# JinfengX/PointCloudPDF

Measured on AMD Instinct MI355X. Metric: points/sec fwd+bwd (PT-v1 Seg50 + PDF U-decoder, 100k-pt scenes), higher is better.
Workload: dtype f32

## Files before the change

### include/pdfops.h

```cpp
#ifndef PDFOPS_H
#define PDFOPS_H

#ifdef __cplusplus
extern "C" {
#endif

#define PDF_OK 0
#define PDF_ERR_BAD_ARG (-1)
#define PDF_ERR_NSAMPLE (-2)
#define PDF_ERR_UNSUPPORTED (-3)

#define PDF_ABI_VERSION 17
int pdf_abi_version(void);
const char *pdf_build_info(void);
int pdf_dist_fma_mode(void);
#define PDF_MMA_F32 0
#define PDF_MMA_F16 1
#define PDF_MMA_BF16 2

int pdf_knn_query(int m, int nsample, const float *xyz, const float *new_xyz,
                  const int *offset, const int *new_offset, int b,
                  int *idx, float *dist2, void *stream);

long pdf_knn_workspace_bytes(int b, int n, int m);
int pdf_knn_grid_supported(int nsample);
int pdf_knn_query_ws(int m, int nsample, int n, const float *xyz, const float *new_xyz, const int *offset,
                     const int *new_offset, int b, int *idx, float *dist2, void *workspace, long workspace_bytes,
                     void *stream);
int pdf_knn_grid_build(int n, const float *xyz, const int *offset, int b, void *workspace, long workspace_bytes, void *stream);
int pdf_knn_query_grid(int m, int nsample, int n, const float *xyz, const float *new_xyz, const int *offset, const int *new_offset, int b,
                       int *idx, float *dist2, void *workspace, long workspace_bytes, void *stream);
int pdf_knn_query_ws_counted(int m, int nsample, int n, const float *xyz, const float *new_xyz, const int *offset,
                             const int *new_offset, int b, int *idx, float *dist2, void *workspace, long workspace_bytes,
                             unsigned long long *pairs, void *stream);
int pdf_knn_query_list(int m, int nsample, const float *xyz, const float *new_xyz, const int *offset,
                       const int *new_offset, int b, int *idx, float *dist2, const int *qlist, const int *qcount,
                       void *stream);

int pdf_ball_query(int m, int nsample, float min_radius, float max_radius, const float *xyz, const float *new_xyz,
                   const int *offset, const int *new_offset, int b, int *idx, float *dist2, void *stream);

int pdf_random_ball_query(int m, int nsample, float min_radius, float max_radius, const int *order, const float *xyz,
                          const float *new_xyz, const int *offset, const int *new_offset, int b, int *idx, float *dist2,
                          void *stream);

int pdf_farthest_point_sampling(int b, int n, const float *xyz, const int *offset,
                                const int *new_offset, float *tmp, int *idx, void *stream);

int pdf_fps_reference_block_log2(int n);

long pdf_fps_workspace_bytes(int b, int n_total);
long pdf_fps_stats_offset(int b, int n_total);
int pdf_farthest_point_sampling_bucketed(int b, int n, int n_total, const float *xyz, const int *offset,
                                         const int *new_offset, void *workspace, long workspace_bytes,
                                         int *idx, void *stream);

int pdf_grouping_forward(int m, int nsample, int c, const float *input, const int *idx, float *output, void *stream);
int pdf_grouping_backward(int m, int nsample, int c, const float *grad_output, const int *idx, float *grad_input, void *stream);
int pdf_grouping_forward_ordered(int m, int nsample, int c, const float *input, const int *idx, const int *order, float *output, void *stream);
int pdf_group_forward_ordered(int m, int nsample, int c, int with_xyz, const float *feat, const float *xyz, const float *new_xyz,
                              const int *idx, const int *order, float *output, void *stream);
int pdf_interpolation_forward_ordered(int n, int c, int k, const float *input, const int *idx, const float *weight, const int *order,
                                      float *output, void *stream);
int pdf_subtraction_forward_ordered(int n, int nsample, int c, const float *input1, const float *input2, const int *idx, const int *order,
                                    float *output, void *stream);
int pdf_aggregation_forward_ordered(int n, int nsample, int c, int w_c, const float *input, const float *position, const float *weight,
                                    const int *idx, const int *order, float *output, void *stream);

int pdf_interpolation_forward(int n, int c, int k, const float *input, const int *idx, const float *weight, float *output, void *stream);
int pdf_interpolation_backward(int n, int c, int k, const float *grad_output, const int *idx, const float *weight, float *grad_input, void *stream);

int pdf_subtraction_forward(int n, int nsample, int c, const float *input1, const float *input2, const int *idx, float *output, void *stream);
int pdf_subtraction_backward(int n, int nsample, int c, const int *idx, const float *grad_output, float *grad_input1, float *grad_input2, void *stream);

int pdf_aggregation_forward(int n, int nsample, int c, int w_c, const float *input, const float *position,
                            const float *weight, const int *idx, float *output, void *stream);
int pdf_aggregation_backward(int n, int nsample, int c, int w_c, const float *input, const float *position,
                             const float *weight, const int *idx, const float *grad_output,
                             float *grad_input, float *grad_position, float *grad_weight, void *stream);

int pdf_attention_relation_step_forward(int m, int g, int c, const float *query, const float *key, const float *weight,
                                        const int *index_target, const int *index_refer, float *output, void *stream);
int pdf_attention_relation_step_backward(int m, int g, int c, const float *query, float *grad_query,
                                         const float *key, float *grad_key, const float *weight, float *grad_weight,
                                         const int *index_target, const int *index_refer, const float *grad_output, void *stream);
int pdf_attention_fusion_step_forward(int m, int g, int c, const float *weight, const float *value,
                                      const int *index_target, const int *index_refer, float *output, void *stream);
int pdf_attention_fusion_step_backward(int m, int g, int c, const float *weight, float *grad_weight,
                                       const float *value, float *grad_value,
                                       const int *index_target, const int *index_refer, const float *grad_output, void *stream);


int pdf_group_forward(int m, int nsample, int c, int with_xyz, const float *feat, const float *xyz,
                      const float *new_xyz, const int *idx, float *output, void *stream);
int pdf_group_backward(int m, int nsample, int c, int with_xyz, const float *grad_output, const int *idx,
                       float *grad_feat, void *stream);

int pdf_interpolation_weights(int n, int k, const float *dist2, float *weight, void *stream);

int pdf_pt_layer_supported(int nsample, int c);
long pdf_pt_layer_partial_floats(int n, int nsample, int c);
int pdf_pt_layer_forward(int n, int nsample, int c, const float *xq, const float *xk, const float *xv,
                         const float *p, const int *idx, const float *const *weights,
                         const float *const *bn_params, float *const *bn_buffers, int training, float eps,
                         float momentum, float *bn, float *saved, float *H, float *partial, float *out,
                         int storage_bf16, const int *order, void *stream);
int pdf_pt_layer_forward_m(int n, int nsample, int c, const float *xq, const float *xk, const float *xv,
                           const float *p, const int *idx, const float *const *weights,
                           const float *const *bn_params, float *const *bn_buffers, int training, float eps,
                           float momentum, float *bn, float *saved, float *H, float *partial, float *out,
                           int storage_bf16, const int *order, const double *moments, int *out_stat_rows, void *stream);

long pdf_pt_layer_bwd_partial_floats(int n, int nsample, int c);
long pdf_pt_layer_bwd_sums_floats(int c);
int pdf_pt_layer_backward(int n, int nsample, int c, const float *xq, const float *xk, const float *xv,
                          const float *p, const int *idx, const float *const *weights, const float *bn,
                          const float *saved, const float *H, const float *gout, float *gxq, float *gxk,
                          float *gxv, float *G2, float *G3, float *Wsm, float *GR, const int *inv_off, const int *inv_entry,
                          int entry_base, float *partial, float *sums, int storage_bf16, const int *order, const double *moments,
                          void *stream);

int pdf_bn_supported(int c);
long pdf_bn_partial_floats(long n, int c);
int pdf_bn_act_forward(long n, int c, const float *x, const float *res, const float *gamma, const float *beta,
                       float *running_mean, float *running_var, int training, float eps, float momentum, int relu,
                       float *coef, float *partial, float *y, void *stream);
int pdf_bn_act_backward(long n, int c, const float *gy, const float *x, const float *res, const float *coef,
                        int training, int relu, float *partial, float *sums, float *gx, float *gres, void *stream);
int pdf_bn_coef(long n, int c, const float *x, const float *gamma, const float *beta, float *running_mean,
                float *running_var, int training, float eps, float momentum, float *coef, float *partial, void *stream);
int pdf_bn_apply(long n, int c, const float *x, const float *res, const float *coef, int relu, float *y, void *stream);

long pdf_rowlin_partial_floats(long n, int o);
int pdf_rowlin_partial_rows(long n, int k, int o);
int pdf_rowlin_forward(long n, int k, int o, const float *x, long ldx, const float *w, int transpose_w,
                       const float *bias, const float *scale, const float *shift, int relu, float *y, long ldy,
                       int accumulate, float *partial, int mma_input, void *stream);
long pdf_rowlin_wgrad_ws_floats(long n, int k, int o, int ng);
int pdf_rowlin_wgrad(long n, int k, int o, const float *g, long ldg, const float *x, long ldx,
                     const float *scale, const float *shift, int relu, float *dw, float *db, float *ws, int mma_input, void *stream);
int pdf_bn_coef_from_partial(const float *partial, int rows, long n, int c, const float *gamma, const float *beta,
                             float *running_mean, float *running_var, float eps, float momentum, float *coef, void *stream);

int pdf_rowlin_multi(long n, int k, int o, int nin, int nout, const float *const *x, long ldx, const float *const *w,
                     int transpose_w, const float *const *bias, const float *scale, const float *shift, int relu,
                     float *const *y, long ldy, int accumulate, int mma_input, void *stream);
int pdf_rowlin_wgrad_multi(long n, int k, int o, int ng, const float *const *g, long ldg, const float *x, long ldx,
                           const float *scale, const float *shift, int relu, float *const *dw, float *const *db, float *ws, int mma_input, void *stream);
int pdf_rowlin_wgrad_group(long n, int k, int o, int ng, const float *const *g, long ldg, const float *const *x, long ldx,
                           const float *const *scale, const float *const *shift, const int *relu, float *const *dw,
                           float *const *db, float *ws, int mma_input, void *stream);

int pdf_kpconv_supported(int kp, int cin);
int pdf_kpconv_gather(int n, int m, int kp, int cin, const float *query, const float *support, const int *neighbors, const float *x,
                      const float *k_points, float extent, float *weighted, void *stream);
int pdf_kpconv_scatter(int n, int m, int kp, int cin, const float *query, const float *support, const int *neighbors,
                       const float *grad_weighted, const float *k_points, float extent, float *grad_x, void *stream);
int pdf_rowlin_dgrad_bstats(long n, int k, int o, int nin, const float *const *x, long ldx, const float *const *w, float *y, long ldy,
                            const float *bx, long ldb, const float *bcoef, int brelu, float *partial, int *partial_rows,
                            int mma_input, void *stream);
int pdf_rowlin_forward_bn(long n, int k, int o, const float *x, long ldx, const float *w, const float *bias, const float *scale,
                          const float *shift, int relu, float *y, long ldy, float *partial, const float *gamma, const float *beta,
                          float *running_mean, float *running_var, float eps, float momentum, float *coef, int mma_input, void *stream);
int pdf_bn_act_backward_presummed(long n, int c, const float *gy, const float *x, const float *coef, int training, int relu,
                                  const float *partial, int partial_rows, float *sums, float *gx, void *stream);

int pdf_bn_coef_eval_or_partial(const float *partial, int rows, long n, int c, const float *gamma, const float *beta,
                                float *running_mean, float *running_var, int training, float eps, float momentum,
                                float *coef, void *stream);
int pdf_block_pre_forward(long n, int c, void *const *p, int training, float eps, float momentum, int mma_input, void *stream);
int pdf_block_pre_backward(long n, int c, void *const *p, int training, int mma_input, void *stream);
int pdf_block_post_forward(long n, int c, void *const *p, int training, float eps, float momentum, int mma_input, void *stream);
int pdf_block_post_backward(long n, int c, void *const *p, int training, int mma_input, void *stream);
int pdf_bottleneck_forward(long n, int nsample, int c, void *const *p, int training, float eps, float momentum, int storage_bf16, int mma_input, void *stream);
int pdf_bottleneck_backward(long n, int nsample, int c, void *const *p, int training, int entry_base, int storage_bf16, int mma_input, void *stream);
int pdf_linbn_forward(long n, int k, int o, void *const *p, int training, int relu, float eps, float momentum, int mma_input, void *stream);
int pdf_linbn_backward(long n, int k, int o, void *const *p, int training, int relu, int mma_input, void *stream);

int pdf_rowlin_forward_roww(long n, int k, int o, const float *x, long ldx, const float *w, int transpose_w, float *y, long ldy,
                            int accumulate, const float *roww, long rws, int mma_input, void *stream);
int pdf_rowlin_wgrad_roww(long n, int k, int o, const float *g, long ldg, const float *x, long ldx, float *dw, const float *roww,
                          long rws, float *ws, int mma_input, void *stream);
int pdf_bn_bwd_sums(long n, int c, const float *gy, const float *x, const float *coef, int relu, float *partial, float *sums,
                    void *stream);

int pdf_td_supported(int nsample, int cin, int cout);
int pdf_td_tables(long m, int b, const float *p_src, const float *p_new, const int *idx, const int *new_offset, float *rel4, float *Z,
                  float *scene_sums, long n, const int *inv_off, const int *inv_entry, int entry_base,
                  void *stream);
long pdf_td_gram_floats(int cin);
long pdf_td_fwd_scratch_floats(long n, int cin);
long pdf_td_bwd_scratch_floats(long m, int cin, int cout);
int pdf_td_forward(long n, long m, int cin, int cout, void *const *p, int training, float eps, float momentum, int mma_input, void *stream);
int pdf_td_backward(long n, long m, int cin, int cout, void *const *p, int entry_base, int mma_input, void *stream);

int pdf_seg_sum_rows(long n, int c, const float *src, const int *inv_off, const int *inv_entry, int entry_base, float scale, float *out,
                     void *stream);
int pdf_seg_sum_rows_own(long n, int c, int nsample, const float *src, const int *inv_off, const int *inv_entry, int entry_base, float scale,
                         const int *order, float *out, float *out_own, void *stream);
int pdf_seg_sum_rows_strided(long n, int c, const float *src, long src_stride, const int *inv_off, const int *inv_entry, int entry_base,
                             float scale, float *out, void *stream);
int pdf_seg_sum_rows_x(long n, int c, const float *src, long src_stride, int src_bf16, const int *inv_off, const int *inv_entry, int entry_base,
                       float scale, float *out, void *stream);
int pdf_seg_sum_weighted_x(long n, int c, int nsample, int w_c, const float *src, const float *w, int w_bf16, const int *inv_off,
                           const int *inv_entry, int entry_base, const int *order, float *out, void *stream);
int pdf_seg_sum_weighted_ordered(long n, int c, int nsample, int w_c, const float *src, const float *w, const int *inv_off,
                                 const int *inv_entry, int entry_base, const int *order, float *out, void *stream);
int pdf_seg_sum_weighted(long n, int c, int nsample, int w_c, const float *src, const float *w, const int *inv_off, const int *inv_entry,
                         int entry_base, float *out, void *stream);

long pdf_ce_workspace_floats(void);
int pdf_ce_forward(long n, int c, const float *logits, const long *target, long ignore, float *grad, float *acc, float *loss,
                   void *stream);
int pdf_ce_backward(long n, int c, const float *dlogits, const float *acc, const float *gy, float *grad_out, void *stream);

#define PDF_REDUCE_NONE 0
#define PDF_REDUCE_MEAN 1
#define PDF_REDUCE_SUM 2
long pdf_criteria_workspace_floats(int c);
int pdf_ce_ex_forward(long n, int c, const float *logits, const long *target, const float *weight, float label_smoothing, int reduction,
                      long ignore, float *grad, float *acc, float *loss, void *stream);
int pdf_ce_ex_backward(long n, int c, const float *dlogits, const float *acc, const float *gy, int reduction, float *grad_out, void *stream);
int pdf_focal_forward(long n, int c, const float *logits, const long *target, const float *alpha_vec, float alpha, float gamma, int reduction,
                      long ignore, float *grad, float *acc, float *loss, void *stream);
int pdf_focal_backward(long n, int c, const float *dlogits, const float *acc, const float *gy, float *grad_out, void *stream);
int pdf_dice_forward(long n, int c, const float *logits, const long *target, float smooth, float exponent, long ignore, float *prob,
                     float *acc, float *loss, void *stream);
int pdf_dice_backward(long n, int c, const float *prob, const long *target, long ignore, float exponent, const float *acc, const float *gy,
                      float *grad_out, void *stream);
int pdf_bfocal_forward(long n, const float *pred, const float *target, float alpha, float gamma, int logits, int reduce, float *grad,
                       float *acc, float *loss, void *stream);
int pdf_bfocal_backward(long n, const float *dpred, const float *acc, const float *gy, int reduce, float *grad_out, void *stream);

int pdf_cac_supported(int K, int c);
long pdf_cac_workspace_floats(long n, int K, int c, int scenes);
int pdf_cac_soft_proto_forward(long n, int K, int c, int scenes, const float *feat, const float *logits, const int *offset,
                               float conf_thresh, float *proto, float *mass, float *ws, void *stream);
int pdf_cac_soft_proto_backward(long n, int K, int c, int scenes, const float *feat, const float *logits, const int *offset,
                                float conf_thresh, const float *proto, const float *mass, const float *gproto, float *gfeat,
                                float *glogits, void *stream);
int pdf_cac_label_proto_forward(long n, int K, int c, const float *feat, const long *target, const float *base, float *proto,
                                float *count, float *ws, void *stream);
int pdf_cac_label_proto_backward(long n, int K, int c, const long *target, const float *count, const float *gproto, float *gfeat,
                                 void *stream);
int pdf_cac_cosine_forward(long n, int K, int c, int scenes, const float *x, const float *proto, const int *offset, float scale,
                           float *out, void *stream);
int pdf_cac_cosine_backward(long n, int K, int c, int scenes, const float *x, const float *proto, const int *offset, float scale,
                            const float *gout, float *gx, float *gproto, float *ws, void *stream);
// ... 252 lines not shown
```

### pointcloudpdf_amd/_native.py

```python
import ctypes
import os
import threading

import torch

_HERE = os.path.dirname(os.path.abspath(__file__))
DIST_FMA = int(os.environ.get("PDFOPS_DIST_FMA", "0") or 0)
if DIST_FMA not in (0, 1, 2):
    raise RuntimeError(f"PDFOPS_DIST_FMA={DIST_FMA}: expected 0 (as written), 1 or 2 (csrc/pdfops_common.h)")


def library_path(dist_fma=0):
    return os.path.join(_HERE, "lib", "libpdfops.so" if not dist_fma else f"libpdfops_fma{int(dist_fma)}.so")


LIB_PATH = library_path(DIST_FMA)
ABI_VERSION = 17

c_int = ctypes.c_int
c_long = ctypes.c_long
c_void_p = ctypes.c_void_p
c_float = ctypes.c_float
c_double = ctypes.c_double

_PROTOS = {
    "knn_query": "iippppipp",
    "ball_query": "iiffppppipp",
    "random_ball_query": "iiffpppppipp",
    "farthest_point_sampling": "iippppp",
    "grouping_forward": "iiippp",
    "grouping_backward": "iiippp",
    "interpolation_forward": "iiipppp",
    "interpolation_backward": "iiipppp",
    "subtraction_forward": "iiipppp",
    "subtraction_backward": "iiipppp",
    "aggregation_forward": "iiiippppp",
    "aggregation_backward": "iiiipppppppp",
    "attention_relation_step_forward": "iiipppppp",
    "attention_relation_step_backward": "iiippppppppp",
    "attention_fusion_step_forward": "iiippppp",
    "attention_fusion_step_backward": "iiippppppp",
    "attention_step1_forward_v2": "iiiiippppp",
    "attention_step1_backward_v2": "iiiiippppppp",
    "dot_prod_with_idx_forward_v3": "iiiiipppppppp",
    "dot_prod_with_idx_backward_v3": "iiiiipppppppppppp",
    "attention_step2_with_rel_pos_value_forward_v2": "iiiiippppppp",
    "attention_step2_with_rel_pos_value_backward_v2": "iiiiipppppppppp",
    "segment_softmax_forward": "iiippp",
    "segment_softmax_backward": "iiipppp",
}
_HIP_ONLY_PROTOS = {
    "grid_hash": "lippdddippp",
    "grid_hash_f64": "lippdddppp",
    "philox4x64": "llllp",
    "aug_bounds": "ippppp",
    "aug_points": "ilpipppppp",
    "aug_keys": "ilpplp",
    "aug_elastic_noise": "ilpplp",
    "aug_elastic_blur": "ilpppi",
    "aug_elastic_apply": "ilpppppdpp",
    "radius_neighbors_self": "iifppipppl",
    "radius_neighbors_self_adaptive": "iiffppippppl",
    "vote_accumulate": "lipppppp",
    "fragment_bounds": "lliiipppppp",
    "fragment_gather": "lliiipppppipppppppp",
    "fragment_vote": "lliiippppppppp",
    "graph_forest": "lipppppipppl",
    "gmm2_1d": "ipppidd",
    "dot_prod_with_idx_forward_v3_l": "iiiiipppppppp",
    "dot_prod_with_idx_backward_v3_l": "iiiiipppppppppppp",
    "attention_step2_with_rel_pos_value_backward_v2_l": "iiiiipppppppppp",
    "scene_sum_rows": "ipiplip",
    "scene_repeat_rows": "iplipip",
    "region_stats": "ippppifppp",
    "region_seeds": "ippppip",
    "region_grow": "ippipppipiipppp",
    "region_edges": "ipppppippppppppppppl",
    "sort_floats_dev": "ipppppp",
    "gmm2_weak_dev": "ippppppppidd",
    "region_mask": "ippppppp",
    "region_tree": "ippipppppppp",
    "graph_forest_dev": "lipppppippppl",
    "gmm2_1d_dev": "ippppidd",
    "graph_forest_batch_dev": "ippippppppipppl",
    "wa_segment_rows": "iiiipppppplfpplf",
    "wa_segment_rows_ordered": "iiiipppppplfpplfp",
    "wa_table_grad": "iiiippppplfpp",
    "wa_grad_attn": "iiiiiplppplppp",
    "wa_logits_forward": "iiiiipplfpppppp",
    "wa_permute_edges": "iippp",
    "wa_logits_forward_ordered": "iiiiipplfppppppp",
    "wa_grad_attn_ordered": "iiiiiplppplpppp",
    "window_keys": "ippippfippp",
    "window_keys_scene": "ippippfippp",
    "scene_bounds": "ippipp",
    "window_edges_count": "ippipppppp",
    "window_edges_fill": "ipppppppffipppp",
    "group_forward": "iiiippppp",
    "group_backward": "iiiippp",
    "interpolation_weights": "iipp",
# ... 570 lines not shown
        lib.pdf_spconv_colsum_ws_floats.restype = c_long
        lib.pdf_spconv_colsum_ws_floats.argtypes = [c_int]
        lib.pdf_incr_kl_workspace_floats.restype = c_long
        lib.pdf_incr_kl_workspace_floats.argtypes = []
        lib.pdf_incr_kl_forward.restype = c_int
        lib.pdf_incr_kl_forward.argtypes = [c_long, c_int, c_int, c_void_p, c_void_p, c_void_p, c_long, ctypes.c_float, ctypes.c_float,
                                            c_void_p, c_void_p, c_void_p, c_void_p]
        lib.pdf_incr_kl_backward.restype = c_int
        lib.pdf_incr_kl_backward.argtypes = [c_long, c_int, c_void_p, c_void_p, c_void_p, c_void_p, c_void_p]
        lib.pdf_lovasz_workspace_bytes.restype = c_long
        lib.pdf_lovasz_workspace_bytes.argtypes = [c_long, c_int]
        lib.pdf_lovasz_forward.restype = c_int
        lib.pdf_lovasz_forward.argtypes = [c_long, c_int, c_void_p, c_void_p, c_long, c_void_p, c_void_p, c_void_p, c_void_p, c_void_p, c_void_p]
        lib.pdf_lovasz_backward.restype = c_int
        lib.pdf_lovasz_backward.argtypes = [c_long, c_int, c_void_p, c_void_p, ctypes.c_float, c_void_p, c_void_p]
        lib.pdf_openset_metrics_workspace_bytes.restype = c_long
        lib.pdf_openset_metrics_workspace_bytes.argtypes = [c_long, c_int]
        lib.pdf_openset_metrics.restype = c_int
        lib.pdf_openset_metrics.argtypes = [c_long, c_int, c_void_p, c_void_p, c_void_p, c_void_p, c_long, c_void_p, c_int, c_void_p, c_void_p,
                                            c_void_p, c_void_p]
        lib.pdf_knn_rel_moments.restype = c_int
        lib.pdf_knn_rel_moments.argtypes = [c_int, c_long, c_int, c_void_p, c_void_p, c_void_p, c_void_p, c_void_p, c_void_p]
        lib.pdf_knn_rel_moments_ws_doubles.restype = c_long
        lib.pdf_knn_rel_moments_ws_doubles.argtypes = [c_int, c_long]
        lib.pdf_knn_rel_moments_q.restype = c_int
        lib.pdf_knn_rel_moments_q.argtypes = [c_int, c_long, c_int, c_void_p, c_void_p, c_void_p, c_void_p, c_void_p, c_void_p, c_void_p]
        class CopySeg(ctypes.Structure):
            _fields_ = [("src", c_void_p), ("dst", c_void_p), ("nbytes", c_long), ("src_offset", c_void_p), ("sub", c_void_p),
                        ("sub_const", c_int), ("src_elems", c_int)]

        self.CopySeg = CopySeg
        lib.pdf_stage_copy.restype = c_int
        lib.pdf_stage_copy.argtypes = [c_int, c_void_p, c_void_p]
        lib.pdf_scene_morton_keys.restype = c_int
        lib.pdf_scene_morton_keys.argtypes = [c_long, c_int, c_void_p, c_void_p, c_void_p, c_void_p, c_void_p]
        lib.pdf_sgd_chunk.restype = c_int
        lib.pdf_sgd_chunk.argtypes = []
        lib.pdf_sgd_step.restype = c_int
        lib.pdf_sgd_step.argtypes = [c_int, c_void_p, c_void_p, ctypes.c_float, ctypes.c_float, ctypes.c_float, c_void_p, c_void_p]
        lib.pdf_grad_unscale.restype = c_int
        lib.pdf_grad_unscale.argtypes = [c_int, c_void_p, c_void_p, c_void_p, c_void_p, c_void_p]
        lib.pdf_scaler_update.restype = c_int
        lib.pdf_scaler_update.argtypes = [c_void_p, c_void_p, c_void_p, c_void_p, ctypes.c_float, ctypes.c_float, c_int, c_void_p]
        lib.pdf_adam_step.restype = c_int
        lib.pdf_adam_step.argtypes = [c_int, c_int, c_void_p, c_void_p, ctypes.c_double, ctypes.c_double, ctypes.c_double, ctypes.c_double,
                                      ctypes.c_double, c_int, c_void_p, c_void_p]
        lib.pdf_adam_grad_unscale.restype = c_int
        lib.pdf_adam_grad_unscale.argtypes = [c_int, c_void_p, c_void_p, c_void_p, c_void_p, c_void_p]
        lib.pdf_linbn_forward.restype = c_int
        lib.pdf_linbn_forward.argtypes = [c_long, c_int, c_int, c_void_p, c_int, c_int, ctypes.c_float, ctypes.c_float, c_int, c_void_p]
        lib.pdf_linbn_backward.restype = c_int
        lib.pdf_linbn_backward.argtypes = [c_long, c_int, c_int, c_void_p, c_int, c_int, c_int, c_void_p]
        lib.pdf_bottleneck_forward.restype = c_int
        lib.pdf_bottleneck_forward.argtypes = [c_long, c_int, c_int, c_void_p, c_int, ctypes.c_float, ctypes.c_float, c_int, c_int, c_void_p]
        lib.pdf_bottleneck_backward.restype = c_int
        lib.pdf_bottleneck_backward.argtypes = [c_long, c_int, c_int, c_void_p, c_int, c_int, c_int, c_int, c_void_p]
        for nm in ("pre_backward", "post_backward"):
            f = getattr(lib, "pdf_block_" + nm)
            f.restype = c_int
            f.argtypes = [c_long, c_int, c_void_p, c_int, c_int, c_void_p]
        lib.pdf_rowlin_multi.restype = c_int
        lib.pdf_rowlin_multi.argtypes = [c_long, c_int, c_int, c_int, c_int, c_void_p, c_long, c_void_p, c_int, c_void_p, c_void_p, c_void_p,
                                         c_int, c_void_p, c_long, c_int, c_int, c_void_p]
        lib.pdf_kpconv_supported.restype = c_int
        lib.pdf_kpconv_supported.argtypes = [c_int, c_int]
        for nm in ("pdf_kpconv_gather", "pdf_kpconv_scatter"):
            f = getattr(lib, nm)
            f.restype = c_int
            f.argtypes = [c_int, c_int, c_int, c_int, c_void_p, c_void_p, c_void_p, c_void_p, c_void_p, ctypes.c_float, c_void_p, c_void_p]
        lib.pdf_rowlin_wgrad_group.restype = c_int
        lib.pdf_rowlin_wgrad_group.argtypes = [c_long, c_int, c_int, c_int, c_void_p, c_long, c_void_p, c_long, c_void_p, c_void_p, c_void_p,
                                               c_void_p, c_void_p, c_void_p, c_int, c_void_p]
        lib.pdf_rowlin_wgrad_multi.restype = c_int
        lib.pdf_rowlin_wgrad_multi.argtypes = [c_long, c_int, c_int, c_int, c_void_p, c_long, c_void_p, c_long, c_void_p, c_void_p, c_int,
                                               c_void_p, c_void_p, c_void_p, c_int, c_void_p]
        lib.pdf_rowlin_wgrad_ws_floats.restype = c_long
        lib.pdf_rowlin_wgrad_ws_floats.argtypes = [c_long, c_int, c_int, c_int]
        lib.pdf_rowlin_dgrad_bstats.restype = c_int
        lib.pdf_rowlin_dgrad_bstats.argtypes = [c_long, c_int, c_int, c_int, c_void_p, c_long, c_void_p, c_void_p, c_long, c_void_p, c_long,
                                                c_void_p, c_int, c_void_p, ctypes.POINTER(c_int), c_int, c_void_p]
        lib.pdf_bn_act_backward_presummed.restype = c_int
        lib.pdf_bn_act_backward_presummed.argtypes = [c_long, c_int, c_void_p, c_void_p, c_void_p, c_int, c_int, c_void_p, c_int, c_void_p,
                                                      c_void_p, c_void_p]
        lib.pdf_rowlin_partial_floats.restype = c_long
        lib.pdf_rowlin_partial_floats.argtypes = [c_long, c_int]
        lib.pdf_rowlin_partial_rows.restype = c_int
        lib.pdf_rowlin_partial_rows.argtypes = [c_long, c_int, c_int]
        lib.pdf_rowlin_forward.restype = c_int
        lib.pdf_rowlin_forward.argtypes = [c_long, c_int, c_int, c_void_p, c_long, c_void_p, c_int, c_void_p, c_void_p, c_void_p,
                                           c_int, c_void_p, c_long, c_int, c_void_p, c_int, c_void_p]
        lib.pdf_rowlin_wgrad.restype = c_int
        lib.pdf_rowlin_wgrad.argtypes = [c_long, c_int, c_int, c_void_p, c_long, c_void_p, c_long, c_void_p, c_void_p, c_int,
                                         c_void_p, c_void_p, c_void_p, c_int, c_void_p]
        lib.pdf_bn_coef_from_partial.restype = c_int
        lib.pdf_bn_coef_from_partial.argtypes = [c_void_p, c_int, c_long, c_int, c_void_p, c_void_p, c_void_p, c_void_p,
                                                 ctypes.c_float, ctypes.c_float, c_void_p, c_void_p]
        lib.pdf_bn_coef.restype = c_int
        lib.pdf_bn_coef.argtypes = [c_long, c_int, c_void_p, c_void_p, c_void_p, c_void_p, c_void_p, c_int, ctypes.c_float,
                                    ctypes.c_float, c_void_p, c_void_p, c_void_p]
        lib.pdf_bn_apply.restype = c_int
        lib.pdf_bn_apply.argtypes = [c_long, c_int, c_void_p, c_void_p, c_void_p, c_int, c_void_p, c_void_p]
        lib.pdf_bn_supported.restype = c_int
        lib.pdf_bn_supported.argtypes = [c_int]
        lib.pdf_bn_partial_floats.restype = c_long
        lib.pdf_bn_partial_floats.argtypes = [c_long, c_int]
        lib.pdf_bn_act_forward.restype = c_int
        lib.pdf_bn_act_forward.argtypes = [c_long, c_int] + [c_void_p] * 6 + [c_int, ctypes.c_float, ctypes.c_float, c_int] + [c_void_p] * 4
        lib.pdf_bn_act_backward.restype = c_int
        lib.pdf_bn_act_backward.argtypes = [c_long, c_int] + [c_void_p] * 4 + [c_int, c_int] + [c_void_p] * 5
        lib.pdf_pt_layer_supported.restype = c_int
        lib.pdf_pt_layer_supported.argtypes = [c_int, c_int]
        for fn in (lib.pdf_pt_layer_partial_floats, lib.pdf_pt_layer_bwd_partial_floats):
            fn.restype = c_long
            fn.argtypes = [c_int, c_int, c_int]
        lib.pdf_pt_layer_bwd_sums_floats.restype = c_long
        lib.pdf_pt_layer_bwd_sums_floats.argtypes = [c_int]
        lib.pdf_pt_layer_forward.restype = c_int
        lib.pdf_pt_layer_forward.argtypes = [c_int, c_int, c_int] + [c_void_p] * 8 + [c_int, ctypes.c_float, ctypes.c_float] + [c_void_p] * 5 + [c_int, c_void_p, c_void_p]
        lib.pdf_knn_grid_build.restype = c_int
        lib.pdf_knn_grid_build.argtypes = [c_int, c_void_p, c_void_p, c_int, c_void_p, c_long, c_void_p]
        lib.pdf_knn_query_grid.restype = c_int
        lib.pdf_knn_query_grid.argtypes = [c_int, c_int, c_int, c_void_p, c_void_p, c_void_p, c_void_p, c_int, c_void_p, c_void_p, c_void_p, c_long, c_void_p]
        lib.pdf_pt_layer_backward.restype = c_int
        lib.pdf_pt_layer_backward.argtypes = [c_int, c_int, c_int] + [c_void_p] * 19 + [c_int] + [c_void_p] * 2 + [c_int, c_void_p, c_void_p, c_void_p]
        lib.pdf_grid_pool_workspace_bytes.restype = c_long
        lib.pdf_grid_pool_workspace_bytes.argtypes = [c_long]
        lib.pdf_gva_supported.restype = c_int
        lib.pdf_gva_supported.argtypes = [c_int, c_int, c_int]
        self.fps_mode = os.environ.get("PDFOPS_FPS", "bucketed")
        self.knn_mode = os.environ.get("PDFOPS_KNN", "grid")
        lib.pdf_knn_workspace_bytes.restype = c_long
        lib.pdf_knn_workspace_bytes.argtypes = [c_int, c_int, c_int]
        lib.pdf_graph_forest_workspace_bytes.restype = c_long
        lib.pdf_region_grow_list_points.restype = c_long
        lib.pdf_region_grow_list_points.argtypes = []
        lib.pdf_graph_forest_workspace_bytes.argtypes = [c_long, c_long, c_long]
        lib.pdf_knn_grid_supported.restype = c_int
        lib.pdf_knn_grid_supported.argtypes = [c_int]
        lib.pdf_knn_query_ws.restype = c_int
        lib.pdf_knn_query_ws.argtypes = [c_int, c_int, c_int] + [c_void_p] * 4 + [c_int] + [c_void_p] * 3 + [c_long, c_void_p]
        lib.pdf_knn_query_ws_counted.restype = c_int
        lib.pdf_knn_query_ws_counted.argtypes = [c_int, c_int, c_int] + [c_void_p] * 4 + [c_int] + [c_void_p] * 3 + [c_long, c_void_p, c_void_p]

    KNN_GRID_MAX_SCENES = 64
    use_inverse = os.environ.get("PDFOPS_INVERSE", "1") != "0"
    storage_bf16 = os.environ.get("PDFOPS_STORAGE", "f32") == "bf16"

    def set_storage(self, kind):
        if kind not in ("f32", "bf16"):
            raise ValueError("storage: 'f32' or 'bf16'")
        self.storage_bf16 = kind == "bf16"

    def grouping_forward(self, input, idx):
        _check(input, torch.float32, "input"); _check(idx, torch.int32, "idx")
        m, ns = idx.shape
        c = input.shape[1]
        out = self._new(input, (m, ns, c), torch.float32)
        self._call("grouping_forward_ordered", m, ns, c, input, idx, order_of(idx), out)
        return out

    def interpolation_forward(self, input, idx, weight):
        _check(input, torch.float32, "input"); _check(idx, torch.int32, "idx"); _check(weight, torch.float32, "weight")
        n, k = idx.shape
        c = input.shape[1]
        out = self._new(input, (n, c), torch.float32)
        self._call("interpolation_forward_ordered", n, c, k, input, idx, weight, order_of(idx), out)
# ... 1534 lines not shown
```

### pointcloudpdf_amd/csrc/block.hip

```cpp
#include "pdfops_common.h"

namespace {
struct Err {
    int rc = 0;
    Err &operator<<(int r) { if (rc == 0 && r != 0) rc = r; return *this; }
};

}

extern "C" int pdf_bn_coef_eval_or_partial(const float *partial, int rows, long n, int c, const float *gamma, const float *beta,
                                           float *running_mean, float *running_var, int training, float eps, float momentum,
                                           float *coef, void *stream) {
    if (training) return pdf_bn_coef_from_partial(partial, rows, n, c, gamma, beta, running_mean, running_var, eps, momentum, coef, stream);
    return pdf_bn_coef(n, c, nullptr, gamma, beta, running_mean, running_var, 0, eps, momentum, coef, nullptr, stream);
}

extern "C" int pdf_block_pre_forward(long n, int c, void *const *p, int training, float eps, float momentum, int mma_input, void *stream) {
    if (n < 1 || !p) return PDF_ERR_BAD_ARG;
    if (!pdf_bn_supported(c)) return PDF_ERR_UNSUPPORTED;
    const float *x = (const float *)p[0], *W1 = (const float *)p[1], *g1 = (const float *)p[2], *b1 = (const float *)p[3];
    float *rm1 = (float *)p[4], *rv1 = (float *)p[5];
    float *z1 = (float *)p[12], *coef1 = (float *)p[13], *partial = (float *)p[17];
    Err e;
    if (training) {
        e << pdf_rowlin_forward_bn(n, c, c, x, c, W1, nullptr, nullptr, nullptr, 0, z1, c, partial, g1, b1, rm1, rv1, eps, momentum, coef1, mma_input, stream);
    } else {
        e << pdf_rowlin_forward(n, c, c, x, c, W1, 0, nullptr, nullptr, nullptr, 0, z1, c, 0, nullptr, mma_input, stream);
        e << pdf_bn_coef_eval_or_partial(partial, 0, n, c, g1, b1, rm1, rv1, 0, eps, momentum, coef1, stream);
    }
    const float *xs[1] = {z1}, *ws[3] = {(const float *)p[6], (const float *)p[8], (const float *)p[10]};
    const float *bs[3] = {(const float *)p[7], (const float *)p[9], (const float *)p[11]};
    float *ys[3] = {(float *)p[14], (float *)p[15], (float *)p[16]};
    e << pdf_rowlin_multi(n, c, c, 1, 3, xs, c, ws, 0, bs, coef1, coef1 + c, 1, ys, c, 0, mma_input, stream);
    return e.rc;
}

static bool inkernel_bn() {
    static const bool on = [] { const char *v = getenv("PDFOPS_INKERNEL_BN"); return !(v && v[0] == '0'); }();
    return on;
}
static bool dgrad_bstats() {
    static const bool on = [] { const char *v = getenv("PDFOPS_DGRAD_BSTATS"); return !(v && v[0] == '0'); }();
    return on;
}

static int block_pre_backward(long n, int c, void *const *p, int training, int accumulate_gx, int mma_input, void *stream, bool defer_wgrad = false) {
    if (n < 1 || !p || !p[14]) return PDF_ERR_BAD_ARG;
    const float *x = (const float *)p[0], *z1 = (const float *)p[1], *coef1 = (const float *)p[2], *W1 = (const float *)p[3];
    float *gx = (float *)p[10], *grads = (float *)p[11], *dy = (float *)p[12], *partial = (float *)p[13], *wslab = (float *)p[14];
    const long cc = (long)c * c;
    float *dW1 = grads, *db1 = grads + cc, *dqkv = db1 + 2 * c;
    Err e;
    const float *gs[3] = {(const float *)p[7], (const float *)p[8], (const float *)p[9]};
    const float *ws[3] = {(const float *)p[4], (const float *)p[5], (const float *)p[6]};
    float *dws[3] = {dqkv, dqkv + (cc + c), dqkv + 2 * (cc + c)}, *dbs[3] = {dqkv + cc, dqkv + (cc + c) + cc, dqkv + 2 * (cc + c) + cc};
    float *ys[1] = {dy};
    if (!defer_wgrad) e << pdf_rowlin_wgrad_multi(n, c, c, 3, gs, c, z1, c, coef1, coef1 + c, 1, dws, dbs, wslab, mma_input, stream);
    int prow = 0;
    const int rc1 = dgrad_bstats() ? pdf_rowlin_dgrad_bstats(n, c, c, 3, gs, c, ws, dy, c, z1, c, coef1, 1, partial, &prow, mma_input, stream) : PDF_ERR_UNSUPPORTED;
    if (rc1 == PDF_ERR_UNSUPPORTED) {
        e << pdf_rowlin_multi(n, c, c, 3, 1, gs, c, ws, 1, nullptr, nullptr, nullptr, 0, ys, c, 0, mma_input, stream);
        e << pdf_bn_act_backward(n, c, dy, z1, nullptr, coef1, training, 1, partial, db1, dy, nullptr, stream);
    } else {
        e << rc1;
        e << pdf_bn_act_backward_presummed(n, c, dy, z1, coef1, training, 1, partial, prow, db1, dy, stream);
    }
    if (!defer_wgrad) e << pdf_rowlin_wgrad(n, c, c, dy, c, x, c, nullptr, nullptr, 0, dW1, nullptr, wslab, mma_input, stream);
    e << pdf_rowlin_forward(n, c, c, dy, c, W1, 1, nullptr, nullptr, nullptr, 0, gx, c, accumulate_gx, nullptr, mma_input, stream);
    return e.rc;
}

extern "C" int pdf_block_pre_backward(long n, int c, void *const *p, int training, int mma_input, void *stream) {
    return block_pre_backward(n, c, p, training, 0, mma_input, stream, false);
}

static int block_post_forward(long n, int c, void *const *p, int training, float eps, float momentum, int t_stat_rows, int mma_input, void *stream) {
    if (n < 1 || !p) return PDF_ERR_BAD_ARG;
    if (!pdf_bn_supported(c)) return PDF_ERR_UNSUPPORTED;
    const float *t = (const float *)p[0], *x = (const float *)p[1];
    float *coef2 = (float *)p[11], *z3 = (float *)p[12], *coef3 = (float *)p[13], *y = (float *)p[14], *partial = (float *)p[15];
    Err e;
    if (training && t_stat_rows > 0)
        e << pdf_bn_coef_from_partial(partial, t_stat_rows, n, c, (const float *)p[2], (const float *)p[3], (float *)p[4], (float *)p[5], eps, momentum, coef2, stream);
    else
        e << pdf_bn_coef(n, c, t, (const float *)p[2], (const float *)p[3], (float *)p[4], (float *)p[5], training, eps, momentum, coef2, partial, stream);
    bool applied = false;
    if (training && inkernel_bn()) {
        int rows = 0;
        const int rc = pdf_rowlin_forward_stats_ho(n, c, c, t, c, (const float *)p[6], nullptr, coef2, coef2 + c, 1, z3, c, partial + PDF_HO_FLOATS, partial,
                                                   &rows, mma_input, stream);
        if (rc == PDF_OK) {
            e << pdf_bn_apply_rows(n, c, z3, x, partial + PDF_HO_FLOATS, rows, (const float *)p[7], (const float *)p[8], (float *)p[9], (float *)p[10], eps,
                                   momentum, coef3, partial, 1, y, stream);
            applied = true;
        } else if (rc != PDF_ERR_UNSUPPORTED) {
            e << rc;
        }
    }
    if (applied) return e.rc;
    if (training) {
        e << pdf_rowlin_forward_bn(n, c, c, t, c, (const float *)p[6], nullptr, coef2, coef2 + c, 1, z3, c, partial, (const float *)p[7], (const float *)p[8],
                                   (float *)p[9], (float *)p[10], eps, momentum, coef3, mma_input, stream);
    } else {
        e << pdf_rowlin_forward(n, c, c, t, c, (const float *)p[6], 0, nullptr, coef2, coef2 + c, 1, z3, c, 0, nullptr, mma_input, stream);
        e << pdf_bn_coef_eval_or_partial(partial, 0, n, c, (const float *)p[7], (const float *)p[8], (float *)p[9], (float *)p[10], 0, eps, momentum, coef3, stream);
    }
    e << pdf_bn_apply(n, c, z3, x, coef3, 1, y, stream);
    return e.rc;
}
extern "C" int pdf_block_post_forward(long n, int c, void *const *p, int training, float eps, float momentum, int mma_input, void *stream) {
    return block_post_forward(n, c, p, training, eps, momentum, 0, mma_input, stream);
}

static int block_post_backward(long n, int c, void *const *p, int training, int mma_input, void *stream, bool defer_wgrad = false) {
    if (n < 1 || !p || !p[12]) return PDF_ERR_BAD_ARG;
    const float *gy = (const float *)p[0], *t = (const float *)p[1], *x = (const float *)p[2], *z3 = (const float *)p[3];
    const float *coef2 = (const float *)p[4], *coef3 = (const float *)p[5], *W3 = (const float *)p[6];
    float *gt = (float *)p[7], *gres = (float *)p[8], *grads = (float *)p[9], *da = (float *)p[10], *partial = (float *)p[11];
    const long cc = (long)c * c;
    float *dW3 = grads, *db2 = grads + cc, *db3 = db2 + 2 * c;
    Err e;
    e << pdf_bn_act_backward(n, c, gy, z3, x, coef3, training, 1, partial, db3, da, gres, stream);
    if (!defer_wgrad) e << pdf_rowlin_wgrad(n, c, c, da, c, t, c, coef2, coef2 + c, 1, dW3, nullptr, (float *)p[12], mma_input, stream);
    int prow = 0;
    const float *das[1] = {da}, *w3s[1] = {W3};
    const int rc2 = dgrad_bstats() ? pdf_rowlin_dgrad_bstats(n, c, c, 1, das, c, w3s, gt, c, t, c, coef2, 1, partial, &prow, mma_input, stream) : PDF_ERR_UNSUPPORTED;
    if (rc2 == PDF_ERR_UNSUPPORTED) {
        e << pdf_rowlin_forward(n, c, c, da, c, W3, 1, nullptr, nullptr, nullptr, 0, gt, c, 0, nullptr, mma_input, stream);
        e << pdf_bn_act_backward(n, c, gt, t, nullptr, coef2, training, 1, partial, db2, gt, nullptr, stream);
    } else {
        e << rc2;
        e << pdf_bn_act_backward_presummed(n, c, gt, t, coef2, training, 1, partial, prow, db2, gt, stream);
    }
    return e.rc;
}

extern "C" int pdf_block_post_backward(long n, int c, void *const *p, int training, int mma_input, void *stream) {
    return block_post_backward(n, c, p, training, mma_input, stream, false);
}

extern "C" int pdf_bottleneck_forward(long n, int nsample, int c, void *const *p, int training, float eps, float momentum, int storage_bf16, int mma_input, void *stream) {
    if (n < 1 || !p) return PDF_ERR_BAD_ARG;
    Err e;
    void *pre[18] = {p[0], p[1], p[2], p[3], p[4], p[5], p[6], p[7], p[8], p[9], p[10], p[11], p[43], p[44], p[45], p[46], p[47], p[56]};
    e << pdf_block_pre_forward(n, c, pre, training, eps, momentum, mma_input, stream);
    const float *weights[8], *bn_params[6];
    float *bn_buffers[6];
    for (int i = 0; i < 8; ++i) weights[i] = (const float *)p[14 + i];
    for (int i = 0; i < 6; ++i) { bn_params[i] = (const float *)p[22 + i]; bn_buffers[i] = (float *)p[28 + i]; }
    static const bool p4_stats = [] { const char *v = getenv("PDFOPS_P4_STATS"); return !(v && v[0] == '0'); }();
    int t_rows = 0;
    e << pdf_pt_layer_forward_m((int)n, nsample, c, (const float *)p[45], (const float *)p[46], (const float *)p[47], (const float *)p[12],
                                (const int *)p[13], weights, bn_params, bn_buffers, training, eps, momentum, (float *)p[48], (float *)p[49],
                                (float *)p[50], (float *)p[56], (float *)p[51], storage_bf16, (const int *)p[57], (const double *)p[58],
                                p4_stats ? &t_rows : nullptr, stream);
    void *post[16] = {p[51], p[0], p[34], p[35], p[36], p[37], p[38], p[39], p[40], p[41], p[42], p[52], p[53], p[54], p[55], p[56]};
    e << block_post_forward(n, c, post, training, eps, momentum, e.rc == 0 ? t_rows : 0, mma_input, stream);
    return e.rc;
}

extern "C" int pdf_bottleneck_backward(long n, int nsample, int c, void *const *p, int training, int entry_base, int storage_bf16, int mma_input, void *stream) {
    if (n < 1 || !p) return PDF_ERR_BAD_ARG;
    Err e;
    if (!p[50]) return PDF_ERR_BAD_ARG;
    static const bool group = [] { const char *v = getenv("PDFOPS_WGRAD_GROUP"); return !(v && v[0] == '0'); }();
    float *ws_post = (float *)p[50], *ws_pre = ws_post + pdf_rowlin_wgrad_ws_floats(n, c, c, 1);
    void *post[13] = {p[0], p[24], p[1], p[25], p[26], p[27], p[28], p[33], p[29], p[31], p[34], p[40], ws_post};
    e << block_post_backward(n, c, post, training, mma_input, stream, group);
    const float *weights[8];
    for (int i = 0; i < 8; ++i) weights[i] = (const float *)p[10 + i];
    e << pdf_pt_layer_backward((int)n, nsample, c, (const float *)p[21], (const float *)p[22], (const float *)p[23], (const float *)p[8],
                               (const int *)p[9], weights, (const float *)p[18], (const float *)p[19], (const float *)p[20],
                               (const float *)p[33], (float *)p[35], (float *)p[36], (float *)p[37], (float *)p[38], (float *)p[39],
                               (float *)p[41], (float *)p[42], (const int *)p[43], (const int *)p[44], entry_base,
                               (float *)p[40], (float *)p[32], storage_bf16, (const int *)p[49], (const double *)p[46], stream);
    void *pre[15] = {p[1], p[2], p[3], p[4], p[5], p[6], p[7], p[35], p[36], p[37], p[29], p[30], p[45], p[40], ws_pre};
    e << block_pre_backward(n, c, pre, training, 1, mma_input, stream, group);
    if (group && e.rc == 0) {
        const long cc = (long)c * c;
        float *gpre = (float *)p[30], *gpost = (float *)p[31];
        float *dW1 = gpre, *dqkv = gpre + cc + 2 * c, *dW3 = gpost;
        const float *coef1 = (const float *)p[3], *coef2 = (const float *)p[26];
        const float *g[5] = {(const float *)p[34], (const float *)p[35], (const float *)p[36], (const float *)p[37], (const float *)p[45]};
        const float *x[5] = {(const float *)p[24], (const float *)p[2], (const float *)p[2], (const float *)p[2], (const float *)p[1]};
        const float *sc[5] = {coef2, coef1, coef1, coef1, nullptr}, *sh[5] = {coef2 + c, coef1 + c, coef1 + c, coef1 + c, nullptr};
        const int relu[5] = {1, 1, 1, 1, 0};
        float *dw[5] = {dW3, dqkv, dqkv + (cc + c), dqkv + 2 * (cc + c), dW1};
        float *db[5] = {nullptr, dqkv + cc, dqkv + (cc + c) + cc, dqkv + 2 * (cc + c) + cc, nullptr};
        const int rc = pdf_rowlin_wgrad_group(n, c, c, 5, g, c, x, c, sc, sh, relu, dw, db, ws_post, mma_input, stream);
        if (rc == PDF_ERR_UNSUPPORTED) {
            e << pdf_rowlin_wgrad(n, c, c, g[0], c, x[0], c, sc[0], sh[0], 1, dw[0], nullptr, ws_post, mma_input, stream);
            e << pdf_rowlin_wgrad_multi(n, c, c, 3, g + 1, c, x[1], c, sc[1], sh[1], 1, dw + 1, db + 1, ws_pre, mma_input, stream);
            e << pdf_rowlin_wgrad(n, c, c, g[4], c, x[4], c, nullptr, nullptr, 0, dw[4], nullptr, ws_pre, mma_input, stream);
        } else {
            e << rc;
        }
    }
    return e.rc;
}

extern "C" int pdf_linbn_forward(long n, int k, int o, void *const *p, int training, int relu, float eps, float momentum, int mma_input, void *stream) {
    if (n < 1 || !p) return PDF_ERR_BAD_ARG;
    if (!pdf_bn_supported(o)) return PDF_ERR_UNSUPPORTED;
    Err e;
    float *z = (float *)p[7], *coef = (float *)p[8], *partial = (float *)p[10];
    if (training) {
        e << pdf_rowlin_forward_bn(n, k, o, (const float *)p[0], k, (const float *)p[1], (const float *)p[2], nullptr, nullptr, 0, z, o, partial,
                                   (const float *)p[3], (const float *)p[4], (float *)p[5], (float *)p[6], eps, momentum, coef, mma_input, stream);
    } else {
        e << pdf_rowlin_forward(n, k, o, (const float *)p[0], k, (const float *)p[1], 0, (const float *)p[2], nullptr, nullptr, 0, z, o, 0, nullptr, mma_input, stream);
        e << pdf_bn_coef_eval_or_partial(partial, 0, n, o, (const float *)p[3], (const float *)p[4], (float *)p[5], (float *)p[6], 0, eps, momentum, coef, stream);
    }
    e << pdf_bn_apply(n, o, z, nullptr, coef, relu, (float *)p[9], stream);
    return e.rc;
}

extern "C" int pdf_linbn_backward(long n, int k, int o, void *const *p, int training, int relu, int mma_input, void *stream) {
    if (n < 1 || !p || !p[9]) return PDF_ERR_BAD_ARG;
    float *grads = (float *)p[6], *gz = (float *)p[7];
    const long ok = (long)o * k;
    Err e;
    e << pdf_bn_act_backward(n, o, (const float *)p[0], (const float *)p[2], nullptr, (const float *)p[3], training, relu, (float *)p[8],
                             grads + ok + o, gz, nullptr, stream);
    if (p[5]) e << pdf_rowlin_forward(n, o, k, gz, o, (const float *)p[4], 1, nullptr, nullptr, nullptr, 0, (float *)p[5], k, 0, nullptr, mma_input, stream);
    e << pdf_rowlin_wgrad(n, k, o, gz, o, (const float *)p[1], k, nullptr, nullptr, 0, grads, grads + ok, (float *)p[9], mma_input, stream);
    return e.rc;
}
```

### pointcloudpdf_amd/csrc/pdfops_common.h

```cpp
#pragma once
#include <hip/hip_runtime.h>
#include <stdint.h>
#include <atomic>
#include "../../include/pdfops.h"

#define PDF_WAVE 64
#define PDF_MAX_DEVICES_LDS 64

static inline int pdf_launch_status() {
    hipError_t e = hipGetLastError();
    return e == hipSuccess ? PDF_OK : (int)e;
}

struct PdfLdsLimit { std::atomic<int> state[PDF_MAX_DEVICES_LDS]; };
static inline bool pdf_lds_limit_raised(PdfLdsLimit &site, const void *kernel, int bytes) {
    int dev = 0;
    if (hipGetDevice(&dev) != hipSuccess || dev < 0 || dev >= PDF_MAX_DEVICES_LDS) return hipFuncSetAttribute(kernel, hipFuncAttributeMaxDynamicSharedMemorySize, bytes) == hipSuccess;
    int st = site.state[dev].load(std::memory_order_acquire);
    if (st == 0) {
        st = hipFuncSetAttribute(kernel, hipFuncAttributeMaxDynamicSharedMemorySize, bytes) == hipSuccess ? 1 : 2;
        if (st == 2) (void)hipGetLastError();
        site.state[dev].store(st, std::memory_order_release);
    }
    return st == 1;
// ... 9 lines not shown
        T *p = reinterpret_cast<T *>(reinterpret_cast<uintptr_t>(base) + off);
        off += (count * sizeof(T) + 255) & ~(size_t)255;
        return p;
    }
};

#define PDF_MAX_BLOCKS 2048

__device__ __forceinline__ int pdf_lane() { return (int)(threadIdx.x & 63); }

__device__ __forceinline__ void wave_sync() {
    __builtin_amdgcn_fence(__ATOMIC_RELEASE, "wavefront");
    __builtin_amdgcn_wave_barrier();
    __builtin_amdgcn_fence(__ATOMIC_ACQUIRE, "wavefront");
}

__device__ __forceinline__ int pdf_wave_min_i32(int v) {
#pragma unroll
    for (int o = 32; o >= 1; o >>= 1) v = min(v, __shfl_xor(v, o, 64));
    return v;
}
__device__ __forceinline__ int pdf_wave_max_i32(int v) {
#pragma unroll
    for (int o = 32; o >= 1; o >>= 1) v = max(v, __shfl_xor(v, o, 64));
    return v;
}
__device__ __forceinline__ unsigned long long pdf_wave_max_u64(unsigned long long v) {
#pragma unroll
    for (int o = 32; o >= 1; o >>= 1) {
        unsigned long long w = __shfl_xor(v, o, 64);
        v = w > v ? w : v;
    }
    return v;
}
__device__ __forceinline__ float pdf_wave_sum_f32(float v) {
#pragma unroll
    for (int o = 32; o >= 1; o >>= 1) v += __shfl_xor(v, o, 64);
    return v;
}

#ifndef PDF_DIST_FMA
#define PDF_DIST_FMA 0
#endif
__host__ __device__ __forceinline__ float pdf_sqdist3(float dx, float dy, float dz) {
#if PDF_DIST_FMA == 1
    return __builtin_fmaf(dz, dz, __builtin_fmaf(dy, dy, dx * dx));
#elif PDF_DIST_FMA == 2
    return __builtin_fmaf(dz, dz, __builtin_fmaf(dx, dx, dy * dy));
#else
    return dx * dx + dy * dy + dz * dz;
#endif
}

__device__ __forceinline__ unsigned pdf_f32_ordered(float f) {
    unsigned u = __float_as_uint(f);
    return (u & 0x80000000u) ? ~u : (u | 0x80000000u);
}

__device__ __forceinline__ void pdf_atomic_add(float *p, float v) {
    __hip_atomic_fetch_add(p, v, __ATOMIC_RELAXED, __HIP_MEMORY_SCOPE_AGENT);
}

#define PDF_XCDS 8
__device__ __forceinline__ unsigned pdf_xcd_chunked_block(unsigned b, unsigned g) {
    const unsigned q = g / PDF_XCDS, r = g % PDF_XCDS, x = b % PDF_XCDS;
    return (x < r ? x * (q + 1) : r * (q + 1) + (x - r) * q) + b / PDF_XCDS;
}

struct PdfRowsBn {
    const float *rows; int nrows; int c; double count;
    const float *gamma, *beta; float *running_mean, *running_var; float eps, momentum;
    float *coef;
    unsigned long long *gran;
    unsigned *sync;
};
#define PDF_HO_WORDS(c) (2 * (size_t)(c) * 2 + 4)
#define PDF_HO_FLOATS PDF_HO_WORDS(1024)
int pdf_rowlin_forward_stats_ho(long n, int k, int o, const float *x, long ldx, const float *w, const float *bias, const float *scale,
                                const float *shift, int relu, float *y, long ldy, float *rows_out, void *handoff, int *rows, int mma_input,
                                void *stream);
int pdf_bn_apply_rows(long n, int c, const float *x, const float *res, const float *rows, int nrows, const float *gamma, const float *beta,
                      float *running_mean, float *running_var, float eps, float momentum, float *coef, void *handoff, int relu, float *y,
                      void *stream);

__device__ __forceinline__ void pdf_handoff_zero(unsigned long long *gran, int c, unsigned *sync) {
    for (int e = threadIdx.x; e < 2 * c; e += blockDim.x) gran[e] = 0ull;
    if (threadIdx.x == 0) sync[0] = 0u;
}

template <int NT>
__device__ __forceinline__ void pdf_bn_reduce_slice(const PdfRowsBn &b, int sl, double *lds_red) {
    constexpr int RL = NT / 16;
    const int c = b.c, cl = threadIdx.x & 15, rl = threadIdx.x >> 4;
    const int ch = sl * 16 + cl;
    double s = 0.0, ss = 0.0;
    if (ch < c) {
        const float *p0 = b.rows + ch, *p1 = b.rows + c + ch;
        const size_t stride = 2 * (size_t)c;
        for (int r = rl; r < b.nrows; r += 8 * RL) {
            float v0[8], v1[8];
#pragma unroll
            for (int t = 0; t < 8; ++t) {
                const int rr = r + t * RL < b.nrows ? r + t * RL : b.nrows - 1;
                v0[t] = p0[(size_t)rr * stride]; v1[t] = p1[(size_t)rr * stride];
            }
#pragma unroll
            for (int t = 0; t < 8; ++t) {
                const bool ok = r + t * RL < b.nrows;
                s += ok ? (double)v0[t] : 0.0; ss += ok ? (double)v1[t] : 0.0;
            }
        }
    }
    __syncthreads();
    lds_red[(0 * RL + rl) * 17 + cl] = s;
    lds_red[(1 * RL + rl) * 17 + cl] = ss;
    __syncthreads();
    if (rl == 0 && ch < c) {
        double a = 0.0, q = 0.0;
        for (int k = 0; k < RL; ++k) { a += lds_red[(0 * RL + k) * 17 + cl]; q += lds_red[(1 * RL + k) * 17 + cl]; }
        const double mean = a / b.count;
        double var = q / b.count - mean * mean;
        if (var < 0.0) var = 0.0;
        const float rstd = (float)(1.0 / sqrt(var + (double)b.eps));
        const float sc = b.gamma[ch] * rstd, sh = b.beta[ch] - (float)mean * sc;
        b.coef[ch] = sc; b.coef[c + ch] = sh; b.coef[2 * c + ch] = (float)mean; b.coef[3 * c + ch] = rstd;
        if (b.running_mean && b.sync != nullptr) {
            const double unbiased = b.count > 1.0 ? var * b.count / (b.count - 1.0) : var;
            b.running_mean[ch] = (1.f - b.momentum) * b.running_mean[ch] + b.momentum * (float)mean;
            b.running_var[ch] = (1.f - b.momentum) * b.running_var[ch] + b.momentum * (float)unbiased;
        }
        __hip_atomic_store(b.gran + ch, (1ull << 32) | (unsigned long long)__float_as_uint(sc), __ATOMIC_RELAXED, __HIP_MEMORY_SCOPE_AGENT);
        __hip_atomic_store(b.gran + c + ch, (1ull << 32) | (unsigned long long)__float_as_uint(sh), __ATOMIC_RELAXED, __HIP_MEMORY_SCOPE_AGENT);
    }
}

template <int NT>
__device__ __forceinline__ void pdf_bn_coef_inkernel(const PdfRowsBn &b, float *lds_coef, double *lds_red, unsigned *lds_word) {
    (void)lds_word;
    const int c = b.c, nsl = (c + 15) / 16;
    const unsigned me = blockIdx.x + gridDim.x * (blockIdx.y + gridDim.y * blockIdx.z), nblk = gridDim.x * gridDim.y * gridDim.z;
    for (unsigned sl = me; sl < (unsigned)nsl; sl += nblk) pdf_bn_reduce_slice<NT>(b, (int)sl, lds_red);
    for (unsigned spins = 0;; ++spins) {
        bool ok = true;
        for (int e = threadIdx.x; e < 2 * c; e += NT) {
            const unsigned long long g = __hip_atomic_load(b.gran + e, __ATOMIC_RELAXED, __HIP_MEMORY_SCOPE_AGENT);
            ok = ok && (g >> 32) == 1ull;
            lds_coef[e] = __uint_as_float((unsigned)g);
        }
        if (__syncthreads_and(ok)) break;
        if (spins == (1u << 14)) {
            PdfRowsBn mine = b;
            mine.sync = nullptr;
            for (int sl = 0; sl < nsl; ++sl) pdf_bn_reduce_slice<NT>(mine, sl, lds_red);
        }
        __builtin_amdgcn_s_sleep(8);
    }
}
```

### pointcloudpdf_amd/csrc/pointwise.hip

```cpp
#include "pdfops_common.h"
#include <cstdlib>

namespace pw {

constexpr int PB = 256;
constexpr int MAXB = 1024;

static inline int grid_rows(long n, int c) {
    const long rows_per_block = (long)PB * 4 / c > 0 ? (long)PB * 4 / c : 1;
    static const int short_rows = [] { const char *v = getenv("PDFOPS_BN_ROWS_SHORT"); const int x = v ? atoi(v) : 0; return x > 0 ? x : 4; }();
    const long per = n * c >= (1L << 22) ? 8 : short_rows;
    long g = (n + rows_per_block * per - 1) / (rows_per_block * per);
    if (g > MAXB) g = MAXB;
    if (g < 1) g = 1;
    return (int)g;
}

__global__ __launch_bounds__(PB) void k_bn_stats(long n, int c, const float *__restrict__ x, float *partial) {
    extern __shared__ float red[];
    const int tpr = c / 4;
    const int rpb = PB / tpr;
    const int tr = threadIdx.x / tpr, tc = threadIdx.x % tpr;
    float s[4] = {0.f, 0.f, 0.f, 0.f}, ss[4] = {0.f, 0.f, 0.f, 0.f};
    if (tr < rpb) {
        for (long r = (long)blockIdx.x * rpb + tr; r < n; r += (long)gridDim.x * rpb) {
            const float4 v = *reinterpret_cast<const float4 *>(x + r * c + tc * 4);
            s[0] += v.x; s[1] += v.y; s[2] += v.z; s[3] += v.w;
            ss[0] += v.x * v.x; ss[1] += v.y * v.y; ss[2] += v.z * v.z; ss[3] += v.w * v.w;
        }
    }
#pragma unroll
    for (int k = 0; k < 4; ++k) { red[threadIdx.x * 8 + k] = s[k]; red[threadIdx.x * 8 + 4 + k] = ss[k]; }
    __syncthreads();
    if (threadIdx.x < tpr) {
#pragma unroll
        for (int k = 0; k < 8; ++k) {
            float a = 0.f;
            for (int rr = 0; rr < rpb; ++rr) a += red[(rr * tpr + threadIdx.x) * 8 + k];
            const int ch = threadIdx.x * 4 + (k & 3);
            partial[(size_t)blockIdx.x * 2 * c + (k < 4 ? ch : c + ch)] = a;
        }
    }
}

template <bool RES>
__global__ __launch_bounds__(PB) void k_bn_apply(long n4, int c4, const float4 *__restrict__ x, const float4 *__restrict__ scale,
                                                 const float4 *__restrict__ shift, const float4 *__restrict__ res, int relu,
                                                 float4 *__restrict__ y) {
    for (long e = (long)blockIdx.x * PB + threadIdx.x; e < n4; e += (long)gridDim.x * PB) {
        const int cc = (int)(e % c4);
        const float4 v = x[e], sc = scale[cc], sh = shift[cc];
        const float4 r = RES ? res[e] : make_float4(0.f, 0.f, 0.f, 0.f);
        float4 o = make_float4(v.x * sc.x + sh.x + r.x, v.y * sc.y + sh.y + r.y, v.z * sc.z + sh.z + r.z, v.w * sc.w + sh.w + r.w);
        if (relu) { o.x = fmaxf(o.x, 0.f); o.y = fmaxf(o.y, 0.f); o.z = fmaxf(o.z, 0.f); o.w = fmaxf(o.w, 0.f); }
        y[e] = o;
    }
}

template <bool RES>
__global__ __launch_bounds__(PB) void k_bn_apply_rows(long n4, int c4, const float4 *__restrict__ x, PdfRowsBn b, const float4 *__restrict__ res,
                                                      int relu, float4 *__restrict__ y) {
    extern __shared__ __attribute__((aligned(16))) float lds[];
    const int c = 4 * c4;
    double *red = reinterpret_cast<double *>(lds + 2 * c);
    unsigned *word = reinterpret_cast<unsigned *>(red + 2 * (PB / 16) * 17);
    pdf_bn_coef_inkernel<PB>(b, lds, red, word);
    const float4 *scale = reinterpret_cast<const float4 *>(lds), *shift = reinterpret_cast<const float4 *>(lds + c);
    for (long e = (long)blockIdx.x * PB + threadIdx.x; e < n4; e += (long)gridDim.x * PB) {
        const int cc = (int)(e % c4);
        const float4 v = x[e], sc = scale[cc], sh = shift[cc];
        const float4 r = RES ? res[e] : make_float4(0.f, 0.f, 0.f, 0.f);
        float4 o = make_float4(v.x * sc.x + sh.x + r.x, v.y * sc.y + sh.y + r.y, v.z * sc.z + sh.z + r.z, v.w * sc.w + sh.w + r.w);
        if (relu) { o.x = fmaxf(o.x, 0.f); o.y = fmaxf(o.y, 0.f); o.z = fmaxf(o.z, 0.f); o.w = fmaxf(o.w, 0.f); }
        y[e] = o;
    }
}

template <bool RES>
__global__ __launch_bounds__(PB) void k_bn_bwd_reduce(long n, int c, const float *__restrict__ gy, const float *__restrict__ x,
                                                      const float *__restrict__ res, const float *__restrict__ scale,
                                                      const float *__restrict__ shift, const float *__restrict__ mean,
                                                      const float *__restrict__ rstd, int relu, float *partial) {
    extern __shared__ float red[];
    const int tpr = c / 4, rpb = PB / tpr;
    const int tr = threadIdx.x / tpr, tc = threadIdx.x % tpr;
    float s[4] = {0.f, 0.f, 0.f, 0.f}, sx[4] = {0.f, 0.f, 0.f, 0.f};
    if (tr < rpb) {
        float sc[4], sh[4], mu[4], rs[4];
#pragma unroll
        for (int k = 0; k < 4; ++k) { sc[k] = scale[tc * 4 + k]; sh[k] = shift[tc * 4 + k]; mu[k] = mean[tc * 4 + k]; rs[k] = rstd[tc * 4 + k]; }
        for (long r = (long)blockIdx.x * rpb + tr; r < n; r += (long)gridDim.x * rpb) {
            const float4 g4 = *reinterpret_cast<const float4 *>(gy + r * c + tc * 4);
            const float4 x4 = *reinterpret_cast<const float4 *>(x + r * c + tc * 4);
            const float4 r4 = RES ? *reinterpret_cast<const float4 *>(res + r * c + tc * 4) : make_float4(0.f, 0.f, 0.f, 0.f);
            const float g[4] = {g4.x, g4.y, g4.z, g4.w}, xv[4] = {x4.x, x4.y, x4.z, x4.w}, rv[4] = {r4.x, r4.y, r4.z, r4.w};
#pragma unroll
            for (int k = 0; k < 4; ++k) {
                const float pre = xv[k] * sc[k] + sh[k] + rv[k];
                const float gm = (!relu || pre > 0.f) ? g[k] : 0.f;
                s[k] += gm;
                sx[k] += gm * ((xv[k] - mu[k]) * rs[k]);
            }
        }
    }
#pragma unroll
    for (int k = 0; k < 4; ++k) { red[threadIdx.x * 8 + k] = s[k]; red[threadIdx.x * 8 + 4 + k] = sx[k]; }
    __syncthreads();
    if (threadIdx.x < tpr) {
#pragma unroll
        for (int k = 0; k < 8; ++k) {
            float a = 0.f;
            for (int rr = 0; rr < rpb; ++rr) a += red[(rr * tpr + threadIdx.x) * 8 + k];
            const int ch = threadIdx.x * 4 + (k & 3);
            partial[(size_t)blockIdx.x * 2 * c + (k < 4 ? ch : c + ch)] = a;
        }
    }
}

template <bool RES>
__global__ __launch_bounds__(PB) void k_bn_bwd_apply(long n4, int c4, const float4 *__restrict__ gy, const float4 *__restrict__ x,
                                                     const float4 *__restrict__ res, const float4 *__restrict__ scale,
                                                     const float4 *__restrict__ shift, const float4 *__restrict__ mean,
                                                     const float4 *__restrict__ rstd, const float4 *__restrict__ sums, float inv_n,
                                                     int relu, float4 *__restrict__ gx, float4 *__restrict__ gres) {
    for (long e = (long)blockIdx.x * PB + threadIdx.x; e < n4; e += (long)gridDim.x * PB) {
        const int cc = (int)(e % c4);
        const float4 g4 = gy[e], x4 = x[e], sc = scale[cc], sh = shift[cc], mu = mean[cc], rs = rstd[cc];
        const float4 s1 = sums[cc], s2 = sums[c4 + cc];
        const float4 r4 = RES ? res[e] : make_float4(0.f, 0.f, 0.f, 0.f);
        float4 gm, o;
#define PW_ONE(f)                                                                     \
        {                                                                             \
            const float pre = x4.f * sc.f + sh.f + r4.f;                              \
            gm.f = (!relu || pre > 0.f) ? g4.f : 0.f;                                 \
            const float xh = (x4.f - mu.f) * rs.f;                                    \
            o.f = sc.f * (gm.f - s1.f * inv_n - xh * s2.f * inv_n);                   \
        }
        PW_ONE(x) PW_ONE(y) PW_ONE(z) PW_ONE(w)
#undef PW_ONE
        gx[e] = o;
        if (gres) gres[e] = gm;
    }
}

template <bool RES>
__global__ __launch_bounds__(PB) void k_bn_bwd_eval(long n4, int c4, const float4 *__restrict__ gy, const float4 *__restrict__ x,
                                                    const float4 *__restrict__ res, const float4 *__restrict__ scale,
                                                    const float4 *__restrict__ shift, int relu, float4 *__restrict__ gx,
                                                    float4 *__restrict__ gres) {
    for (long e = (long)blockIdx.x * PB + threadIdx.x; e < n4; e += (long)gridDim.x * PB) {
        const int cc = (int)(e % c4);
        const float4 g4 = gy[e], x4 = x[e], sc = scale[cc], sh = shift[cc];
        const float4 r4 = RES ? res[e] : make_float4(0.f, 0.f, 0.f, 0.f);
        float4 gm;
        gm.x = (!relu || x4.x * sc.x + sh.x + r4.x > 0.f) ? g4.x : 0.f;
        gm.y = (!relu || x4.y * sc.y + sh.y + r4.y > 0.f) ? g4.y : 0.f;
        gm.z = (!relu || x4.z * sc.z + sh.z + r4.z > 0.f) ? g4.z : 0.f;
        gm.w = (!relu || x4.w * sc.w + sh.w + r4.w > 0.f) ? g4.w : 0.f;
        gx[e] = make_float4(gm.x * sc.x, gm.y * sc.y, gm.z * sc.z, gm.w * sc.w);
        if (gres) gres[e] = gm;
    }
}

static inline int grid_elems(long n4) {
    long g = (n4 + PB - 1) / PB;
    if (g > 2048) g = 2048;
    if (g < 1) g = 1;
    return (int)g;
}

}

namespace fl {
void launch_bn_finalize(const float *partial, int rows, int nch, double count, const float *gamma, const float *beta, float eps,
                        float momentum, float *running_mean, float *running_var, float *scale, float *shift, float *mean_out,
                        float *rstd_out, hipStream_t s);
void launch_bn_eval(int nch, const float *gamma, const float *beta, float eps, const float *running_mean, const float *running_var,
                    float *scale, float *shift, float *mean_out, float *rstd_out, hipStream_t s);
void launch_colsum(const float *partial, int rows, int width, float *out, hipStream_t s);
}

extern "C" int pdf_bn_supported(int c) { return c >= 4 && c % 4 == 0 && c <= 1024 && (1024 % c == 0); }
extern "C" long pdf_bn_partial_floats(long n, int c) { return (long)pw::grid_rows(n, c) * 2 * c + (long)PDF_HO_FLOATS; }

extern "C" int pdf_bn_act_forward(long n, int c, const float *x, const float *res, const float *gamma, const float *beta,
                                  float *running_mean, float *running_var, int training, float eps, float momentum,
                                  int relu, float *coef, float *partial, float *y, void *stream) {
    if (n < 1 || !x || !gamma || !beta || !coef || !y) return PDF_ERR_BAD_ARG;
    if (!pdf_bn_supported(c)) return PDF_ERR_UNSUPPORTED;
    hipStream_t s = static_cast<hipStream_t>(stream);
    float *scale = coef, *shift = coef + c, *mean = coef + 2 * c, *rstd = coef + 3 * c;
    if (training) {
        if (!partial) return PDF_ERR_BAD_ARG;
        const int g = pw::grid_rows(n, c);
        pw::k_bn_stats<<<g, pw::PB, pw::PB * 8 * sizeof(float), s>>>(n, c, x, partial);
        fl::launch_bn_finalize(partial, g, c, (double)n, gamma, beta, eps, momentum, running_mean, running_var, scale, shift, mean, rstd, s);
    } else {
        if (!running_mean || !running_var) return PDF_ERR_BAD_ARG;
        fl::launch_bn_eval(c, gamma, beta, eps, running_mean, running_var, scale, shift, mean, rstd, s);
    }
    const long n4 = n * (c / 4);
    (res ? pw::k_bn_apply<true> : pw::k_bn_apply<false>)<<<pw::grid_elems(n4), pw::PB, 0, s>>>(n4, c / 4, reinterpret_cast<const float4 *>(x),
                                                        reinterpret_cast<const float4 *>(scale), reinterpret_cast<const float4 *>(shift),
                                                        reinterpret_cast<const float4 *>(res), relu, reinterpret_cast<float4 *>(y));
    return pdf_launch_status();
}

static int bn_act_backward(long n, int c, const float *gy, const float *x, const float *res, const float *coef,
                           int training, int relu, float *partial, float *sums, int sums_zeroed, float *gx, float *gres, void *stream,
                           int presummed = 0) {
    (void)sums_zeroed;
    if (n < 1 || !gy || !x || !coef || !partial || !sums || !gx) return PDF_ERR_BAD_ARG;
    if (!pdf_bn_supported(c)) return PDF_ERR_UNSUPPORTED;
    hipStream_t s = static_cast<hipStream_t>(stream);
    const float *scale = coef, *shift = coef + c, *mean = coef + 2 * c, *rstd = coef + 3 * c;
    const int g = pw::grid_rows(n, c);
    const long n4 = n * (c / 4);
    if (presummed > 0) {
        fl::launch_colsum(partial, presummed, 2 * c, sums, s);
    } else {
        (res ? pw::k_bn_bwd_reduce<true> : pw::k_bn_bwd_reduce<false>)<<<g, pw::PB, pw::PB * 8 * sizeof(float), s>>>(
            n, c, gy, x, res, scale, shift, mean, rstd, relu, partial);
        fl::launch_colsum(partial, g, 2 * c, sums, s);
    }
#define F4(p) reinterpret_cast<const float4 *>(p)
    if (training)
        (res ? pw::k_bn_bwd_apply<true> : pw::k_bn_bwd_apply<false>)<<<pw::grid_elems(n4), pw::PB, 0, s>>>(n4, c / 4, F4(gy), F4(x), F4(res), F4(scale), F4(shift), F4(mean), F4(rstd),
                                                                F4(sums), (float)(1.0 / (double)n), relu, reinterpret_cast<float4 *>(gx),
                                                                reinterpret_cast<float4 *>(gres));
    else
        (res ? pw::k_bn_bwd_eval<true> : pw::k_bn_bwd_eval<false>)<<<pw::grid_elems(n4), pw::PB, 0, s>>>(n4, c / 4, F4(gy), F4(x), F4(res), F4(scale), F4(shift), relu,
                                                               reinterpret_cast<float4 *>(gx), reinterpret_cast<float4 *>(gres));
#undef F4
    return pdf_launch_status();
}

extern "C" int pdf_bn_act_backward(long n, int c, const float *gy, const float *x, const float *res, const float *coef,
                                   int training, int relu, float *partial, float *sums, float *gx, float *gres, void *stream) {
    return bn_act_backward(n, c, gy, x, res, coef, training, relu, partial, sums, 0, gx, gres, stream);
}
extern "C" int pdf_bn_act_backward_presummed(long n, int c, const float *gy, const float *x, const float *coef, int training, int relu,
                                             const float *partial, int partial_rows, float *sums, float *gx, void *stream) {
    if (partial_rows < 1 || !partial) return PDF_ERR_BAD_ARG;
    return bn_act_backward(n, c, gy, x, nullptr, coef, training, relu, const_cast<float *>(partial), sums, 0, gx, nullptr, stream, partial_rows);
}
extern "C" int pdf_bn_coef_from_partial(const float *partial, int rows, long n, int c, const float *gamma, const float *beta,
                                        float *running_mean, float *running_var, float eps, float momentum, float *coef,
                                        void *stream) {
    if (!partial || rows < 1 || n < 1 || c < 1 || !gamma || !beta || !coef) return PDF_ERR_BAD_ARG;
    fl::launch_bn_finalize(partial, rows, c, (double)n, gamma, beta, eps, momentum, running_mean, running_var, coef, coef + c,
                           coef + 2 * c, coef + 3 * c, static_cast<hipStream_t>(stream));
    return pdf_launch_status();
}

extern "C" int pdf_bn_apply(long n, int c, const float *x, const float *res, const float *coef, int relu, float *y, void *stream) {
    if (n < 1 || !x || !coef || !y) return PDF_ERR_BAD_ARG;
    if (!pdf_bn_supported(c)) return PDF_ERR_UNSUPPORTED;
    const long n4 = n * (c / 4);
    (res ? pw::k_bn_apply<true> : pw::k_bn_apply<false>)<<<pw::grid_elems(n4), pw::PB, 0, static_cast<hipStream_t>(stream)>>>(
        n4, c / 4, reinterpret_cast<const float4 *>(x), reinterpret_cast<const float4 *>(coef), reinterpret_cast<const float4 *>(coef + c),
        reinterpret_cast<const float4 *>(res), relu, reinterpret_cast<float4 *>(y));
    return pdf_launch_status();
}

int pdf_bn_apply_rows(long n, int c, const float *x, const float *res, const float *rows, int nrows, const float *gamma, const float *beta,
                      float *running_mean, float *running_var, float eps, float momentum, float *coef, void *handoff, int relu, float *y,
                      void *stream) {
    if (n < 1 || !x || !rows || nrows < 1 || !gamma || !beta || !coef || !handoff || !y) return PDF_ERR_BAD_ARG;
    if (!pdf_bn_supported(c)) return PDF_ERR_UNSUPPORTED;
    PdfRowsBn b;
    b.rows = rows; b.nrows = nrows; b.c = c; b.count = (double)n; b.gamma = gamma; b.beta = beta; b.running_mean = running_mean;
    b.running_var = running_var; b.eps = eps; b.momentum = momentum; b.coef = coef;
    b.gran = static_cast<unsigned long long *>(handoff); b.sync = reinterpret_cast<unsigned *>(b.gran + 2 * (size_t)c);
    const long n4 = n * (c / 4);
    const size_t lds = sizeof(float) * 2 * c + sizeof(double) * 2 * (pw::PB / 16) * 17 + 16;
    (res ? pw::k_bn_apply_rows<true> : pw::k_bn_apply_rows<false>)<<<pw::grid_elems(n4), pw::PB, lds, static_cast<hipStream_t>(stream)>>>(
        n4, c / 4, reinterpret_cast<const float4 *>(x), b, reinterpret_cast<const float4 *>(res), relu, reinterpret_cast<float4 *>(y));
    return pdf_launch_status();
}

extern "C" int pdf_bn_coef(long n, int c, const float *x, const float *gamma, const float *beta, float *running_mean,
                           float *running_var, int training, float eps, float momentum, float *coef, float *partial, void *stream) {
    if (n < 1 || !gamma || !beta || !coef) return PDF_ERR_BAD_ARG;
    if (!pdf_bn_supported(c)) return PDF_ERR_UNSUPPORTED;
    hipStream_t s = static_cast<hipStream_t>(stream);
    if (training) {
        if (!partial || !x) return PDF_ERR_BAD_ARG;
        const int g = pw::grid_rows(n, c);
        pw::k_bn_stats<<<g, pw::PB, pw::PB * 8 * sizeof(float), s>>>(n, c, x, partial);
        fl::launch_bn_finalize(partial, g, c, (double)n, gamma, beta, eps, momentum, running_mean, running_var, coef, coef + c, coef + 2 * c, coef + 3 * c, s);
    } else {
        if (!running_mean || !running_var) return PDF_ERR_BAD_ARG;
        fl::launch_bn_eval(c, gamma, beta, eps, running_mean, running_var, coef, coef + c, coef + 2 * c, coef + 3 * c, s);
    }
    return pdf_launch_status();
}

extern "C" int pdf_bn_bwd_sums(long n, int c, const float *gy, const float *x, const float *coef, int relu, float *partial, float *sums,
                               void *stream) {
    if (n < 1 || !gy || !x || !coef || !partial || !sums) return PDF_ERR_BAD_ARG;
    if (!pdf_bn_supported(c)) return PDF_ERR_UNSUPPORTED;
    hipStream_t s = static_cast<hipStream_t>(stream);
    const int g = pw::grid_rows(n, c);
    pw::k_bn_bwd_reduce<false><<<g, pw::PB, pw::PB * 8 * sizeof(float), s>>>(n, c, gy, x, nullptr, coef, coef + c, coef + 2 * c, coef + 3 * c, relu, partial);
    fl::launch_colsum(partial, g, 2 * c, sums, s);
    return pdf_launch_status();
}
```

### pointcloudpdf_amd/csrc/rowlin.hip

```cpp
#include "pdfops_common.h"
#include <cstdlib>

namespace rl {

typedef float f32x16 __attribute__((ext_vector_type(16)));
constexpr int BM = 128, BN = 64, BK = 32, LDT = 33;

struct FwdArgs {
    long N;
    int K, O;
    const float *X; long ldx;
    const float *W; long wso, wsk;
    const float *bias;
    const float *scale, *shift;
    int relu;
    float *Y; long ldy;
    int accumulate;
    float *partial;
};

template <bool PRE, bool STATS>
__global__ __launch_bounds__(256) void k_rowlin(FwdArgs a) {
    __shared__ float xs[BM * LDT];
    __shared__ float ws[BN * LDT];
// ... 64 lines not shown
        }
    }
    if (STATS) {
        __syncthreads();
        if (tid < BN && o0 + tid < a.O) {
            const float s = red[0][0][tid] + red[1][0][tid] + red[2][0][tid] + red[3][0][tid];
            const float ss = red[0][1][tid] + red[1][1][tid] + red[2][1][tid] + red[3][1][tid];
            a.partial[(size_t)blockIdx.x * 2 * a.O + o0 + tid] = s;
            a.partial[(size_t)blockIdx.x * 2 * a.O + a.O + o0 + tid] = ss;
        }
    }
}

struct WArgs {
    long N;
    int K, O;
    const float *G; long ldg;
    const float *X; long ldx;
    const float *scale, *shift;
    int relu;
    float *dW;
    float *db;
    long rows_per_block;
    float *slab;
    float *bslab;
};

template <bool PRE>
__global__ __launch_bounds__(256) void k_wgrad(WArgs a) {
    const int lane = threadIdx.x & 63, wave = threadIdx.x >> 6;
    const int kblocks = (a.K + 31) / 32;
    const int o0 = (blockIdx.y / kblocks) * 32, c0 = (blockIdx.y % kblocks) * 32;
    const int ch = lane & 31, par = lane >> 5;
    const int oc = o0 + ch, cc = c0 + ch;
    const bool ov = oc < a.O, cv = cc < a.K;
    float sc = 1.f, sh = 0.f;
    if (PRE && cv) { sc = a.scale[cc]; sh = a.shift[cc]; }
    const long rb = (long)blockIdx.x * a.rows_per_block;
    const long re = min(rb + a.rows_per_block, a.N);
    f32x16 acc;
#pragma unroll
    for (int r = 0; r < 16; ++r) acc[r] = 0.f;
    float gsum = 0.f;
    for (long r0 = rb + 8 * wave; r0 < re; r0 += 32) {
        float g[4], x[4];
#pragma unroll
        for (int u = 0; u < 4; ++u) {
            const long r = r0 + 2 * u + par;
            g[u] = (r < re && ov) ? a.G[r * a.ldg + oc] : 0.f;
            float v = 0.f;
            if (r < re && cv) {
                v = a.X[r * a.ldx + cc];
                if (PRE) { v = v * sc + sh; if (a.relu) v = fmaxf(v, 0.f); }
            }
            x[u] = v;
        }
#pragma unroll
        for (int u = 0; u < 4; ++u) {
            acc = __builtin_amdgcn_mfma_f32_32x32x2f32(g[u], x[u], acc, 0, 0, 0);
            gsum += g[u];
        }
    }
    __shared__ float comb[4][1024 + 32];
#pragma unroll
    for (int r = 0; r < 16; ++r) {
        const int i = (r & 3) + 8 * (r >> 2) + 4 * (lane >> 5);
        comb[wave][i * 32 + ch] = acc[r];
    }
    gsum += __shfl_xor(gsum, 32, 64);
    if (lane < 32) comb[wave][1024 + ch] = gsum;
    __syncthreads();
    const size_t sidx = blockIdx.x, nsl = gridDim.x;
    float *slab = a.slab + ((size_t)blockIdx.y * nsl + sidx) * 1024;
#pragma unroll
    for (int e = threadIdx.x; e < 1024; e += 256) slab[e] = ((comb[0][e] + comb[1][e]) + comb[2][e]) + comb[3][e];
    if (a.db && c0 == 0 && threadIdx.x < 32)
        a.bslab[((size_t)(o0 / 32) * nsl + sidx) * 32 + threadIdx.x] =
            ((comb[0][1024 + threadIdx.x] + comb[1][1024 + threadIdx.x]) + comb[2][1024 + threadIdx.x]) + comb[3][1024 + threadIdx.x];
}

}

namespace rl2 {
int try_forward(long n, int k, int o, int nin, int nout, const float *const *x, long ldx, const float *const *w, int transpose_w,
                const float *const *bias, const float *scale, const float *shift, int relu, float *const *y, long ldy,
                int accumulate, float *partial, int mma, hipStream_t s, const float *roww = nullptr, long rws = 0, const float *bx = nullptr,
                long ldb = 0, const float *bcoef = nullptr, int brelu = 0, int *partial_rows = nullptr, long ldw = 0, void *handoff = nullptr);
long stats_rows_floats(long n, int o);
int try_wgrad(long n, int k, int o, int ng, const float *const *g, long ldg, const float *x, long ldx, const float *scale,
              const float *shift, int relu, float *const *dw, float *const *db, float *ws, int mma, hipStream_t s, const float *roww = nullptr, long rws = 0);
long wgrad_ws_floats(long n, int k, int o, int ng);
constexpr int WG_MAXG = 5;
struct RArgs {
    const float *slab, *bslab;
    float *dW[WG_MAXG], *db[WG_MAXG];
    int B, tiles_k, tiles, otiles, split, K, O;
};
int try_wgrad_group(long n, int k, int o, int ng, const float *const *g, long ldg, const float *const *x, long ldx, const float *const *scale,
                    const float *const *shift, const int *relu, float *const *dw, float *const *db, float *ws, int mma, hipStream_t s);
void launch_slab_reduce(const RArgs &a, int ng, bool any_bias, hipStream_t s);
int stats_rows(long n);
}

static inline void tiled_wg_plan(long n, int k, int o, int *blocks_oc, long *split, long *rows_per_block) {
    *blocks_oc = ((o + 31) / 32) * ((k + 31) / 32);
    long sp = (2048 + *blocks_oc - 1) / *blocks_oc;
    const long max_split = (n + 255) / 256;
    if (sp > max_split) sp = max_split;
    if (sp < 1) sp = 1;
    *rows_per_block = ((n + sp - 1) / sp + 31) / 32 * 32;
    *split = (n + *rows_per_block - 1) / *rows_per_block;
}

static inline bool rowlin_streams(int k, int o) {
    return (k == 32 || k == 64 || k == 128 || k == 256 || k == 512) && o % 16 == 0 && getenv("PDFOPS_ROWLIN_TILED") == nullptr;
}

extern "C" int pdf_rowlin_partial_rows(long n, int k, int o) {
    return rowlin_streams(k, o) ? rl2::stats_rows(n) : (int)((n + rl::BM - 1) / rl::BM);
}
extern "C" long pdf_rowlin_partial_floats(long n, int o) {
    const long a = (n + rl::BM - 1) / rl::BM * 2 * (long)o, b = rl2::stats_rows_floats(n, o);
    return (a > b ? a : b) + (long)PDF_HO_FLOATS;
}

extern "C" int pdf_rowlin_forward(long n, int k, int o, const float *x, long ldx, const float *w, int transpose_w,
                                  const float *bias, const float *scale, const float *shift, int relu, float *y, long ldy,
                                  int accumulate, float *partial, int mma_input, void *stream) {
    if (mma_input < 0 || mma_input > 2) return PDF_ERR_BAD_ARG;
    if (n < 1 || k < 1 || o < 1 || !x || !w || !y || ldx < k || ldy < o) return PDF_ERR_BAD_ARG;
    if (rowlin_streams(k, o)) {
        if (rl2::try_forward(n, k, o, 1, 1, &x, ldx, &w, transpose_w, &bias, scale, shift, relu, &y, ldy, accumulate, partial,
                             mma_input, static_cast<hipStream_t>(stream)))
            return pdf_launch_status();
        if (partial) return PDF_ERR_BAD_ARG;
    }
    if (!transpose_w && !partial && !scale && k == 1024 && rowlin_streams(512, o) && !(ldx & 3) && !(ldy & 3)) {
        const float *xs[2] = {x, x + 512}, *ws[2] = {w, w + 512};
        if (rl2::try_forward(n, 512, o, 2, 1, xs, ldx, ws, 0, &bias, nullptr, nullptr, 0, &y, ldy, accumulate, nullptr, mma_input, static_cast<hipStream_t>(stream),
                             nullptr, 0, nullptr, 0, nullptr, 0, nullptr, k))
            return pdf_launch_status();
    }
    rl::FwdArgs a;
    a.N = n; a.K = k; a.O = o; a.X = x; a.ldx = ldx; a.W = w;
    a.wso = transpose_w ? 1 : k; a.wsk = transpose_w ? o : 1;
    a.bias = bias; a.scale = scale; a.shift = shift; a.relu = relu; a.Y = y; a.ldy = ldy; a.accumulate = accumulate;
    a.partial = partial;
    const dim3 grid((unsigned)((n + rl::BM - 1) / rl::BM), (unsigned)((o + rl::BN - 1) / rl::BN));
    hipStream_t s = static_cast<hipStream_t>(stream);
    const bool pre = scale != nullptr, stats = partial != nullptr;
    if (pre && stats) rl::k_rowlin<true, true><<<grid, 256, 0, s>>>(a);
    else if (pre) rl::k_rowlin<true, false><<<grid, 256, 0, s>>>(a);
    else if (stats) rl::k_rowlin<false, true><<<grid, 256, 0, s>>>(a);
    else rl::k_rowlin<false, false><<<grid, 256, 0, s>>>(a);
    return pdf_launch_status();
}

extern "C" long pdf_rowlin_wgrad_ws_floats(long n, int k, int o, int ng) {
    if (n < 1 || k < 1 || o < 1 || ng < 1) return 0;
    int blocks_oc; long split, rpb;
    tiled_wg_plan(n, k, o, &blocks_oc, &split, &rpb);
    const long tiled = (long)blocks_oc * split * 4 * 1024 + (long)((o + 31) / 32) * split * 4 * 32;
    const long streaming = rowlin_streams(k, o) ? rl2::wgrad_ws_floats(n, k, o, ng) : 0;
    return tiled > streaming ? tiled : streaming;
}

extern "C" int pdf_bn_coef_from_partial(const float *partial, int rows, long n, int c, const float *gamma, const float *beta,
                                        float *running_mean, float *running_var, float eps, float momentum, float *coef, void *stream);

extern "C" int pdf_rowlin_forward_bn(long n, int k, int o, const float *x, long ldx, const float *w, const float *bias, const float *scale,
                                     const float *shift, int relu, float *y, long ldy, float *partial, const float *gamma, const float *beta,
                                     float *running_mean, float *running_var, float eps, float momentum, float *coef, int mma_input, void *stream) {
    if (mma_input < 0 || mma_input > 2) return PDF_ERR_BAD_ARG;
    if (n < 1 || k < 1 || o < 1 || !x || !w || !y || !partial || !gamma || !beta || !coef || ldx < k || ldy < o) return PDF_ERR_BAD_ARG;
    if (rowlin_streams(k, o)) {
        int rows = 0;
        if (rl2::try_forward(n, k, o, 1, 1, &x, ldx, &w, 0, &bias, scale, shift, relu, &y, ldy, 0, partial, mma_input, static_cast<hipStream_t>(stream),
                             nullptr, 0, nullptr, 0, nullptr, 0, &rows)) {
            return pdf_bn_coef_from_partial(partial, rows, n, o, gamma, beta, running_mean, running_var, eps, momentum, coef, stream);
        }
    }
    const int rc = pdf_rowlin_forward(n, k, o, x, ldx, w, 0, bias, scale, shift, relu, y, ldy, 0, partial, mma_input, stream);
// ... 12 lines not shown
}

extern "C" int pdf_rowlin_wgrad(long n, int k, int o, const float *g, long ldg, const float *x, long ldx,
                                const float *scale, const float *shift, int relu, float *dw, float *db, float *ws, int mma_input, void *stream) {
    if (mma_input < 0 || mma_input > 2) return PDF_ERR_BAD_ARG;
    if (n < 1 || k < 1 || o < 1 || !g || !x || !dw || !ws || ldg < o || ldx < k) return PDF_ERR_BAD_ARG;
    if (rowlin_streams(k, o) && rl2::try_wgrad(n, k, o, 1, &g, ldg, x, ldx, scale, shift, relu, &dw, &db, ws, mma_input, static_cast<hipStream_t>(stream)))
        return pdf_launch_status();
    rl::WArgs a;
    a.N = n; a.K = k; a.O = o; a.G = g; a.ldg = ldg; a.X = x; a.ldx = ldx; a.scale = scale; a.shift = shift; a.relu = relu;
    a.dW = dw; a.db = db;
    int blocks_oc; long split;
    tiled_wg_plan(n, k, o, &blocks_oc, &split, &a.rows_per_block);
    a.slab = ws;
    a.bslab = ws + (size_t)blocks_oc * split * 1024;
    const dim3 grid((unsigned)split, (unsigned)blocks_oc);
    hipStream_t s = static_cast<hipStream_t>(stream);
    if (scale) rl::k_wgrad<true><<<grid, 256, 0, s>>>(a);
    else rl::k_wgrad<false><<<grid, 256, 0, s>>>(a);
    rl2::RArgs r;
    r.slab = a.slab; r.bslab = a.bslab; r.B = 32; r.tiles_k = (k + 31) / 32; r.tiles = blocks_oc; r.otiles = (o + 31) / 32; r.split = (int)split;
    r.K = k; r.O = o;
    r.dW[0] = dw; r.db[0] = db; r.dW[1] = r.dW[2] = nullptr; r.db[1] = r.db[2] = nullptr;
    rl2::launch_slab_reduce(r, 1, db != nullptr, s);
    return pdf_launch_status();
}

extern "C" int pdf_rowlin_multi(long n, int k, int o, int nin, int nout, const float *const *x, long ldx, const float *const *w,
                                int transpose_w, const float *const *bias, const float *scale, const float *shift, int relu,
                                float *const *y, long ldy, int accumulate, int mma_input, void *stream) {
    if (mma_input < 0 || mma_input > 2) return PDF_ERR_BAD_ARG;
    if (n < 1 || k < 1 || o < 1 || !x || !w || !y || nin < 1 || nout < 1 || nin > 3 || nout > 3 || (nin > 1 && nout > 1)) return PDF_ERR_BAD_ARG;
    if (rowlin_streams(k, o) && rl2::try_forward(n, k, o, nin, nout, x, ldx, w, transpose_w, bias, scale, shift, relu, y, ldy, accumulate,
                                                 nullptr, mma_input, static_cast<hipStream_t>(stream)))
        return pdf_launch_status();
    int rc = 0;
    if (nin == 1) {
        for (int i = 0; i < nout && rc == 0; ++i)
            rc = pdf_rowlin_forward(n, k, o, x[0], ldx, w[i], transpose_w, bias ? bias[i] : nullptr, scale, shift, relu, y[i], ldy, accumulate, nullptr, mma_input, stream);
    } else {
        for (int i = 0; i < nin && rc == 0; ++i)
            rc = pdf_rowlin_forward(n, k, o, x[i], ldx, w[i], transpose_w, (i == 0 && bias) ? bias[0] : nullptr, scale, shift, relu, y[0], ldy,
                                    accumulate || i > 0, nullptr, mma_input, stream);
    }
    return rc;
}

extern "C" int pdf_rowlin_dgrad_bstats(long n, int k, int o, int nin, const float *const *x, long ldx, const float *const *w, float *y, long ldy,
                                       const float *bx, long ldb, const float *bcoef, int brelu, float *partial, int *partial_rows,
                                       int mma_input, void *stream) {
    if (mma_input < 0 || mma_input > 2) return PDF_ERR_BAD_ARG;
    if (n < 1 || k < 1 || o < 1 || !x || !w || !y || nin < 1 || nin > 3 || !bx || !bcoef || !partial || !partial_rows) return PDF_ERR_BAD_ARG;
    if (!rowlin_streams(k, o)) return PDF_ERR_UNSUPPORTED;
    float *ys[1] = {y};
    if (!rl2::try_forward(n, k, o, nin, 1, x, ldx, w, 1, nullptr, nullptr, nullptr, 0, ys, ldy, 0, partial, mma_input, static_cast<hipStream_t>(stream),
                          nullptr, 0, bx, ldb, bcoef, brelu, partial_rows))
        return PDF_ERR_UNSUPPORTED;
    return pdf_launch_status();
}

extern "C" int pdf_rowlin_wgrad_multi(long n, int k, int o, int ng, const float *const *g, long ldg, const float *x, long ldx,
                                      const float *scale, const float *shift, int relu, float *const *dw, float *const *db,
                                      float *ws, int mma_input, void *stream) {
    if (mma_input < 0 || mma_input > 2) return PDF_ERR_BAD_ARG;
    if (n < 1 || k < 1 || o < 1 || ng < 1 || ng > 3 || !g || !x || !dw || !ws) return PDF_ERR_BAD_ARG;
    if (rowlin_streams(k, o) && rl2::try_wgrad(n, k, o, ng, g, ldg, x, ldx, scale, shift, relu, dw, db, ws, mma_input, static_cast<hipStream_t>(stream)))
        return pdf_launch_status();
    int rc = 0;
    for (int i = 0; i < ng && rc == 0; ++i) rc = pdf_rowlin_wgrad(n, k, o, g[i], ldg, x, ldx, scale, shift, relu, dw[i], db ? db[i] : nullptr, ws, mma_input, stream);
    return rc;
}

extern "C" int pdf_rowlin_wgrad_group(long n, int k, int o, int ng, const float *const *g, long ldg, const float *const *x, long ldx,
                                      const float *const *scale, const float *const *shift, const int *relu, float *const *dw,
                                      float *const *db, float *ws, int mma_input, void *stream) {
    if (mma_input < 0 || mma_input > 2) return PDF_ERR_BAD_ARG;
    if (n < 1 || k < 1 || o < 1 || ng < 1 || ng > rl2::WG_MAXG || !g || !x || !scale || !shift || !relu || !dw || !ws) return PDF_ERR_BAD_ARG;
    for (int i = 0; i < ng; ++i) if (!g[i] || !x[i] || !dw[i] || (scale[i] && !shift[i])) return PDF_ERR_BAD_ARG;
    if (!rowlin_streams(k, o) || !rl2::try_wgrad_group(n, k, o, ng, g, ldg, x, ldx, scale, shift, relu, dw, db, ws, mma_input, static_cast<hipStream_t>(stream)))
        return PDF_ERR_UNSUPPORTED;
    return pdf_launch_status();
}

extern "C" int pdf_rowlin_forward_roww(long n, int k, int o, const float *x, long ldx, const float *w, int transpose_w, float *y, long ldy,
                                       int accumulate, const float *roww, long rws, int mma_input, void *stream) {
    if (mma_input < 0 || mma_input > 2) return PDF_ERR_BAD_ARG;
    if (n < 1 || !x || !w || !y || !rowlin_streams(k, o)) return PDF_ERR_UNSUPPORTED;
    const float *bias = nullptr;
    if (!rl2::try_forward(n, k, o, 1, 1, &x, ldx, &w, transpose_w, &bias, nullptr, nullptr, 0, &y, ldy, accumulate, nullptr,
                          mma_input, static_cast<hipStream_t>(stream), roww, rws))
        return PDF_ERR_UNSUPPORTED;
    return pdf_launch_status();
}
extern "C" int pdf_rowlin_wgrad_roww(long n, int k, int o, const float *g, long ldg, const float *x, long ldx, float *dw, const float *roww,
                                     long rws, float *ws, int mma_input, void *stream) {
    if (mma_input < 0 || mma_input > 2) return PDF_ERR_BAD_ARG;
    if (n < 1 || !g || !x || !dw || !ws || !rowlin_streams(k, o)) return PDF_ERR_UNSUPPORTED;
    float *db = nullptr;
    if (!rl2::try_wgrad(n, k, o, 1, &g, ldg, x, ldx, nullptr, nullptr, 0, &dw, &db, ws, mma_input, static_cast<hipStream_t>(stream), roww, rws))
        return PDF_ERR_UNSUPPORTED;
    return pdf_launch_status();
}
```

### pointcloudpdf_amd/csrc/rowlin2.hip

```cpp
#define RL2_MAIN_TU
#include "rowlin2_impl.h"

namespace rl2 {
template int try_forward_mp<0>(long, int, int, int, int, const float *const *, long, const float *const *, int, const float *const *, const float *,
                               const float *, int, float *const *, long, int, float *, hipStream_t, const float *, long, const float *, long,
                               const float *, int, int *, long, void *);
template int try_wgrad_mp<0>(long, int, int, int, const float *const *, long, const float *, long, const float *, const float *, int,
                             float *const *, float *const *, float *, hipStream_t, const float *, long);
template int try_wgrad_group_mp<0>(long, int, int, int, const float *const *, long, const float *const *, long, const float *const *, const float *const *, const int *,
                                   float *const *, float *const *, float *, hipStream_t);
extern template int try_wgrad_group_mp<1>(long, int, int, int, const float *const *, long, const float *const *, long, const float *const *, const float *const *, const int *,
                                   float *const *, float *const *, float *, hipStream_t);
extern template int try_wgrad_group_mp<2>(long, int, int, int, const float *const *, long, const float *const *, long, const float *const *, const float *const *, const int *,
                                   float *const *, float *const *, float *, hipStream_t);
extern template int try_forward_mp<1>(long, int, int, int, int, const float *const *, long, const float *const *, int, const float *const *, const float *,
                                      const float *, int, float *const *, long, int, float *, hipStream_t, const float *, long, const float *, long,
                                      const float *, int, int *, long, void *);
extern template int try_forward_mp<2>(long, int, int, int, int, const float *const *, long, const float *const *, int, const float *const *, const float *,
                                      const float *, int, float *const *, long, int, float *, hipStream_t, const float *, long, const float *, long,
                                      const float *, int, int *, long, void *);
extern template int try_wgrad_mp<1>(long, int, int, int, const float *const *, long, const float *, long, const float *, const float *, int,
                                    float *const *, float *const *, float *, hipStream_t, const float *, long);
extern template int try_wgrad_mp<2>(long, int, int, int, const float *const *, long, const float *, long, const float *, const float *, int,
                                    float *const *, float *const *, float *, hipStream_t, const float *, long);

int try_forward(long n, int k, int o, int nin, int nout, const float *const *x, long ldx, const float *const *w, int transpose_w,
                const float *const *bias, const float *scale, const float *shift, int relu, float *const *y, long ldy,
                int accumulate, float *partial, int mma, hipStream_t s, const float *roww, long rws, const float *bx, long ldb, const float *bcoef,
                int brelu, int *partial_rows, long ldw, void *handoff) {
#define RL2_FWD(MP_) try_forward_mp<MP_>(n, k, o, nin, nout, x, ldx, w, transpose_w, bias, scale, shift, relu, y, ldy, accumulate, partial, s, roww, rws, \
                                         bx, ldb, bcoef, brelu, partial_rows, ldw, handoff)
    switch (mma) {
    case 1: return RL2_FWD(1);
    case 2: return RL2_FWD(2);
    default: return RL2_FWD(0);
    }
#undef RL2_FWD
}

int try_wgrad(long n, int k, int o, int ng, const float *const *g, long ldg, const float *x, long ldx, const float *scale,
              const float *shift, int relu, float *const *dw, float *const *db, float *ws, int mma, hipStream_t s, const float *roww, long rws) {
    switch (mma) {
    case 1: return try_wgrad_mp<1>(n, k, o, ng, g, ldg, x, ldx, scale, shift, relu, dw, db, ws, s, roww, rws);
    case 2: return try_wgrad_mp<2>(n, k, o, ng, g, ldg, x, ldx, scale, shift, relu, dw, db, ws, s, roww, rws);
    default: return try_wgrad_mp<0>(n, k, o, ng, g, ldg, x, ldx, scale, shift, relu, dw, db, ws, s, roww, rws);
    }
}

int try_wgrad_group(long n, int k, int o, int ng, const float *const *g, long ldg, const float *const *x, long ldx, const float *const *scale,
                    const float *const *shift, const int *relu, float *const *dw, float *const *db, float *ws, int mma, hipStream_t s) {
    switch (mma) {
    case 1: return try_wgrad_group_mp<1>(n, k, o, ng, g, ldg, x, ldx, scale, shift, relu, dw, db, ws, s);
    case 2: return try_wgrad_group_mp<2>(n, k, o, ng, g, ldg, x, ldx, scale, shift, relu, dw, db, ws, s);
    default: return try_wgrad_group_mp<0>(n, k, o, ng, g, ldg, x, ldx, scale, shift, relu, dw, db, ws, s);
    }
}
}
```

### pointcloudpdf_amd/csrc/rowlin2_bf16.hip

```cpp
#include "rowlin2_impl.h"

namespace rl2 {
template int try_forward_mp<2>(long, int, int, int, int, const float *const *, long, const float *const *, int, const float *const *, const float *,
                               const float *, int, float *const *, long, int, float *, hipStream_t, const float *, long, const float *, long,
                               const float *, int, int *, long, void *);
template int try_wgrad_mp<2>(long, int, int, int, const float *const *, long, const float *, long, const float *, const float *, int,
                             float *const *, float *const *, float *, hipStream_t, const float *, long);
template int try_wgrad_group_mp<2>(long, int, int, int, const float *const *, long, const float *const *, long, const float *const *, const float *const *, const int *,
                                   float *const *, float *const *, float *, hipStream_t);
}
```

### pointcloudpdf_amd/csrc/rowlin2_f16.hip

```cpp
#include "rowlin2_impl.h"

namespace rl2 {
template int try_forward_mp<1>(long, int, int, int, int, const float *const *, long, const float *const *, int, const float *const *, const float *,
                               const float *, int, float *const *, long, int, float *, hipStream_t, const float *, long, const float *, long,
                               const float *, int, int *, long, void *);
template int try_wgrad_mp<1>(long, int, int, int, const float *const *, long, const float *, long, const float *, const float *, int,
                             float *const *, float *const *, float *, hipStream_t, const float *, long);
template int try_wgrad_group_mp<1>(long, int, int, int, const float *const *, long, const float *const *, long, const float *const *, const float *const *, const int *,
                                   float *const *, float *const *, float *, hipStream_t);
}
```

### pointcloudpdf_amd/csrc/rowlin2_impl.h

```cpp
#pragma once
#include "pdfops_common.h"
#include <algorithm>
#include <cstdlib>
#include <cstring>

namespace rl2 {

typedef float f32x4 __attribute__((ext_vector_type(4)));

typedef _Float16 h16x4 __attribute__((ext_vector_type(4)));
typedef __bf16 b16x4 __attribute__((ext_vector_type(4)));
typedef short s16x4 __attribute__((ext_vector_type(4)));
template <int MP> struct Mma;
template <> struct Mma<0> {
    typedef f32x4 frag;
    static __device__ __forceinline__ frag cvt(f32x4 v) { return v; }
};
template <> struct Mma<1> {
    typedef h16x4 frag;
    static __device__ __forceinline__ frag cvt(f32x4 v) { return __builtin_convertvector(v, h16x4); }
    static __device__ __forceinline__ f32x4 mma(frag a, frag b, f32x4 acc) { return __builtin_amdgcn_mfma_f32_16x16x16f16(a, b, acc, 0, 0, 0); }
};
template <> struct Mma<2> {
    typedef s16x4 frag;
    static __device__ __forceinline__ frag cvt(f32x4 v) { return __builtin_bit_cast(s16x4, __builtin_convertvector(v, b16x4)); }
    static __device__ __forceinline__ f32x4 mma(frag a, frag b, f32x4 acc) { return __builtin_amdgcn_mfma_f32_16x16x16bf16_1k(a, b, acc, 0, 0, 0); }
};

long stats_rows_floats(long n, int o);

struct FwdArgs {
    long N;
    int O;
    const float *X[3]; long ldx;
    const float *W[3]; long wso, wsk;
    const float *bias[3];
    const float *scale, *shift; int relu;
    float *Y[3]; long ldy;
    int accumulate;
    float *partial;
    const float *bx; long ldb; const float *bcoef; int brelu;
    const float *roww; long rws;
    unsigned long long *ho_gran; unsigned *ho_sync;
};

constexpr int FWD_CAP = 1024;
static inline int fwd_row_blocks(long n) {
    const long tiles = (n + 15) / 16, b = (tiles + 3) / 4;
    return (int)(b < 1 ? 1 : (b > FWD_CAP ? FWD_CAP : b));
}

template <int K, int NOB, int NIN, bool PRE, int ST, int MP>
__global__ __launch_bounds__(256) void k_fwd(FwdArgs a) {
    typedef typename Mma<MP>::frag wfrag;
    constexpr bool STATS = ST != 0;
    constexpr int NJ = K / 16;
    constexpr bool COEF_REGS = K <= 64;
    const int lane = threadIdx.x & 63, wave = threadIdx.x >> 6;
    const int li = lane & 15, kq = lane >> 4;
    if (ST == 1 && a.ho_gran && blockIdx.x == 0 && blockIdx.y == 0) pdf_handoff_zero(a.ho_gran, a.O, a.ho_sync);
    const int gcol0 = blockIdx.y * NOB * 16;
    int outi[NOB], colb[NOB];
#pragma unroll
    for (int ob = 0; ob < NOB; ++ob) { outi[ob] = (gcol0 + ob * 16) / a.O; colb[ob] = gcol0 + ob * 16 - outi[ob] * a.O; }
    wfrag Wr[NIN][NOB][NJ];
#pragma unroll
    for (int in = 0; in < NIN; ++in) {
#pragma unroll
        for (int ob = 0; ob < NOB; ++ob) {
            const float *W = a.W[NIN > 1 ? in : outi[ob]];
            const long o = colb[ob] + li;
#pragma unroll
            for (int j = 0; j < NJ; ++j) {
                f32x4 w4;
                if (a.wsk == 1) {
                    w4 = *reinterpret_cast<const f32x4 *>(W + o * a.wso + 16 * j + 4 * kq);
                } else {
#pragma unroll
                    for (int c = 0; c < 4; ++c) w4[c] = W[o * a.wso + (long)(16 * j + 4 * kq + c) * a.wsk];
                }
                Wr[in][ob][j] = Mma<MP>::cvt(w4);
            }
        }
    }
    f32x4 bias4[NOB];
#pragma unroll
    for (int ob = 0; ob < NOB; ++ob) {
        const float *b = a.bias[NIN > 1 ? 0 : outi[ob]];
#pragma unroll
        for (int r = 0; r < 4; ++r) bias4[ob][r] = b ? b[colb[ob] + 4 * kq + r] : 0.f;
    }
    f32x4 sc4[COEF_REGS && PRE ? NJ : 1], sh4[COEF_REGS && PRE ? NJ : 1];
    if (PRE && COEF_REGS) {
#pragma unroll
        for (int j = 0; j < NJ; ++j) {
            sc4[j] = *reinterpret_cast<const f32x4 *>(a.scale + 16 * j + 4 * kq);
            sh4[j] = *reinterpret_cast<const f32x4 *>(a.shift + 16 * j + 4 * kq);
        }
    }
    f32x4 s4[STATS ? NOB : 1], ss4[STATS ? NOB : 1];
    if (STATS) {
#pragma unroll
        for (int ob = 0; ob < NOB; ++ob) { s4[ob] = f32x4{0.f, 0.f, 0.f, 0.f}; ss4[ob] = f32x4{0.f, 0.f, 0.f, 0.f}; }
    }
    __shared__ float bco[ST == 2 ? 3 : 1][NOB * 16];
    if (ST == 2) {
        if (threadIdx.x < 3 * NOB * 16) {
            const int v = threadIdx.x / (NOB * 16), t = threadIdx.x % (NOB * 16);
            bco[ST == 2 ? v : 0][t] = a.bcoef[(long)v * a.O + gcol0 + t];
        }
        __syncthreads();
    }
    __shared__ float pco[PRE && !COEF_REGS ? 2 : 1][PRE && !COEF_REGS ? K : 1];
    if (PRE && !COEF_REGS) {
        for (int t = threadIdx.x; t < K; t += 256) { pco[0][t] = a.scale[t]; pco[PRE && !COEF_REGS ? 1 : 0][t] = a.shift[t]; }
        __syncthreads();
    }
    const float relu_lo = a.relu ? 0.f : -INFINITY;
    constexpr int XB0 = NJ < 16 ? NJ : 16;
    constexpr int XB = (K == 256 && NIN == 3) ? 4 : ((ST != 0 && NOB > 1 && NIN * NOB * NJ * 4 >= 128) ? ((PRE && K == 128) ? 2 : XB0 / 2) : XB0);
    const long ntiles = (a.N + 15) / 16;
    for (long tile = (long)blockIdx.x * 4 + wave; tile < ntiles; tile += (long)gridDim.x * 4) {
        const long n = tile * 16 + li;
        const bool valid = n < a.N;
        f32x4 acc[NOB];
#pragma unroll
        for (int ob = 0; ob < NOB; ++ob) acc[ob] = f32x4{0.f, 0.f, 0.f, 0.f};
#pragma unroll
        for (int in = 0; in < NIN; ++in) {
            const float *xr = a.X[in] + (valid ? n : 0) * a.ldx + 4 * kq;
#pragma unroll
            for (int j0 = 0; j0 < NJ; j0 += XB) {
                f32x4 xb[XB];
#pragma unroll
                for (int t = 0; t < XB; ++t) xb[t] = *reinterpret_cast<const f32x4 *>(xr + 16 * (j0 + t));
                __builtin_amdgcn_sched_barrier(0);
#pragma unroll
                for (int t = 0; t < XB; ++t) {
                    const int j = j0 + t;
                    f32x4 x4 = xb[t];
                    if (PRE) {
                        const f32x4 sc = COEF_REGS ? sc4[COEF_REGS ? j : 0] : *reinterpret_cast<const f32x4 *>(&pco[0][16 * j + 4 * kq]);
                        const f32x4 sh = COEF_REGS ? sh4[COEF_REGS ? j : 0] : *reinterpret_cast<const f32x4 *>(&pco[PRE && !COEF_REGS ? 1 : 0][16 * j + 4 * kq]);
                        x4 = x4 * sc + sh;
#pragma unroll
                        for (int c = 0; c < 4; ++c) x4[c] = fmaxf(x4[c], relu_lo);
                    }
                    if constexpr (MP == 0) {
#pragma unroll
                        for (int c = 0; c < 4; ++c)
#pragma unroll
                            for (int ob = 0; ob < NOB; ++ob)
                                acc[ob] = __builtin_amdgcn_mfma_f32_16x16x4f32(Wr[in][ob][j][c], x4[c], acc[ob], 0, 0, 0);
                    } else {
                        const wfrag xh = Mma<MP>::cvt(x4);
#pragma unroll
                        for (int ob = 0; ob < NOB; ++ob) acc[ob] = Mma<MP>::mma(Wr[in][ob][j], xh, acc[ob]);
                    }
                }
            }
        }
#pragma unroll
        for (int ob = 0; ob < NOB; ++ob) {
            f32x4 v = acc[ob];
            if (a.roww) v *= a.roww[(valid ? n : 0) * a.rws];
            v += bias4[ob];
            float *dst = a.Y[outi[ob]] + (valid ? n : 0) * a.ldy + colb[ob] + 4 * kq;
            if (a.accumulate && valid) v += *reinterpret_cast<const f32x4 *>(dst);
            if (valid) *reinterpret_cast<f32x4 *>(dst) = v;
            if (ST == 1 && valid) { s4[ob] += v; ss4[ob] += v * v; }
            if (ST == 2) {
                const f32x4 x4 = *reinterpret_cast<const f32x4 *>(a.bx + (valid ? n : 0) * a.ldb + colb[ob] + 4 * kq);
                const f32x4 sc = *reinterpret_cast<const f32x4 *>(&bco[0][ob * 16 + 4 * kq]);
                const f32x4 sh = *reinterpret_cast<const f32x4 *>(&bco[ST == 2 ? 1 : 0][ob * 16 + 4 * kq]);
                const f32x4 mu = *reinterpret_cast<const f32x4 *>(&bco[ST == 2 ? 2 : 0][ob * 16 + 4 * kq]);
                const f32x4 pre = x4 * sc + sh;
                f32x4 gm;
#pragma unroll
                for (int c = 0; c < 4; ++c) gm[c] = (valid && (!a.brelu || pre[c] > 0.f)) ? v[c] : 0.f;
                s4[ob] += gm;
                ss4[ob] += gm * (x4 - mu);
            }
        }
    }
    if (STATS) {
        __shared__ float red[4][2][NOB * 16];
#pragma unroll
        for (int ob = 0; ob < NOB; ++ob)
#pragma unroll
            for (int r = 0; r < 4; ++r) {
                float s = s4[ob][r], ss = ss4[ob][r];
#pragma unroll
                for (int m = 1; m < 16; m <<= 1) { s += __shfl_xor(s, m, 64); ss += __shfl_xor(ss, m, 64); }
                if (li == 0) { red[wave][0][ob * 16 + 4 * kq + r] = s; red[wave][1][ob * 16 + 4 * kq + r] = ss; }
            }
        __syncthreads();
        const int t = threadIdx.x;
        if (t < NOB * 16) {
            float *row = a.partial + (size_t)blockIdx.x * 2 * a.O;
            row[gcol0 + t] = red[0][0][t] + red[1][0][t] + red[2][0][t] + red[3][0][t];
            const float ss = red[0][1][t] + red[1][1][t] + red[2][1][t] + red[3][1][t];
            row[a.O + gcol0 + t] = ST == 2 ? ss * a.bcoef[3 * (long)a.O + gcol0 + t] : ss;
        }
    }
}

constexpr int GROUP_GN = 2;
template <int K, int GN, int NIN, int MP> constexpr int group_lds_bytes() { return NIN * GN * (K / 16) * 64 * (int)sizeof(typename Mma<MP>::frag); }

template <int K, int GN, int NIN, bool PRE, int ST, int MP>
__global__ __launch_bounds__(256, 2) void k_fwd_group(FwdArgs a) {
    typedef typename Mma<MP>::frag wfrag;
    constexpr bool STATS = ST != 0;
    constexpr int NJ = K / 16;
    static_assert(K >= 128 && NJ % 8 == 0 && (NIN == 1 || NIN == 3), "group form: K = 128 / 256 / 512, one or three inputs");
    extern __shared__ __attribute__((aligned(16))) unsigned char group_lds[];
    wfrag *Wl = reinterpret_cast<wfrag *>(group_lds);
    const int lane = threadIdx.x & 63, wave = threadIdx.x >> 6;
    const int li = lane & 15, kq = lane >> 4;
    if (ST == 1 && a.ho_gran && blockIdx.x == 0 && blockIdx.y == 0) pdf_handoff_zero(a.ho_gran, a.O, a.ho_sync);
    const int gcol0 = blockIdx.y * GN * 16;
    int outi[GN], colb[GN];
#pragma unroll
    for (int ob = 0; ob < GN; ++ob) { outi[ob] = (gcol0 + ob * 16) / a.O; colb[ob] = gcol0 + ob * 16 - outi[ob] * a.O; }
    {
        constexpr int PER_WAVE = NIN * GN * NJ / 4;
        f32x4 w4[PER_WAVE];
#pragma unroll
        for (int t = 0; t < PER_WAVE; ++t) {
            const int f = t * 4 + wave;
            const int j = f % NJ, ob = (f / NJ) % GN, in = f / (NJ * GN);
            const int col = gcol0 + ob * 16, oi = col / a.O;
            const float *W = a.W[NIN > 1 ? in : oi];
            const long o = col - oi * a.O + li;
            if (a.wsk == 1) {
                w4[t] = *reinterpret_cast<const f32x4 *>(W + o * a.wso + 16 * j + 4 * kq);
            } else {
#pragma unroll
                for (int c = 0; c < 4; ++c) w4[t][c] = W[o * a.wso + (long)(16 * j + 4 * kq + c) * a.wsk];
            }
        }
#pragma unroll
        for (int t = 0; t < PER_WAVE; ++t) Wl[(t * 4 + wave) * 64 + lane] = Mma<MP>::cvt(w4[t]);
    }
    __shared__ float bco[ST == 2 ? 3 : 1][GN * 16];
    if (ST == 2 && threadIdx.x < 3 * GN * 16) {
        const int v = threadIdx.x / (GN * 16), t = threadIdx.x % (GN * 16);
        bco[ST == 2 ? v : 0][t] = a.bcoef[(long)v * a.O + gcol0 + t];
    }
    __shared__ float pco[PRE ? 2 : 1][PRE ? K : 1];
    if (PRE)
        for (int t = threadIdx.x; t < K; t += 256) { pco[0][t] = a.scale[t]; pco[PRE ? 1 : 0][t] = a.shift[t]; }
    __syncthreads();
    f32x4 s4[STATS ? GN : 1], ss4[STATS ? GN : 1];
    if (STATS) {
#pragma unroll
        for (int ob = 0; ob < GN; ++ob) { s4[ob] = f32x4{0.f, 0.f, 0.f, 0.f}; ss4[ob] = f32x4{0.f, 0.f, 0.f, 0.f}; }
    }
    const float relu_lo = a.relu ? 0.f : -INFINITY;
    constexpr int XB = 8, NBJ = NJ / XB, NB = NIN * NBJ;
    const long ntiles = (a.N + 15) / 16;
    for (long tile = (long)blockIdx.x * 4 + wave; tile < ntiles; tile += (long)gridDim.x * 4) {
        const long n = tile * 16 + li;
        const bool valid = n < a.N;
        const long row = valid ? n : 0;
        f32x4 acc[GN];
#pragma unroll
        for (int ob = 0; ob < GN; ++ob) acc[ob] = f32x4{0.f, 0.f, 0.f, 0.f};
        f32x4 xb[2][XB];
#pragma unroll
        for (int t = 0; t < XB; ++t) xb[0][t] = *reinterpret_cast<const f32x4 *>(a.X[0] + row * a.ldx + 4 * kq + 16 * t);
#pragma unroll
        for (int b = 0; b < NB; ++b) {
            if (b + 1 < NB) {
                const float *xr = a.X[(b + 1) / NBJ] + row * a.ldx + 4 * kq + 16 * ((b + 1) % NBJ) * XB;
#pragma unroll
                for (int t = 0; t < XB; ++t) xb[(b + 1) & 1][t] = *reinterpret_cast<const f32x4 *>(xr + 16 * t);
            }
            __builtin_amdgcn_sched_barrier(0);
            const int in = b / NBJ;
#pragma unroll
            for (int t = 0; t < XB; ++t) {
                const int j = (b % NBJ) * XB + t;
                f32x4 x4 = xb[b & 1][t];
                if (PRE) {
                    const f32x4 sc = *reinterpret_cast<const f32x4 *>(&pco[0][16 * j + 4 * kq]);
                    const f32x4 sh = *reinterpret_cast<const f32x4 *>(&pco[PRE ? 1 : 0][16 * j + 4 * kq]);
                    x4 = x4 * sc + sh;
#pragma unroll
                    for (int c = 0; c < 4; ++c) x4[c] = fmaxf(x4[c], relu_lo);
                }
                wfrag wa[GN];
#pragma unroll
                for (int ob = 0; ob < GN; ++ob) wa[ob] = Wl[((in * GN + ob) * NJ + j) * 64 + lane];
                if constexpr (MP == 0) {
#pragma unroll
                    for (int c = 0; c < 4; ++c)
#pragma unroll
                        for (int ob = 0; ob < GN; ++ob)
                            acc[ob] = __builtin_amdgcn_mfma_f32_16x16x4f32(wa[ob][c], x4[c], acc[ob], 0, 0, 0);
                } else {
                    const wfrag xh = Mma<MP>::cvt(x4);
#pragma unroll
                    for (int ob = 0; ob < GN; ++ob) acc[ob] = Mma<MP>::mma(wa[ob], xh, acc[ob]);
                }
            }
        }
#pragma unroll
        for (int ob = 0; ob < GN; ++ob) {
            f32x4 v = acc[ob];
            if (a.roww) v *= a.roww[row * a.rws];
            const float *bp = a.bias[NIN > 1 ? 0 : outi[ob]];
            f32x4 bias4;
#pragma unroll
            for (int r = 0; r < 4; ++r) bias4[r] = bp ? bp[colb[ob] + 4 * kq + r] : 0.f;
            v += bias4;
            float *dst = a.Y[outi[ob]] + row * a.ldy + colb[ob] + 4 * kq;
            if (a.accumulate && valid) v += *reinterpret_cast<const f32x4 *>(dst);
            if (valid) *reinterpret_cast<f32x4 *>(dst) = v;
            if (ST == 1 && valid) { s4[ob] += v; ss4[ob] += v * v; }
            if (ST == 2) {
                const f32x4 x4 = *reinterpret_cast<const f32x4 *>(a.bx + row * a.ldb + colb[ob] + 4 * kq);
                const f32x4 sc = *reinterpret_cast<const f32x4 *>(&bco[0][ob * 16 + 4 * kq]);
                const f32x4 sh = *reinterpret_cast<const f32x4 *>(&bco[ST == 2 ? 1 : 0][ob * 16 + 4 * kq]);
                const f32x4 mu = *reinterpret_cast<const f32x4 *>(&bco[ST == 2 ? 2 : 0][ob * 16 + 4 * kq]);
                const f32x4 pre = x4 * sc + sh;
                f32x4 gm;
#pragma unroll
                for (int c = 0; c < 4; ++c) gm[c] = (valid && (!a.brelu || pre[c] > 0.f)) ? v[c] : 0.f;
                s4[ob] += gm;
                ss4[ob] += gm * (x4 - mu);
            }
        }
    }
    if (STATS) {
        __shared__ float red[4][2][GN * 16];
#pragma unroll
        for (int ob = 0; ob < GN; ++ob)
#pragma unroll
            for (int r = 0; r < 4; ++r) {
                float s = s4[ob][r], ss = ss4[ob][r];
#pragma unroll
                for (int m = 1; m < 16; m <<= 1) { s += __shfl_xor(s, m, 64); ss += __shfl_xor(ss, m, 64); }
                if (li == 0) { red[wave][0][ob * 16 + 4 * kq + r] = s; red[wave][1][ob * 16 + 4 * kq + r] = ss; }
            }
        __syncthreads();
        const int t = threadIdx.x;
        if (t < GN * 16) {
            float *prow = a.partial + (size_t)blockIdx.x * 2 * a.O;
            prow[gcol0 + t] = red[0][0][t] + red[1][0][t] + red[2][0][t] + red[3][0][t];
            const float ss = red[0][1][t] + red[1][1][t] + red[2][1][t] + red[3][1][t];
            prow[a.O + gcol0 + t] = ST == 2 ? ss * a.bcoef[3 * (long)a.O + gcol0 + t] : ss;
        }
    }
}

constexpr int WG_MAXG = 5;
struct WArgs {
    long N;
    int K, O;
    const float *G[WG_MAXG]; long ldg;
    const float *X; long ldx;
    const float *scale, *shift; int relu;
    int per_z; const float *Xz[WG_MAXG]; const float *scalez[WG_MAXG], *shiftz[WG_MAXG]; int reluz[WG_MAXG];
    float *dW[WG_MAXG], *db[WG_MAXG];
    long rows_per_block;
    const float *roww; long rws;
    float *slab;
    float *bslab;
};

template <int VW> struct Vec;
template <> struct Vec<2> { typedef float type __attribute__((ext_vector_type(2))); };
template <> struct Vec<4> { typedef float type __attribute__((ext_vector_type(4))); };

template <int VW, bool PRE, bool RW, int MP>
__global__ __launch_bounds__(256) void k_wg(WArgs a) {
    typedef typename Vec<VW>::type vec;
    constexpr int B = 16 * VW;
    __shared__ float red[4][B * B];
    __shared__ float redb[4][B];
    const int lane = threadIdx.x & 63, wave = threadIdx.x >> 6;
    const int li = lane & 15, nq = lane >> 4;
    const int nkb = a.K / B;
    const int ob = (blockIdx.y / nkb) * B, kb = (blockIdx.y % nkb) * B;
    const float *G = a.G[blockIdx.z];
    const float *X = (PRE && a.per_z) ? a.Xz[blockIdx.z] : a.X;
    vec sc, sh;
    bool relu = a.relu != 0;
    if (PRE) {
        const float *scp = a.per_z ? a.scalez[blockIdx.z] : a.scale, *shp = a.per_z ? a.shiftz[blockIdx.z] : a.shift;
        if (a.per_z) relu = scp != nullptr && a.reluz[blockIdx.z] != 0;
        if (scp) {
            sc = *reinterpret_cast<const vec *>(scp + kb + VW * li);
            sh = *reinterpret_cast<const vec *>(shp + kb + VW * li);
        } else {
#pragma unroll
            for (int c = 0; c < VW; ++c) { sc[c] = 1.f; sh[c] = 0.f; }
        }
    }
    const float relu_lo = relu ? 0.f : -INFINITY;
    f32x4 acc[VW][VW];
    float gsum[VW];
#pragma unroll
    for (int c = 0; c < VW; ++c) {
        gsum[c] = 0.f;
#pragma unroll
        for (int c2 = 0; c2 < VW; ++c2) acc[c][c2] = f32x4{0.f, 0.f, 0.f, 0.f};
    }
    const long rb = (long)blockIdx.x * a.rows_per_block;
    const long re = rb + a.rows_per_block < a.N ? rb + a.rows_per_block : a.N;
    for (long r0 = rb + 16 * wave; r0 < re; r0 += 64) {
        vec gv[4], xv[4];
        float rw[RW ? 4 : 1];
        bool ok[4];
#pragma unroll
        for (int t = 0; t < 4; ++t) {
            const long n = r0 + 4 * t + nq;
            ok[t] = n < re;
            const long nn = ok[t] ? n : rb;
            gv[t] = *reinterpret_cast<const vec *>(G + nn * a.ldg + ob + VW * li);
            xv[t] = *reinterpret_cast<const vec *>(X + nn * a.ldx + kb + VW * li);
            if (RW) rw[RW ? t : 0] = a.roww[nn * a.rws];
        }
        __builtin_amdgcn_sched_barrier(0);
#pragma unroll
        for (int t = 0; t < 4; ++t) {
            if (RW) gv[t] *= rw[RW ? t : 0];
            if (PRE) {
                xv[t] = xv[t] * sc + sh;
#pragma unroll
                for (int c = 0; c < VW; ++c) xv[t][c] = fmaxf(xv[t][c], relu_lo);
            }
#pragma unroll
            for (int c = 0; c < VW; ++c) { gv[t][c] = ok[t] ? gv[t][c] : 0.f; xv[t][c] = ok[t] ? xv[t][c] : 0.f; }
        }
        if constexpr (MP == 0) {
#pragma unroll
            for (int t = 0; t < 4; ++t)
#pragma unroll
                for (int c = 0; c < VW; ++c) {
                    gsum[c] += gv[t][c];
#pragma unroll
                    for (int c2 = 0; c2 < VW; ++c2)
                        acc[c][c2] = __builtin_amdgcn_mfma_f32_16x16x4f32(gv[t][c], xv[t][c2], acc[c][c2], 0, 0, 0);
                }
        } else {
            typename Mma<MP>::frag ga[VW], xa[VW];
#pragma unroll
            for (int c = 0; c < VW; ++c) {
                gsum[c] += (gv[0][c] + gv[1][c]) + (gv[2][c] + gv[3][c]);
                ga[c] = Mma<MP>::cvt(f32x4{gv[0][c], gv[1][c], gv[2][c], gv[3][c]});
                xa[c] = Mma<MP>::cvt(f32x4{xv[0][c], xv[1][c], xv[2][c], xv[3][c]});
            }
#pragma unroll
            for (int c = 0; c < VW; ++c)
#pragma unroll
                for (int c2 = 0; c2 < VW; ++c2) acc[c][c2] = Mma<MP>::mma(ga[c], xa[c2], acc[c][c2]);
        }
    }
#pragma unroll
    for (int c = 0; c < VW; ++c)
#pragma unroll
        for (int c2 = 0; c2 < VW; ++c2)
#pragma unroll
            for (int r = 0; r < 4; ++r) red[wave][(VW * (4 * nq + r) + c) * B + VW * li + c2] = acc[c][c2][r];
    float *db = a.db[blockIdx.z];
    const bool want_db = db && kb == 0;
    if (want_db) {
#pragma unroll
        for (int c = 0; c < VW; ++c) {
            float g = gsum[c];
            g += __shfl_xor(g, 16, 64);
            g += __shfl_xor(g, 32, 64);
            if (nq == 0) redb[wave][VW * li + c] = g;
        }
    }
    __syncthreads();
    float *slab = a.slab + (((size_t)blockIdx.z * gridDim.y + blockIdx.y) * gridDim.x + blockIdx.x) * (B * B);
    for (int e = threadIdx.x; e < B * B; e += 256) slab[e] = (red[0][e] + red[1][e]) + (red[2][e] + red[3][e]);
    if (want_db && threadIdx.x < B)
        a.bslab[(((size_t)blockIdx.z * (a.O / B) + ob / B) * gridDim.x + blockIdx.x) * B + threadIdx.x] =
            (redb[0][threadIdx.x] + redb[1][threadIdx.x]) + (redb[2][threadIdx.x] + redb[3][threadIdx.x]);
}

struct RArgs {
    const float *slab, *bslab;
    float *dW[WG_MAXG], *db[WG_MAXG];
    int B, tiles_k, tiles, otiles, split, K, O;
};
void launch_slab_reduce(const RArgs &a, int ng, bool any_bias, hipStream_t s);
template <int L>
__global__ __launch_bounds__(64 * L) void k_slab_reduce(RArgs a) {
    __shared__ float red[L][64];
    const int e = threadIdx.x & 63, l = threadIdx.x >> 6, z = blockIdx.z;
    const int ei = blockIdx.x * 64 + e;
    const bool bias = (int)blockIdx.y >= a.tiles;
    const int t = bias ? (int)blockIdx.y - a.tiles : (int)blockIdx.y;
    const int len = bias ? a.B : a.B * a.B;
    if (bias && (int)blockIdx.x * 64 >= len) return;
    const float *src = bias ? a.bslab + ((size_t)z * a.otiles + t) * a.split * a.B : a.slab + ((size_t)z * a.tiles + t) * a.split * (size_t)(a.B * a.B);
    float s = 0.f;
    if (ei < len) {
        int k = l;
        for (; k + 3 * L < a.split; k += 4 * L) {
            const float v0 = src[(size_t)k * len + ei], v1 = src[(size_t)(k + L) * len + ei];
            const float v2 = src[(size_t)(k + 2 * L) * len + ei], v3 = src[(size_t)(k + 3 * L) * len + ei];
            s = (((s + v0) + v1) + v2) + v3;
        }
        for (; k < a.split; k += L) s += src[(size_t)k * len + ei];
    }
    red[l][e] = s;
    __syncthreads();
    if (l != 0 || ei >= len) return;
#pragma unroll
    for (int k = 1; k < L; ++k) s += red[k][e];
    if (bias) {
        const int o = t * a.B + ei;
        if (a.db[z] && o < a.O) a.db[z][o] = s;
    } else {
        const int o = (t / a.tiles_k) * a.B + ei / a.B, kk = (t % a.tiles_k) * a.B + ei % a.B;
        if (o < a.O && kk < a.K) a.dW[z][(size_t)o * a.K + kk] = s;
    }
}

#ifdef RL2_MAIN_TU
void launch_slab_reduce(const RArgs &a, int ng, bool any_bias, hipStream_t s) {
    const dim3 grid((unsigned)((a.B * a.B + 63) / 64), (unsigned)(a.tiles + (any_bias ? a.otiles : 0)), (unsigned)ng);
    if (a.split > 32) k_slab_reduce<16><<<grid, 64 * 16, 0, s>>>(a);
    else if (a.split > 4) k_slab_reduce<4><<<grid, 64 * 4, 0, s>>>(a);
    else k_slab_reduce<1><<<grid, 64, 0, s>>>(a);
}
#endif

struct WgPlan { int vw, b, nblk; long split, rows_per_block; };
static WgPlan wg_plan(long n, int k, int o, int ng) {
    WgPlan p;
    p.vw = (k % 64 == 0 && o % 64 == 0) ? 4 : ((k % 32 == 0 && o % 32 == 0) ? 2 : 0);
    p.b = 16 * p.vw;
    if (!p.vw) { p.nblk = 0; p.split = 0; p.rows_per_block = 0; return p; }
    p.nblk = (o / p.b) * (k / p.b) * ng;
    static const int target = [] { const char *v = getenv("PDFOPS_WG_BLOCKS"); const int x = v ? atoi(v) : 0; return x > 0 ? x : 512; }();
    long split = (target + p.nblk - 1) / p.nblk;
    const long max_split = (n + 255) / 256;
    if (split > max_split) split = max_split;
    if (split < 1) split = 1;
    p.rows_per_block = ((n + split - 1) / split + 63) / 64 * 64;
    p.split = (n + p.rows_per_block - 1) / p.rows_per_block;
    return p;
}
#ifdef RL2_MAIN_TU
long wgrad_ws_floats(long n, int k, int o, int ng) {
    const WgPlan p = wg_plan(n, k, o, ng);
    if (!p.vw) return 0;
    return (long)p.nblk * p.split * p.b * p.b + (long)ng * (o / p.b) * p.split * p.b;
}
#endif

static inline bool aligned16(const void *p) { return (reinterpret_cast<uintptr_t>(p) & 15) == 0; }

constexpr long GROUP_MAX_ROWS = 16384;
static bool group_form_wanted(const FwdArgs &a, int k, int blocks) {
    if (blocks % GROUP_GN) return false;
    if (const char *f = getenv("PDFOPS_RL_FORM")) {
        if (!strcmp(f, "slab")) return false;
        if (!strcmp(f, "group")) return true;
    }
    return a.N <= GROUP_MAX_ROWS && !(k == 128 && blocks * 16 > a.O);
}

template <int K, int GN, int NIN, bool PRE, int ST, int MP>
static bool launch_group_kernel(const FwdArgs &a, dim3 grid, hipStream_t s) {
    constexpr int lds = group_lds_bytes<K, GN, NIN, MP>();
    static PdfLdsLimit site;
    if (!pdf_lds_limit_raised(site, reinterpret_cast<const void *>(&k_fwd_group<K, GN, NIN, PRE, ST, MP>), lds)) return false;
    k_fwd_group<K, GN, NIN, PRE, ST, MP><<<grid, 256, lds, s>>>(a);
    return true;
}

template <int K, int GN, int NIN, int MP>
static bool launch_fwd_group(const FwdArgs &a, int blocks, int gx, hipStream_t s) {
    const bool pre = a.scale != nullptr, stats = a.partial != nullptr, bst = stats && a.bx != nullptr;
    const dim3 grid((unsigned)gx, (unsigned)(blocks / GN));
    if (bst) return launch_group_kernel<K, GN, NIN, false, 2, MP>(a, grid, s);
    if constexpr (NIN == 1) {
        if (stats) return pre ? launch_group_kernel<K, GN, 1, true, 1, MP>(a, grid, s) : launch_group_kernel<K, GN, 1, false, 1, MP>(a, grid, s);
    }
    return pre ? launch_group_kernel<K, GN, NIN, true, 0, MP>(a, grid, s) : launch_group_kernel<K, GN, NIN, false, 0, MP>(a, grid, s);
}

template <int K, int NOB, int NIN, int MP>
static int launch_fwd(const FwdArgs &a, int nslabs, hipStream_t s) {
    const bool pre = a.scale != nullptr, stats = a.partial != nullptr, bst = stats && a.bx != nullptr;
    static const int total = [] { const char *v = getenv("PDFOPS_RL_BLOCKS"); const int x = v ? atoi(v) : 0; return x > 0 ? x : 512; }();
    int gx = fwd_row_blocks(a.N);
    if (!stats || bst) gx = std::max(1, std::min(gx, std::max(8, total / std::max(nslabs, 1))));
    if constexpr (K >= 128 && NIN != 2) {
        if (group_form_wanted(a, K, nslabs * NOB) && launch_fwd_group<K, GROUP_GN, NIN, MP>(a, nslabs * NOB, gx, s)) return gx;
    }
    const dim3 grid((unsigned)gx, (unsigned)nslabs);
    if (bst) {
        k_fwd<K, NOB, NIN, false, 2, MP><<<grid, 256, 0, s>>>(a);
    } else if (NIN == 1 && stats) {
        if (pre) k_fwd<K, NOB, 1, true, 1, MP><<<grid, 256, 0, s>>>(a);
        else k_fwd<K, NOB, 1, false, 1, MP><<<grid, 256, 0, s>>>(a);
    } else {
        if (pre) k_fwd<K, NOB, NIN, true, 0, MP><<<grid, 256, 0, s>>>(a);
        else k_fwd<K, NOB, NIN, false, 0, MP><<<grid, 256, 0, s>>>(a);
    }
    return gx;
}

#ifdef RL2_MAIN_TU
long stats_rows_floats(long n, int o) { return (long)fwd_row_blocks(n) * 2 * o; }
#endif

template <int MP>
int try_forward_mp(long n, int k, int o, int nin, int nout, const float *const *x, long ldx, const float *const *w, int transpose_w,
                   const float *const *bias, const float *scale, const float *shift, int relu, float *const *y, long ldy,
                   int accumulate, float *partial, hipStream_t s, const float *roww, long rws, const float *bx, long ldb, const float *bcoef,
                   int brelu, int *partial_rows, long ldw, void *handoff) {
    if (nin < 1 || nout < 1 || (nin > 1 && nout > 1) || nin > 3 || nout > 3) return 0;
    if (nin == 2 && (scale || bx)) return 0;
    if (partial && !bx && (nin != 1 || nout != 1)) return 0;
    if (bx && (!partial || nout != 1 || scale || !bcoef || (ldb & 3) || !aligned16(bx) || !aligned16(bcoef))) return 0;
    if ((ldx & 3) || (ldy & 3) || (o & 15)) return 0;
    for (int i = 0; i < (nin > 1 ? nin : nout); ++i) if (!aligned16(w[i])) return 0;
    if (scale && (!aligned16(scale) || !aligned16(shift))) return 0;
    for (int i = 0; i < nin; ++i) if (!aligned16(x[i])) return 0;
    for (int i = 0; i < nout; ++i) if (!aligned16(y[i])) return 0;
    FwdArgs a;
    a.N = n; a.O = o; a.ldx = ldx; a.ldy = ldy; a.scale = scale; a.shift = shift; a.relu = relu; a.accumulate = accumulate;
    a.partial = partial; a.roww = roww; a.rws = rws;
    a.bx = bx; a.ldb = ldb; a.bcoef = bcoef; a.brelu = brelu;
    a.ho_gran = static_cast<unsigned long long *>(handoff);
    a.ho_sync = handoff ? reinterpret_cast<unsigned *>(a.ho_gran + 2 * (size_t)o) : nullptr;
    a.wso = transpose_w ? 1 : (ldw ? ldw : k); a.wsk = transpose_w ? o : 1;
    for (int i = 0; i < 3; ++i) {
        a.X[i] = i < nin ? x[i] : nullptr;
        a.W[i] = i < (nin > 1 ? nin : nout) ? w[i] : nullptr;
        a.bias[i] = (bias && i < nout) ? bias[i] : nullptr;
        a.Y[i] = i < nout ? y[i] : nullptr;
    }
    const int cols = o * nout;
#define PDF_RL2(K_, NOB_, NIN_) do { if (cols % (NOB_ * 16) == 0) { \
        const int r_ = launch_fwd<K_, NOB_, NIN_, MP>(a, cols / (NOB_ * 16), s); \
        if (partial_rows) *partial_rows = r_; \
        return 1; } } while (0)
    if (nin == 1) {
        switch (k) {
        case 32: if (!partial) PDF_RL2(32, 6, 1); PDF_RL2(32, 2, 1); PDF_RL2(32, 1, 1); break;
        case 64: PDF_RL2(64, 4, 1); PDF_RL2(64, 1, 1); break;
        case 128: if (!bx) PDF_RL2(128, 4, 1); else PDF_RL2(128, 2, 1); PDF_RL2(128, 1, 1); break;
        case 256: PDF_RL2(256, 2, 1); PDF_RL2(256, 1, 1); break;
        case 512: PDF_RL2(512, 1, 1); break;
        default: break;
        }
    } else if (nin == 2) {
        if (k == 512) PDF_RL2(512, 1, 2);
    } else if (nin == 3) {
        switch (k) {
        case 32: PDF_RL2(32, 2, 3); break;
        case 64: PDF_RL2(64, 2, 3); break;
        case 128: PDF_RL2(128, 1, 3); break;
        case 256: PDF_RL2(256, 1, 3); break;
        default: break;
        }
    }
#undef PDF_RL2
    return 0;
}

template <int MP>
int try_wgrad_mp(long n, int k, int o, int ng, const float *const *g, long ldg, const float *x, long ldx, const float *scale,
                 const float *shift, int relu, float *const *dw, float *const *db, float *ws, hipStream_t s, const float *roww, long rws) {
    if (ng < 1 || ng > 3 || !ws) return 0;
    const WgPlan p = wg_plan(n, k, o, ng);
    const int vw = p.vw;
    if (!vw) return 0;
    if ((ldg % vw) || (ldx % vw) || !aligned16(x)) return 0;
    if (scale && (!aligned16(scale) || !aligned16(shift))) return 0;
    for (int i = 0; i < ng; ++i) if (!aligned16(g[i])) return 0;
    WArgs a;
    a.N = n; a.K = k; a.O = o; a.ldg = ldg; a.X = x; a.ldx = ldx; a.scale = scale; a.shift = shift; a.relu = relu; a.roww = roww; a.rws = rws;
    a.per_z = 0;
    bool any_bias = false;
    for (int i = 0; i < WG_MAXG; ++i) {
        a.G[i] = i < ng ? g[i] : nullptr; a.dW[i] = i < ng ? dw[i] : nullptr; a.db[i] = (db && i < ng) ? db[i] : nullptr;
        a.Xz[i] = nullptr; a.scalez[i] = a.shiftz[i] = nullptr; a.reluz[i] = 0;
        any_bias = any_bias || a.db[i] != nullptr;
    }
    const int b = p.b;
    a.rows_per_block = p.rows_per_block;
    a.slab = ws;
    a.bslab = ws + (size_t)p.nblk * p.split * b * b;
    const dim3 grid((unsigned)p.split, (unsigned)((o / b) * (k / b)), (unsigned)ng);
#define PDF_WG(VW_) do { \
        if (roww) { if (scale) k_wg<VW_, true, true, MP><<<grid, 256, 0, s>>>(a); else k_wg<VW_, false, true, MP><<<grid, 256, 0, s>>>(a); } \
        else      { if (scale) k_wg<VW_, true, false, MP><<<grid, 256, 0, s>>>(a); else k_wg<VW_, false, false, MP><<<grid, 256, 0, s>>>(a); } } while (0)
    if (vw == 4) PDF_WG(4); else PDF_WG(2);
#undef PDF_WG
    RArgs r;
    r.slab = a.slab; r.bslab = a.bslab; r.B = b; r.tiles_k = k / b; r.tiles = (o / b) * (k / b); r.otiles = o / b; r.split = (int)p.split; r.K = k; r.O = o;
    for (int i = 0; i < WG_MAXG; ++i) { r.dW[i] = a.dW[i]; r.db[i] = a.db[i]; }
    launch_slab_reduce(r, ng, any_bias, s);
    return 1;
}

template <int MP>
int try_wgrad_group_mp(long n, int k, int o, int ng, const float *const *g, long ldg, const float *const *x, long ldx,
                       const float *const *scale, const float *const *shift, const int *relu, float *const *dw, float *const *db,
                       float *ws, hipStream_t s) {
    if (ng < 1 || ng > WG_MAXG || !ws) return 0;
    const WgPlan p = wg_plan(n, k, o, ng);
    const int vw = p.vw;
    if (!vw) return 0;
    if ((ldg % vw) || (ldx % vw)) return 0;
    for (int i = 0; i < ng; ++i) {
        if (!aligned16(g[i]) || !aligned16(x[i])) return 0;
        if (scale[i] && (!aligned16(scale[i]) || !aligned16(shift[i]))) return 0;
    }
    WArgs a;
    a.N = n; a.K = k; a.O = o; a.ldg = ldg; a.X = nullptr; a.ldx = ldx; a.scale = a.shift = nullptr; a.relu = 0; a.roww = nullptr; a.rws = 0;
    a.per_z = 1;
    bool any_bias = false;
    for (int i = 0; i < WG_MAXG; ++i) {
        const bool on = i < ng;
        a.G[i] = on ? g[i] : nullptr; a.Xz[i] = on ? x[i] : nullptr;
        a.scalez[i] = on ? scale[i] : nullptr; a.shiftz[i] = on ? shift[i] : nullptr; a.reluz[i] = on ? relu[i] : 0;
        a.dW[i] = on ? dw[i] : nullptr; a.db[i] = (on && db) ? db[i] : nullptr;
        any_bias = any_bias || a.db[i] != nullptr;
    }
    const int b = p.b;
    a.rows_per_block = p.rows_per_block;
    a.slab = ws;
    a.bslab = ws + (size_t)p.nblk * p.split * b * b;
    const dim3 grid((unsigned)p.split, (unsigned)((o / b) * (k / b)), (unsigned)ng);
    if (vw == 4) k_wg<4, true, false, MP><<<grid, 256, 0, s>>>(a); else k_wg<2, true, false, MP><<<grid, 256, 0, s>>>(a);
    RArgs r;
    r.slab = a.slab; r.bslab = a.bslab; r.B = b; r.tiles_k = k / b; r.tiles = (o / b) * (k / b); r.otiles = o / b; r.split = (int)p.split; r.K = k; r.O = o;
    for (int i = 0; i < WG_MAXG; ++i) { r.dW[i] = a.dW[i]; r.db[i] = a.db[i]; }
    launch_slab_reduce(r, ng, any_bias, s);
    return 1;
}

#ifdef RL2_MAIN_TU
int stats_rows(long n) { return fwd_row_blocks(n); }
#endif

}
```

Measured before the change: 13.75 million.

## Fold batchnorm-backward elementwise into dgrad and wgrad GEMM input loads

Adds a grad-pre path in which the BN+ReLU backward value is computed inside the rowlin forward (dgrad) and weight-gradient kernels as they load the upstream gradient. This replaces a separate materialised pass that wrote the BN input gradient. It is enabled automatically at two sites, the block pre-backward and linbn backward, when the sizes are large, and can be overridden with PDFOPS_BN_FOLD. The cost is that the BN value is recomputed in both the dgrad and wgrad kernels, with extra z loads and more template instantiations. The BN backward arithmetic is moved into a shared helper with fp contraction turned off so the numerics match the unfused path.

```diff
diff --git a/include/pdfops.h b/include/pdfops.h
--- a/include/pdfops.h
+++ b/include/pdfops.h
@@ -10,7 +10,7 @@
 #define PDF_ERR_NSAMPLE (-2)
 #define PDF_ERR_UNSUPPORTED (-3)
 
-#define PDF_ABI_VERSION 17
+#define PDF_ABI_VERSION 18
 int pdf_abi_version(void);
 const char *pdf_build_info(void);
 int pdf_dist_fma_mode(void);
@@ -164,6 +164,16 @@
                           float *running_mean, float *running_var, float eps, float momentum, float *coef, int mma_input, void *stream);
 int pdf_bn_act_backward_presummed(long n, int c, const float *gy, const float *x, const float *coef, int training, int relu,
                                   const float *partial, int partial_rows, float *sums, float *gx, void *stream);
+int pdf_rowlin_forward_bnfold(long n, int k, int o, const float *g, long ldg, const float *z, long ldz, const float *coef, const float *sums,
+                              int relu, const float *w, int transpose_w, float *y, long ldy, int accumulate, int mma_input, void *stream);
+int pdf_rowlin_wgrad_bnfold(long n, int k, int o, const float *g, long ldg, const float *z, long ldz, const float *coef, const float *sums,
+                            int relu, const float *x, long ldx, float *dw, float *db, float *ws, int mma_input, void *stream);
+int pdf_bn_bwd_sums_presummed(int c, const float *partial, int partial_rows, float *sums, void *stream);
+int pdf_rowlin_wgrad_group_bnfold(long n, int k, int o, int ng, const float *const *g, long ldg, const float *const *x, long ldx,
+                                  const float *const *scale, const float *const *shift, const int *relu, float *const *dw, float *const *db,
+                                  float *ws, int fold_index, const float *z, long ldz, const float *coef, const float *sums, int fold_relu,
+                                  int mma_input, void *stream);
+int pdf_bn_fold_wanted(int site, long n, int k, int o);
 
 int pdf_bn_coef_eval_or_partial(const float *partial, int rows, long n, int c, const float *gamma, const float *beta,
                                 float *running_mean, float *running_var, int training, float eps, float momentum,
diff --git a/pointcloudpdf_amd/_native.py b/pointcloudpdf_amd/_native.py
--- a/pointcloudpdf_amd/_native.py
+++ b/pointcloudpdf_amd/_native.py
@@ -15,7 +15,7 @@
 
 
 LIB_PATH = library_path(DIST_FMA)
-ABI_VERSION = 17
+ABI_VERSION = 18
 
 c_int = ctypes.c_int
 c_long = ctypes.c_long
@@ -752,6 +752,19 @@
         lib.pdf_bn_act_backward_presummed.restype = c_int
         lib.pdf_bn_act_backward_presummed.argtypes = [c_long, c_int, c_void_p, c_void_p, c_void_p, c_int, c_int, c_void_p, c_int, c_void_p,
                                                       c_void_p, c_void_p]
+        lib.pdf_rowlin_forward_bnfold.restype = c_int
+        lib.pdf_rowlin_forward_bnfold.argtypes = [c_long, c_int, c_int, c_void_p, c_long, c_void_p, c_long, c_void_p, c_void_p, c_int, c_void_p, c_int,
+                                                  c_void_p, c_long, c_int, c_int, c_void_p]
+        lib.pdf_rowlin_wgrad_bnfold.restype = c_int
+        lib.pdf_rowlin_wgrad_bnfold.argtypes = [c_long, c_int, c_int, c_void_p, c_long, c_void_p, c_long, c_void_p, c_void_p, c_int, c_void_p, c_long,
+                                                c_void_p, c_void_p, c_void_p, c_int, c_void_p]
+        lib.pdf_bn_bwd_sums_presummed.restype = c_int
+        lib.pdf_bn_bwd_sums_presummed.argtypes = [c_int, c_void_p, c_int, c_void_p, c_void_p]
+        lib.pdf_bn_fold_wanted.restype = c_int
+        lib.pdf_bn_fold_wanted.argtypes = [c_int, c_long, c_int, c_int]
+        lib.pdf_rowlin_wgrad_group_bnfold.restype = c_int
+        lib.pdf_rowlin_wgrad_group_bnfold.argtypes = [c_long, c_int, c_int, c_int, c_void_p, c_long, c_void_p, c_long, c_void_p, c_void_p, c_void_p, c_void_p,
+                                                      c_void_p, c_void_p, c_int, c_void_p, c_long, c_void_p, c_void_p, c_int, c_int, c_void_p]
         lib.pdf_rowlin_partial_floats.restype = c_long
         lib.pdf_rowlin_partial_floats.argtypes = [c_long, c_int]
         lib.pdf_rowlin_partial_rows.restype = c_int
diff --git a/pointcloudpdf_amd/csrc/block.hip b/pointcloudpdf_amd/csrc/block.hip
--- a/pointcloudpdf_amd/csrc/block.hip
+++ b/pointcloudpdf_amd/csrc/block.hip
@@ -44,7 +44,21 @@
     return on;
 }
 
-static int block_pre_backward(long n, int c, void *const *p, int training, int accumulate_gx, int mma_input, void *stream, bool defer_wgrad = false) {
+enum { BN_FOLD_SITE_A = 0, BN_FOLD_SITE_B = 1 };
+static bool bn_fold_auto(int site, long n, int k, int o) {
+    if (site == BN_FOLD_SITE_A) return o == 32 && n >= 100000;
+    return k <= 64 && o <= 64 && n >= 25000;
+}
+extern "C" int pdf_bn_fold_wanted(int site, long n, int k, int o) {
+    if (const char *v = getenv("PDFOPS_BN_FOLD")) {
+        if (v[0] == '0') return 0;
+        if (v[0] == '1') return 1;
+    }
+    return bn_fold_auto(site, n, k, o) ? 1 : 0;
+}
+
+static int block_pre_backward(long n, int c, void *const *p, int training, int accumulate_gx, int mma_input, void *stream, bool defer_wgrad = false,
+                              bool *folded = nullptr) {
     if (n < 1 || !p || !p[14]) return PDF_ERR_BAD_ARG;
     const float *x = (const float *)p[0], *z1 = (const float *)p[1], *coef1 = (const float *)p[2], *W1 = (const float *)p[3];
     float *gx = (float *)p[10], *grads = (float *)p[11], *dy = (float *)p[12], *partial = (float *)p[13], *wslab = (float *)p[14];
@@ -63,6 +77,14 @@
         e << pdf_bn_act_backward(n, c, dy, z1, nullptr, coef1, training, 1, partial, db1, dy, nullptr, stream);
     } else {
         e << rc1;
+        if (defer_wgrad && folded && training && rc1 == PDF_OK && pdf_bn_fold_wanted(BN_FOLD_SITE_A, n, c, c) && pdf_rowlin_gp_forward_supported(c, c) &&
+            pdf_rowlin_gp_wgrad_supported(c, c)) {
+            e << pdf_bn_bwd_sums_presummed(c, partial, prow, db1, stream);
+            const PdfGradPre gp = {z1, c, coef1, db1, (float)(1.0 / (double)n), 1};
+            e << pdf_rowlin_forward_gp(n, c, c, dy, c, &gp, W1, 1, gx, c, accumulate_gx, mma_input, stream);
+            *folded = true;
+            return e.rc;
+        }
         e << pdf_bn_act_backward_presummed(n, c, dy, z1, coef1, training, 1, partial, prow, db1, dy, stream);
     }
     if (!defer_wgrad) e << pdf_rowlin_wgrad(n, c, c, dy, c, x, c, nullptr, nullptr, 0, dW1, nullptr, wslab, mma_input, stream);
@@ -175,7 +197,8 @@
                                (float *)p[41], (float *)p[42], (const int *)p[43], (const int *)p[44], entry_base,
                                (float *)p[40], (float *)p[32], storage_bf16, (const int *)p[49], (const double *)p[46], stream);
     void *pre[15] = {p[1], p[2], p[3], p[4], p[5], p[6], p[7], p[35], p[36], p[37], p[29], p[30], p[45], p[40], ws_pre};
-    e << block_pre_backward(n, c, pre, training, 1, mma_input, stream, group);
+    bool folded = false;
+    e << block_pre_backward(n, c, pre, training, 1, mma_input, stream, group, &folded);
     if (group && e.rc == 0) {
         const long cc = (long)c * c;
         float *gpre = (float *)p[30], *gpost = (float *)p[31];
@@ -187,6 +210,9 @@
         const int relu[5] = {1, 1, 1, 1, 0};
         float *dw[5] = {dW3, dqkv, dqkv + (cc + c), dqkv + 2 * (cc + c), dW1};
         float *db[5] = {nullptr, dqkv + cc, dqkv + (cc + c) + cc, dqkv + 2 * (cc + c) + cc, nullptr};
+        const PdfGradPre gp1 = {(const float *)p[2], c, coef1, gpre + cc, (float)(1.0 / (double)n), 1};
+        const PdfGradPre *gps[5] = {nullptr, nullptr, nullptr, nullptr, &gp1};
+        if (folded) return pdf_rowlin_wgrad_group_gp(n, c, c, 5, g, c, x, c, sc, sh, relu, dw, db, ws_post, gps, mma_input, stream);
         const int rc = pdf_rowlin_wgrad_group(n, c, c, 5, g, c, x, c, sc, sh, relu, dw, db, ws_post, mma_input, stream);
         if (rc == PDF_ERR_UNSUPPORTED) {
             e << pdf_rowlin_wgrad(n, c, c, g[0], c, x[0], c, sc[0], sh[0], 1, dw[0], nullptr, ws_post, mma_input, stream);
@@ -220,6 +246,16 @@
     float *grads = (float *)p[6], *gz = (float *)p[7];
     const long ok = (long)o * k;
     Err e;
+    if (training && pdf_bn_supported(o) && pdf_bn_fold_wanted(BN_FOLD_SITE_B, n, k, o) && pdf_rowlin_gp_wgrad_supported(k, o) &&
+        (!p[5] || pdf_rowlin_gp_forward_supported(o, k))) {
+        const float *gy = (const float *)p[0], *z = (const float *)p[2], *coef = (const float *)p[3];
+        float *sums = grads + ok + o;
+        e << pdf_bn_bwd_sums(n, o, gy, z, coef, relu, (float *)p[8], sums, stream);
+        const PdfGradPre gp = {z, o, coef, sums, (float)(1.0 / (double)n), relu};
+        if (p[5]) e << pdf_rowlin_forward_gp(n, o, k, gy, o, &gp, (const float *)p[4], 1, (float *)p[5], k, 0, mma_input, stream);
+        e << pdf_rowlin_wgrad_gp(n, k, o, gy, o, &gp, (const float *)p[1], k, grads, grads + ok, (float *)p[9], mma_input, stream);
+        return e.rc;
+    }
     e << pdf_bn_act_backward(n, o, (const float *)p[0], (const float *)p[2], nullptr, (const float *)p[3], training, relu, (float *)p[8],
                              grads + ok + o, gz, nullptr, stream);
     if (p[5]) e << pdf_rowlin_forward(n, o, k, gz, o, (const float *)p[4], 1, nullptr, nullptr, nullptr, 0, (float *)p[5], k, 0, nullptr, mma_input, stream);
diff --git a/pointcloudpdf_amd/csrc/bn_bwd_value.h b/pointcloudpdf_amd/csrc/bn_bwd_value.h
--- /dev/null
+++ b/pointcloudpdf_amd/csrc/bn_bwd_value.h
@@ -0,0 +1,18 @@
+#pragma once
+
+__device__ __forceinline__ float pdf_bn_pre(float z, float scale, float shift) { return __builtin_fmaf(z, scale, shift); }
+
+__device__ __forceinline__ float pdf_bn_bwd_value(float gm, float z, float scale, float mean, float rstd, float s1, float s2, float inv_n) {
+#pragma clang fp contract(off)
+    const float xh = (z - mean) * rstd;
+    const float t = xh * s2;
+    const float a = __builtin_fmaf(-s1, inv_n, gm);
+    const float b = __builtin_fmaf(-t, inv_n, a);
+    return scale * b;
+}
+
+__device__ __forceinline__ float pdf_bn_bwd_fold(float g, float z, float scale, float shift, float mean, float rstd, float s1, float s2,
+                                                 float inv_n, bool relu) {
+    const float gm = (!relu || pdf_bn_pre(z, scale, shift) > 0.f) ? g : 0.f;
+    return pdf_bn_bwd_value(gm, z, scale, mean, rstd, s1, s2, inv_n);
+}
diff --git a/pointcloudpdf_amd/csrc/pdfops_common.h b/pointcloudpdf_amd/csrc/pdfops_common.h
--- a/pointcloudpdf_amd/csrc/pdfops_common.h
+++ b/pointcloudpdf_amd/csrc/pdfops_common.h
@@ -115,6 +115,22 @@
 int pdf_bn_apply_rows(long n, int c, const float *x, const float *res, const float *rows, int nrows, const float *gamma, const float *beta,
                       float *running_mean, float *running_var, float eps, float momentum, float *coef, void *handoff, int relu, float *y,
                       void *stream);
+
+struct PdfGradPre {
+    const float *z; long ldz;
+    const float *coef;
+    const float *sums;
+    float inv_n; int relu;
+};
+bool pdf_rowlin_gp_forward_supported(int k, int o);
+bool pdf_rowlin_gp_wgrad_supported(int k, int o);
+int pdf_rowlin_forward_gp(long n, int k, int o, const float *g, long ldg, const PdfGradPre *gp, const float *w, int transpose_w, float *y, long ldy,
+                          int accumulate, int mma_input, void *stream);
+int pdf_rowlin_wgrad_gp(long n, int k, int o, const float *g, long ldg, const PdfGradPre *gp, const float *x, long ldx, float *dw, float *db,
+                        float *ws, int mma_input, void *stream);
+int pdf_rowlin_wgrad_group_gp(long n, int k, int o, int ng, const float *const *g, long ldg, const float *const *x, long ldx,
+                              const float *const *scale, const float *const *shift, const int *relu, float *const *dw, float *const *db,
+                              float *ws, const PdfGradPre *const *gp, int mma_input, void *stream);
 
 __device__ __forceinline__ void pdf_handoff_zero(unsigned long long *gran, int c, unsigned *sync) {
     for (int e = threadIdx.x; e < 2 * c; e += blockDim.x) gran[e] = 0ull;
diff --git a/pointcloudpdf_amd/csrc/pointwise.hip b/pointcloudpdf_amd/csrc/pointwise.hip
--- a/pointcloudpdf_amd/csrc/pointwise.hip
+++ b/pointcloudpdf_amd/csrc/pointwise.hip
@@ -1,4 +1,5 @@
 #include "pdfops_common.h"
+#include "bn_bwd_value.h"
 #include <cstdlib>
 
 namespace pw {
@@ -131,10 +132,9 @@
         float4 gm, o;
 #define PW_ONE(f)                                                                     \
         {                                                                             \
-            const float pre = x4.f * sc.f + sh.f + r4.f;                              \
+            const float pre = RES ? pdf_bn_pre(x4.f, sc.f, sh.f) + r4.f : pdf_bn_pre(x4.f, sc.f, sh.f); \
             gm.f = (!relu || pre > 0.f) ? g4.f : 0.f;                                 \
-            const float xh = (x4.f - mu.f) * rs.f;                                    \
-            o.f = sc.f * (gm.f - s1.f * inv_n - xh * s2.f * inv_n);                   \
+            o.f = pdf_bn_bwd_value(gm.f, x4.f, sc.f, mu.f, rs.f, s1.f, s2.f, inv_n);  \
         }
         PW_ONE(x) PW_ONE(y) PW_ONE(z) PW_ONE(w)
 #undef PW_ONE
@@ -296,6 +296,13 @@
     return pdf_launch_status();
 }
 
+extern "C" int pdf_bn_bwd_sums_presummed(int c, const float *partial, int partial_rows, float *sums, void *stream) {
+    if (!partial || partial_rows < 1 || !sums) return PDF_ERR_BAD_ARG;
+    if (!pdf_bn_supported(c)) return PDF_ERR_UNSUPPORTED;
+    fl::launch_colsum(partial, partial_rows, 2 * c, sums, static_cast<hipStream_t>(stream));
+    return pdf_launch_status();
+}
+
 extern "C" int pdf_bn_bwd_sums(long n, int c, const float *gy, const float *x, const float *coef, int relu, float *partial, float *sums,
                                void *stream) {
     if (n < 1 || !gy || !x || !coef || !partial || !sums) return PDF_ERR_BAD_ARG;
diff --git a/pointcloudpdf_amd/csrc/rowlin.hip b/pointcloudpdf_amd/csrc/rowlin.hip
--- a/pointcloudpdf_amd/csrc/rowlin.hip
+++ b/pointcloudpdf_amd/csrc/rowlin.hip
@@ -170,13 +170,16 @@
 }
 
 namespace rl2 {
+typedef PdfGradPre GradPre;
 int try_forward(long n, int k, int o, int nin, int nout, const float *const *x, long ldx, const float *const *w, int transpose_w,
                 const float *const *bias, const float *scale, const float *shift, int relu, float *const *y, long ldy,
                 int accumulate, float *partial, int mma, hipStream_t s, const float *roww = nullptr, long rws = 0, const float *bx = nullptr,
-                long ldb = 0, const float *bcoef = nullptr, int brelu = 0, int *partial_rows = nullptr, long ldw = 0, void *handoff = nullptr);
+                long ldb = 0, const float *bcoef = nullptr, int brelu = 0, int *partial_rows = nullptr, long ldw = 0, void *handoff = nullptr,
+                const GradPre *gp = nullptr);
 long stats_rows_floats(long n, int o);
 int try_wgrad(long n, int k, int o, int ng, const float *const *g, long ldg, const float *x, long ldx, const float *scale,
-              const float *shift, int relu, float *const *dw, float *const *db, float *ws, int mma, hipStream_t s, const float *roww = nullptr, long rws = 0);
+              const float *shift, int relu, float *const *dw, float *const *db, float *ws, int mma, hipStream_t s, const float *roww = nullptr, long rws = 0,
+              const GradPre *gp = nullptr);
 long wgrad_ws_floats(long n, int k, int o, int ng);
 constexpr int WG_MAXG = 5;
 struct RArgs {
@@ -185,7 +188,8 @@
     int B, tiles_k, tiles, otiles, split, K, O;
 };
 int try_wgrad_group(long n, int k, int o, int ng, const float *const *g, long ldg, const float *const *x, long ldx, const float *const *scale,
-                    const float *const *shift, const int *relu, float *const *dw, float *const *db, float *ws, int mma, hipStream_t s);
+                    const float *const *shift, const int *relu, float *const *dw, float *const *db, float *ws, int mma, hipStream_t s,
+                    const GradPre *const *gp = nullptr);
 void launch_slab_reduce(const RArgs &a, int ng, bool any_bias, hipStream_t s);
 int stats_rows(long n);
 }
@@ -364,6 +368,64 @@
     return pdf_launch_status();
 }
 
+bool pdf_rowlin_gp_forward_supported(int k, int o) { return rowlin_streams(k, o); }
+bool pdf_rowlin_gp_wgrad_supported(int k, int o) { return rowlin_streams(k, o) && k % 32 == 0 && o % 32 == 0; }
+
+int pdf_rowlin_forward_gp(long n, int k, int o, const float *g, long ldg, const PdfGradPre *gp, const float *w, int transpose_w, float *y, long ldy,
+                          int accumulate, int mma_input, void *stream) {
+    if (mma_input < 0 || mma_input > 2) return PDF_ERR_BAD_ARG;
+    if (n < 1 || k < 1 || o < 1 || !g || !gp || !w || !y || ldg < k || ldy < o || gp->ldz < k) return PDF_ERR_BAD_ARG;
+    const float *bias = nullptr;
+    if (!rowlin_streams(k, o) || !rl2::try_forward(n, k, o, 1, 1, &g, ldg, &w, transpose_w, &bias, nullptr, nullptr, 0, &y, ldy, accumulate, nullptr, mma_input,
+                                                   static_cast<hipStream_t>(stream), nullptr, 0, nullptr, 0, nullptr, 0, nullptr, 0, nullptr, gp))
+        return PDF_ERR_UNSUPPORTED;
+    return pdf_launch_status();
+}
+int pdf_rowlin_wgrad_gp(long n, int k, int o, const float *g, long ldg, const PdfGradPre *gp, const float *x, long ldx, float *dw, float *db,
+                        float *ws, int mma_input, void *stream) {
+    if (mma_input < 0 || mma_input > 2) return PDF_ERR_BAD_ARG;
+    if (n < 1 || k < 1 || o < 1 || !g || !gp || !x || !dw || !ws || ldg < o || ldx < k || gp->ldz < o) return PDF_ERR_BAD_ARG;
+    if (!pdf_rowlin_gp_wgrad_supported(k, o) ||
+        !rl2::try_wgrad(n, k, o, 1, &g, ldg, x, ldx, nullptr, nullptr, 0, &dw, &db, ws, mma_input, static_cast<hipStream_t>(stream), nullptr, 0, gp))
+        return PDF_ERR_UNSUPPORTED;
+    return pdf_launch_status();
+}
+int pdf_rowlin_wgrad_group_gp(long n, int k, int o, int ng, const float *const *g, long ldg, const float *const *x, long ldx,
+                              const float *const *scale, const float *const *shift, const int *relu, float *const *dw, float *const *db,
+                              float *ws, const PdfGradPre *const *gp, int mma_input, void *stream) {
+    if (mma_input < 0 || mma_input > 2) return PDF_ERR_BAD_ARG;
+    if (n < 1 || k < 1 || o < 1 || ng < 1 || ng > rl2::WG_MAXG || !g || !x || !scale || !shift || !relu || !dw || !ws || !gp) return PDF_ERR_BAD_ARG;
+    for (int i = 0; i < ng; ++i) if (!g[i] || !x[i] || !dw[i] || (scale[i] && !shift[i])) return PDF_ERR_BAD_ARG;
+    if (!pdf_rowlin_gp_wgrad_supported(k, o) ||
+        !rl2::try_wgrad_group(n, k, o, ng, g, ldg, x, ldx, scale, shift, relu, dw, db, ws, mma_input, static_cast<hipStream_t>(stream), gp))
+        return PDF_ERR_UNSUPPORTED;
+    return pdf_launch_status();
+}
+
+extern "C" int pdf_rowlin_forward_bnfold(long n, int k, int o, const float *g, long ldg, const float *z, long ldz, const float *coef, const float *sums,
+                                         int relu, const float *w, int transpose_w, float *y, long ldy, int accumulate, int mma_input, void *stream) {
+    if (n < 1) return PDF_ERR_BAD_ARG;
+    const PdfGradPre gp = {z, ldz, coef, sums, (float)(1.0 / (double)n), relu};
+    return pdf_rowlin_forward_gp(n, k, o, g, ldg, &gp, w, transpose_w, y, ldy, accumulate, mma_input, stream);
+}
+extern "C" int pdf_rowlin_wgrad_bnfold(long n, int k, int o, const float *g, long ldg, const float *z, long ldz, const float *coef, const float *sums,
+                                       int relu, const float *x, long ldx, float *dw, float *db, float *ws, int mma_input, void *stream) {
+    if (n < 1) return PDF_ERR_BAD_ARG;
+    const PdfGradPre gp = {z, ldz, coef, sums, (float)(1.0 / (double)n), relu};
+    return pdf_rowlin_wgrad_gp(n, k, o, g, ldg, &gp, x, ldx, dw, db, ws, mma_input, stream);
+}
+
+extern "C" int pdf_rowlin_wgrad_group_bnfold(long n, int k, int o, int ng, const float *const *g, long ldg, const float *const *x, long ldx,
+                                             const float *const *scale, const float *const *shift, const int *relu, float *const *dw,
+                                             float *const *db, float *ws, int fold_index, const float *z, long ldz, const float *coef,
+                                             const float *sums, int fold_relu, int mma_input, void *stream) {
+    if (n < 1 || ng < 1 || ng > rl2::WG_MAXG || fold_index < 0 || fold_index >= ng) return PDF_ERR_BAD_ARG;
+    const PdfGradPre gp = {z, ldz, coef, sums, (float)(1.0 / (double)n), fold_relu};
+    const PdfGradPre *gps[rl2::WG_MAXG] = {nullptr, nullptr, nullptr, nullptr, nullptr};
+    gps[fold_index] = &gp;
+    return pdf_rowlin_wgrad_group_gp(n, k, o, ng, g, ldg, x, ldx, scale, shift, relu, dw, db, ws, gps, mma_input, stream);
+}
+
 extern "C" int pdf_rowlin_forward_roww(long n, int k, int o, const float *x, long ldx, const float *w, int transpose_w, float *y, long ldy,
                                        int accumulate, const float *roww, long rws, int mma_input, void *stream) {
     if (mma_input < 0 || mma_input > 2) return PDF_ERR_BAD_ARG;
diff --git a/pointcloudpdf_amd/csrc/rowlin2.hip b/pointcloudpdf_amd/csrc/rowlin2.hip
--- a/pointcloudpdf_amd/csrc/rowlin2.hip
+++ b/pointcloudpdf_amd/csrc/rowlin2.hip
@@ -4,32 +4,32 @@
 namespace rl2 {
 template int try_forward_mp<0>(long, int, int, int, int, const float *const *, long, const float *const *, int, const float *const *, const float *,
                                const float *, int, float *const *, long, int, float *, hipStream_t, const float *, long, const float *, long,
-                               const float *, int, int *, long, void *);
+                               const float *, int, int *, long, void *, const GradPre *);
 template int try_wgrad_mp<0>(long, int, int, int, const float *const *, long, const float *, long, const float *, const float *, int,
-                             float *const *, float *const *, float *, hipStream_t, const float *, long);
+                             float *const *, float *const *, float *, hipStream_t, const float *, long, const GradPre *);
 template int try_wgrad_group_mp<0>(long, int, int, int, const float *const *, long, const float *const *, long, const float *const *, const float *const *, const int *,
-                                   float *const *, float *const *, float *, hipStream_t);
+                                   float *const *, float *const *, float *, hipStream_t, const GradPre *const *);
 extern template int try_wgrad_group_mp<1>(long, int, int, int, const float *const *, long, const float *const *, long, const float *const *, const float *const *, const int *,
-                                   float *const *, float *const *, float *, hipStream_t);
+                                   float *const *, float *const *, float *, hipStream_t, const GradPre *const *);
 extern template int try_wgrad_group_mp<2>(long, int, int, int, const float *const *, long, const float *const *, long, const float *const *, const float *const *, const int *,
-                                   float *const *, float *const *, float *, hipStream_t);
+                                   float *const *, float *const *, float *, hipStream_t, const GradPre *const *);
 extern template int try_forward_mp<1>(long, int, int, int, int, const float *const *, long, const float *const *, int, const float *const *, const float *,
                                       const float *, int, float *const *, long, int, float *, hipStream_t, const float *, long, const float *, long,
-                                      const float *, int, int *, long, void *);
+                                      const float *, int, int *, long, void *, const GradPre *);
 extern template int try_forward_mp<2>(long, int, int, int, int, const float *const *, long, const float *const *, int, const float *const *, const float *,
                                       const float *, int, float *const *, long, int, float *, hipStream_t, const float *, long, const float *, long,
-                                      const float *, int, int *, long, void *);
+                                      const float *, int, int *, long, void *, const GradPre *);
 extern template int try_wgrad_mp<1>(long, int, int, int, const float *const *, long, const float *, long, const float *, const float *, int,
-                                    float *const *, float *const *, float *, hipStream_t, const float *, long);
+                                    float *const *, float *const *, float *, hipStream_t, const float *, long, const GradPre *);
 extern template int try_wgrad_mp<2>(long, int, int, int, const float *const *, long, const float *, long, const float *, const float *, int,
-                                    float *const *, float *const *, float *, hipStream_t, const float *, long);
+                                    float *const *, float *const *, float *, hipStream_t, const float *, long, const GradPre *);
 
 int try_forward(long n, int k, int o, int nin, int nout, const float *const *x, long ldx, const float *const *w, int transpose_w,
                 const float *const *bias, const float *scale, const float *shift, int relu, float *const *y, long ldy,
                 int accumulate, float *partial, int mma, hipStream_t s, const float *roww, long rws, const float *bx, long ldb, const float *bcoef,
-                int brelu, int *partial_rows, long ldw, void *handoff) {
+                int brelu, int *partial_rows, long ldw, void *handoff, const GradPre *gp) {
 #define RL2_FWD(MP_) try_forward_mp<MP_>(n, k, o, nin, nout, x, ldx, w, transpose_w, bias, scale, shift, relu, y, ldy, accumulate, partial, s, roww, rws, \
-                                         bx, ldb, bcoef, brelu, partial_rows, ldw, handoff)
+                                         bx, ldb, bcoef, brelu, partial_rows, ldw, handoff, gp)
     switch (mma) {
     case 1: return RL2_FWD(1);
     case 2: return RL2_FWD(2);
@@ -39,20 +39,20 @@
 }
 
 int try_wgrad(long n, int k, int o, int ng, const float *const *g, long ldg, const float *x, long ldx, const float *scale,
-              const float *shift, int relu, float *const *dw, float *const *db, float *ws, int mma, hipStream_t s, const float *roww, long rws) {
+              const float *shift, int relu, float *const *dw, float *const *db, float *ws, int mma, hipStream_t s, const float *roww, long rws, const GradPre *gp) {
     switch (mma) {
-    case 1: return try_wgrad_mp<1>(n, k, o, ng, g, ldg, x, ldx, scale, shift, relu, dw, db, ws, s, roww, rws);
-    case 2: return try_wgrad_mp<2>(n, k, o, ng, g, ldg, x, ldx, scale, shift, relu, dw, db, ws, s, roww, rws);
-    default: return try_wgrad_mp<0>(n, k, o, ng, g, ldg, x, ldx, scale, shift, relu, dw, db, ws, s, roww, rws);
+    case 1: return try_wgrad_mp<1>(n, k, o, ng, g, ldg, x, ldx, scale, shift, relu, dw, db, ws, s, roww, rws, gp);
+    case 2: return try_wgrad_mp<2>(n, k, o, ng, g, ldg, x, ldx, scale, shift, relu, dw, db, ws, s, roww, rws, gp);
+    default: return try_wgrad_mp<0>(n, k, o, ng, g, ldg, x, ldx, scale, shift, relu, dw, db, ws, s, roww, rws, gp);
     }
 }
 
 int try_wgrad_group(long n, int k, int o, int ng, const float *const *g, long ldg, const float *const *x, long ldx, const float *const *scale,
-                    const float *const *shift, const int *relu, float *const *dw, float *const *db, float *ws, int mma, hipStream_t s) {
+                    const float *const *shift, const int *relu, float *const *dw, float *const *db, float *ws, int mma, hipStream_t s, const GradPre *const *gp) {
     switch (mma) {
-    case 1: return try_wgrad_group_mp<1>(n, k, o, ng, g, ldg, x, ldx, scale, shift, relu, dw, db, ws, s);
-    case 2: return try_wgrad_group_mp<2>(n, k, o, ng, g, ldg, x, ldx, scale, shift, relu, dw, db, ws, s);
-    default: return try_wgrad_group_mp<0>(n, k, o, ng, g, ldg, x, ldx, scale, shift, relu, dw, db, ws, s);
+    case 1: return try_wgrad_group_mp<1>(n, k, o, ng, g, ldg, x, ldx, scale, shift, relu, dw, db, ws, s, gp);
+    case 2: return try_wgrad_group_mp<2>(n, k, o, ng, g, ldg, x, ldx, scale, shift, relu, dw, db, ws, s, gp);
+    default: return try_wgrad_group_mp<0>(n, k, o, ng, g, ldg, x, ldx, scale, shift, relu, dw, db, ws, s, gp);
     }
 }
 }
diff --git a/pointcloudpdf_amd/csrc/rowlin2_bf16.hip b/pointcloudpdf_amd/csrc/rowlin2_bf16.hip
--- a/pointcloudpdf_amd/csrc/rowlin2_bf16.hip
+++ b/pointcloudpdf_amd/csrc/rowlin2_bf16.hip
@@ -3,9 +3,9 @@
 namespace rl2 {
 template int try_forward_mp<2>(long, int, int, int, int, const float *const *, long, const float *const *, int, const float *const *, const float *,
                                const float *, int, float *const *, long, int, float *, hipStream_t, const float *, long, const float *, long,
-                               const float *, int, int *, long, void *);
+                               const float *, int, int *, long, void *, const GradPre *);
 template int try_wgrad_mp<2>(long, int, int, int, const float *const *, long, const float *, long, const float *, const float *, int,
-                             float *const *, float *const *, float *, hipStream_t, const float *, long);
+                             float *const *, float *const *, float *, hipStream_t, const float *, long, const GradPre *);
 template int try_wgrad_group_mp<2>(long, int, int, int, const float *const *, long, const float *const *, long, const float *const *, const float *const *, const int *,
-                                   float *const *, float *const *, float *, hipStream_t);
+                                   float *const *, float *const *, float *, hipStream_t, const GradPre *const *);
 }
diff --git a/pointcloudpdf_amd/csrc/rowlin2_f16.hip b/pointcloudpdf_amd/csrc/rowlin2_f16.hip
--- a/pointcloudpdf_amd/csrc/rowlin2_f16.hip
+++ b/pointcloudpdf_amd/csrc/rowlin2_f16.hip
@@ -3,9 +3,9 @@
 namespace rl2 {
 template int try_forward_mp<1>(long, int, int, int, int, const float *const *, long, const float *const *, int, const float *const *, const float *,
                                const float *, int, float *const *, long, int, float *, hipStream_t, const float *, long, const float *, long,
-                               const float *, int, int *, long, void *);
+                               const float *, int, int *, long, void *, const GradPre *);
 template int try_wgrad_mp<1>(long, int, int, int, const float *const *, long, const float *, long, const float *, const float *, int,
-                             float *const *, float *const *, float *, hipStream_t, const float *, long);
+                             float *const *, float *const *, float *, hipStream_t, const float *, long, const GradPre *);
 template int try_wgrad_group_mp<1>(long, int, int, int, const float *const *, long, const float *const *, long, const float *const *, const float *const *, const int *,
-                                   float *const *, float *const *, float *, hipStream_t);
+                                   float *const *, float *const *, float *, hipStream_t, const GradPre *const *);
 }
diff --git a/pointcloudpdf_amd/csrc/rowlin2_impl.h b/pointcloudpdf_amd/csrc/rowlin2_impl.h
--- a/pointcloudpdf_amd/csrc/rowlin2_impl.h
+++ b/pointcloudpdf_amd/csrc/rowlin2_impl.h
@@ -1,8 +1,10 @@
 #pragma once
 #include "pdfops_common.h"
+#include "bn_bwd_value.h"
 #include <algorithm>
 #include <cstdlib>
 #include <cstring>
+#include <type_traits>
 
 namespace rl2 {
 
@@ -29,6 +31,19 @@
 
 long stats_rows_floats(long n, int o);
 
+typedef PdfGradPre GradPre;
+static inline bool aligned16(const void *p) { return (reinterpret_cast<uintptr_t>(p) & 15) == 0; }
+static inline bool grad_pre_ok(const GradPre &g, int width) {
+    return g.z && g.coef && g.sums && !(g.ldz & 3) && !(width & 3) && aligned16(g.z) && aligned16(g.coef) && aligned16(g.sums);
+}
+template <typename V, int NV>
+__device__ __forceinline__ V grad_pre_vec(V g, V z, V sc, V sh, V mu, V rs, V s1, V s2, float inv_n, bool relu) {
+    V r;
+#pragma unroll
+    for (int c = 0; c < NV; ++c) r[c] = pdf_bn_bwd_fold(g[c], z[c], sc[c], sh[c], mu[c], rs[c], s1[c], s2[c], inv_n, relu);
+    return r;
+}
+
 struct FwdArgs {
     long N;
     int O;
@@ -42,6 +57,7 @@
     const float *bx; long ldb; const float *bcoef; int brelu;
     const float *roww; long rws;
     unsigned long long *ho_gran; unsigned *ho_sync;
+    GradPre gp;
 };
 
 constexpr int FWD_CAP = 1024;
@@ -50,8 +66,9 @@
     return (int)(b < 1 ? 1 : (b > FWD_CAP ? FWD_CAP : b));
 }
 
-template <int K, int NOB, int NIN, bool PRE, int ST, int MP>
+template <int K, int NOB, int NIN, int PRE, int ST, int MP>
 __global__ __launch_bounds__(256) void k_fwd(FwdArgs a) {
+    static_assert(PRE != 2 || (NIN == 1 && ST == 0), "gradient prologue: one input, no statistics");
     typedef typename Mma<MP>::frag wfrag;
     constexpr bool STATS = ST != 0;
     constexpr int NJ = K / 16;
@@ -90,8 +107,8 @@
 #pragma unroll
         for (int r = 0; r < 4; ++r) bias4[ob][r] = b ? b[colb[ob] + 4 * kq + r] : 0.f;
     }
-    f32x4 sc4[COEF_REGS && PRE ? NJ : 1], sh4[COEF_REGS && PRE ? NJ : 1];
-    if (PRE && COEF_REGS) {
+    f32x4 sc4[COEF_REGS && PRE == 1 ? NJ : 1], sh4[COEF_REGS && PRE == 1 ? NJ : 1];
+    if (PRE == 1 && COEF_REGS) {
 #pragma unroll
         for (int j = 0; j < NJ; ++j) {
             sc4[j] = *reinterpret_cast<const f32x4 *>(a.scale + 16 * j + 4 * kq);
@@ -111,14 +128,32 @@
         }
         __syncthreads();
     }
-    __shared__ float pco[PRE && !COEF_REGS ? 2 : 1][PRE && !COEF_REGS ? K : 1];
-    if (PRE && !COEF_REGS) {
-        for (int t = threadIdx.x; t < K; t += 256) { pco[0][t] = a.scale[t]; pco[PRE && !COEF_REGS ? 1 : 0][t] = a.shift[t]; }
+    __shared__ float pco[PRE == 1 && !COEF_REGS ? 2 : 1][PRE == 1 && !COEF_REGS ? K : 1];
+    if (PRE == 1 && !COEF_REGS) {
+        for (int t = threadIdx.x; t < K; t += 256) { pco[0][t] = a.scale[t]; pco[PRE == 1 && !COEF_REGS ? 1 : 0][t] = a.shift[t]; }
         __syncthreads();
     }
+    constexpr bool GREG = PRE == 2 && COEF_REGS, GLDS = PRE == 2 && !COEF_REGS;
+    f32x4 gc4[GREG ? 6 : 1][GREG ? NJ : 1];
+    __shared__ __attribute__((aligned(16))) float gco[GLDS ? 6 : 1][GLDS ? K : 1];
+    if constexpr (GREG) {
+#pragma unroll
+        for (int v = 0; v < 6; ++v)
+#pragma unroll
+            for (int j = 0; j < NJ; ++j)
+                gc4[v][j] = *reinterpret_cast<const f32x4 *>((v < 4 ? a.gp.coef + (long)v * K : a.gp.sums + (long)(v - 4) * K) + 16 * j + 4 * kq);
+    }
+    if constexpr (GLDS) {
+        for (int t = threadIdx.x; t < 6 * K; t += 256) {
+            const int v = t / K, e = t % K;
+            gco[v][e] = v < 4 ? a.gp.coef[(long)v * K + e] : a.gp.sums[(long)(v - 4) * K + e];
+        }
+        __syncthreads();
+    }
+    const bool grelu = a.gp.relu != 0;
     const float relu_lo = a.relu ? 0.f : -INFINITY;
     constexpr int XB0 = NJ < 16 ? NJ : 16;
-    constexpr int XB = (K == 256 && NIN == 3) ? 4 : ((ST != 0 && NOB > 1 && NIN * NOB * NJ * 4 >= 128) ? ((PRE && K == 128) ? 2 : XB0 / 2) : XB0);
+    constexpr int XB = (K == 256 && NIN == 3) ? 4 : ((ST != 0 && NOB > 1 && NIN * NOB * NJ * 4 >= 128) ? ((PRE && K == 128) ? 2 : XB0 / 2) : ((PRE == 2 && K >= 256) ? XB0 / 2 : XB0));
     const long ntiles = (a.N + 15) / 16;
     for (long tile = (long)blockIdx.x * 4 + wave; tile < ntiles; tile += (long)gridDim.x * 4) {
         const long n = tile * 16 + li;
@@ -129,19 +164,33 @@
 #pragma unroll
         for (int in = 0; in < NIN; ++in) {
             const float *xr = a.X[in] + (valid ? n : 0) * a.ldx + 4 * kq;
+            const float *zr = PRE == 2 ? a.gp.z + (valid ? n : 0) * a.gp.ldz + 4 * kq : nullptr;
 #pragma unroll
             for (int j0 = 0; j0 < NJ; j0 += XB) {
-                f32x4 xb[XB];
+                f32x4 xb[XB], zb[PRE == 2 ? XB : 1];
 #pragma unroll
                 for (int t = 0; t < XB; ++t) xb[t] = *reinterpret_cast<const f32x4 *>(xr + 16 * (j0 + t));
+                if constexpr (PRE == 2) {
+#pragma unroll
+                    for (int t = 0; t < XB; ++t) zb[t] = *reinterpret_cast<const f32x4 *>(zr + 16 * (j0 + t));
+                }
                 __builtin_amdgcn_sched_barrier(0);
 #pragma unroll
                 for (int t = 0; t < XB; ++t) {
                     const int j = j0 + t;
                     f32x4 x4 = xb[t];
-                    if (PRE) {
+                    if constexpr (PRE == 2) {
+                        f32x4 co[6];
+#pragma unroll
+                        for (int v = 0; v < 6; ++v) {
+                            if constexpr (GREG) co[v] = gc4[v][j];
+                            else co[v] = *reinterpret_cast<const f32x4 *>(&gco[GLDS ? v : 0][16 * j + 4 * kq]);
+                        }
+                        x4 = grad_pre_vec<f32x4, 4>(x4, zb[t], co[0], co[1], co[2], co[3], co[4], co[5], a.gp.inv_n, grelu);
+                    }
+                    if (PRE == 1) {
                         const f32x4 sc = COEF_REGS ? sc4[COEF_REGS ? j : 0] : *reinterpret_cast<const f32x4 *>(&pco[0][16 * j + 4 * kq]);
-                        const f32x4 sh = COEF_REGS ? sh4[COEF_REGS ? j : 0] : *reinterpret_cast<const f32x4 *>(&pco[PRE && !COEF_REGS ? 1 : 0][16 * j + 4 * kq]);
+                        const f32x4 sh = COEF_REGS ? sh4[COEF_REGS ? j : 0] : *reinterpret_cast<const f32x4 *>(&pco[PRE == 1 && !COEF_REGS ? 1 : 0][16 * j + 4 * kq]);
                         x4 = x4 * sc + sh;
 #pragma unroll
                         for (int c = 0; c < 4; ++c) x4[c] = fmaxf(x4[c], relu_lo);
@@ -208,8 +257,9 @@
 constexpr int GROUP_GN = 2;
 template <int K, int GN, int NIN, int MP> constexpr int group_lds_bytes() { return NIN * GN * (K / 16) * 64 * (int)sizeof(typename Mma<MP>::frag); }
 
-template <int K, int GN, int NIN, bool PRE, int ST, int MP>
+template <int K, int GN, int NIN, int PRE, int ST, int MP>
 __global__ __launch_bounds__(256, 2) void k_fwd_group(FwdArgs a) {
+    static_assert(PRE != 2 || (NIN == 1 && ST == 0), "gradient prologue: one input, no statistics");
     typedef typename Mma<MP>::frag wfrag;
     constexpr bool STATS = ST != 0;
     constexpr int NJ = K / 16;
@@ -248,9 +298,17 @@
         const int v = threadIdx.x / (GN * 16), t = threadIdx.x % (GN * 16);
         bco[ST == 2 ? v : 0][t] = a.bcoef[(long)v * a.O + gcol0 + t];
     }
-    __shared__ float pco[PRE ? 2 : 1][PRE ? K : 1];
-    if (PRE)
-        for (int t = threadIdx.x; t < K; t += 256) { pco[0][t] = a.scale[t]; pco[PRE ? 1 : 0][t] = a.shift[t]; }
+    __shared__ float pco[PRE == 1 ? 2 : 1][PRE == 1 ? K : 1];
+    if (PRE == 1)
+        for (int t = threadIdx.x; t < K; t += 256) { pco[0][t] = a.scale[t]; pco[PRE == 1 ? 1 : 0][t] = a.shift[t]; }
+    __shared__ __attribute__((aligned(16))) float gco[PRE == 2 ? 6 : 1][PRE == 2 ? K : 1];
+    if constexpr (PRE == 2) {
+        for (int t = threadIdx.x; t < 6 * K; t += 256) {
+            const int v = t / K, e = t % K;
+            gco[v][e] = v < 4 ? a.gp.coef[(long)v * K + e] : a.gp.sums[(long)(v - 4) * K + e];
+        }
+    }
+    const bool grelu = a.gp.relu != 0;
     __syncthreads();
     f32x4 s4[STATS ? GN : 1], ss4[STATS ? GN : 1];
     if (STATS) {
@@ -267,15 +325,24 @@
         f32x4 acc[GN];
 #pragma unroll
         for (int ob = 0; ob < GN; ++ob) acc[ob] = f32x4{0.f, 0.f, 0.f, 0.f};
-        f32x4 xb[2][XB];
+        f32x4 xb[2][XB], zb[PRE == 2 ? 2 : 1][PRE == 2 ? XB : 1];
 #pragma unroll
         for (int t = 0; t < XB; ++t) xb[0][t] = *reinterpret_cast<const f32x4 *>(a.X[0] + row * a.ldx + 4 * kq + 16 * t);
+        if constexpr (PRE == 2) {
+#pragma unroll
+            for (int t = 0; t < XB; ++t) zb[0][t] = *reinterpret_cast<const f32x4 *>(a.gp.z + row * a.gp.ldz + 4 * kq + 16 * t);
+        }
 #pragma unroll
         for (int b = 0; b < NB; ++b) {
             if (b + 1 < NB) {
                 const float *xr = a.X[(b + 1) / NBJ] + row * a.ldx + 4 * kq + 16 * ((b + 1) % NBJ) * XB;
 #pragma unroll
                 for (int t = 0; t < XB; ++t) xb[(b + 1) & 1][t] = *reinterpret_cast<const f32x4 *>(xr + 16 * t);
+                if constexpr (PRE == 2) {
+                    const float *zr = a.gp.z + row * a.gp.ldz + 4 * kq + 16 * ((b + 1) % NBJ) * XB;
+#pragma unroll
+                    for (int t = 0; t < XB; ++t) zb[(b + 1) & 1][t] = *reinterpret_cast<const f32x4 *>(zr + 16 * t);
+                }
             }
             __builtin_amdgcn_sched_barrier(0);
             const int in = b / NBJ;
@@ -283,9 +350,15 @@
             for (int t = 0; t < XB; ++t) {
                 const int j = (b % NBJ) * XB + t;
                 f32x4 x4 = xb[b & 1][t];
-                if (PRE) {
+                if constexpr (PRE == 2) {
+                    f32x4 co[6];
+#pragma unroll
+                    for (int v = 0; v < 6; ++v) co[v] = *reinterpret_cast<const f32x4 *>(&gco[PRE == 2 ? v : 0][16 * j + 4 * kq]);
+                    x4 = grad_pre_vec<f32x4, 4>(x4, zb[PRE == 2 ? b & 1 : 0][PRE == 2 ? t : 0], co[0], co[1], co[2], co[3], co[4], co[5], a.gp.inv_n, grelu);
+                }
+                if (PRE == 1) {
                     const f32x4 sc = *reinterpret_cast<const f32x4 *>(&pco[0][16 * j + 4 * kq]);
-                    const f32x4 sh = *reinterpret_cast<const f32x4 *>(&pco[PRE ? 1 : 0][16 * j + 4 * kq]);
+                    const f32x4 sh = *reinterpret_cast<const f32x4 *>(&pco[PRE == 1 ? 1 : 0][16 * j + 4 * kq]);
                     x4 = x4 * sc + sh;
 #pragma unroll
                     for (int c = 0; c < 4; ++c) x4[c] = fmaxf(x4[c], relu_lo);
@@ -368,14 +441,16 @@
     const float *roww; long rws;
     float *slab;
     float *bslab;
+    GradPre gpz[WG_MAXG];
 };
 
 template <int VW> struct Vec;
 template <> struct Vec<2> { typedef float type __attribute__((ext_vector_type(2))); };
 template <> struct Vec<4> { typedef float type __attribute__((ext_vector_type(4))); };
 
-template <int VW, bool PRE, bool RW, int MP>
+template <int VW, bool PRE, bool RW, int MP, bool GP = false>
 __global__ __launch_bounds__(256) void k_wg(WArgs a) {
+    static_assert(!(GP && RW), "gradient prologue: no row weight");
     typedef typename Vec<VW>::type vec;
     constexpr int B = 16 * VW;
     __shared__ float red[4][B * B];
@@ -400,6 +475,16 @@
         }
     }
     const float relu_lo = relu ? 0.f : -INFINITY;
+    const GradPre gp = a.gpz[GP ? blockIdx.z : 0];
+    const bool gp_on = GP && gp.z != nullptr;
+    vec gco[GP ? 6 : 1];
+    if constexpr (GP) {
+        if (gp_on) {
+#pragma unroll
+            for (int v = 0; v < 6; ++v)
+                gco[v] = *reinterpret_cast<const vec *>((v < 4 ? gp.coef + (long)v * a.O : gp.sums + (long)(v - 4) * a.O) + ob + VW * li);
+        }
+    }
     f32x4 acc[VW][VW];
     float gsum[VW];
 #pragma unroll
@@ -410,8 +495,9 @@
     }
     const long rb = (long)blockIdx.x * a.rows_per_block;
     const long re = rb + a.rows_per_block < a.N ? rb + a.rows_per_block : a.N;
-    for (long r0 = rb + 16 * wave; r0 < re; r0 += 64) {
-        vec gv[4], xv[4];
+    auto trip = [&](auto gon, long r0) __attribute__((always_inline)) {
+        constexpr bool GON = decltype(gon)::value;
+        vec gv[4], xv[4], zv[GON ? 4 : 1];
         float rw[RW ? 4 : 1];
         bool ok[4];
 #pragma unroll
@@ -421,11 +507,14 @@
             const long nn = ok[t] ? n : rb;
             gv[t] = *reinterpret_cast<const vec *>(G + nn * a.ldg + ob + VW * li);
             xv[t] = *reinterpret_cast<const vec *>(X + nn * a.ldx + kb + VW * li);
+            if constexpr (GON) zv[t] = *reinterpret_cast<const vec *>(gp.z + nn * gp.ldz + ob + VW * li);
             if (RW) rw[RW ? t : 0] = a.roww[nn * a.rws];
         }
         __builtin_amdgcn_sched_barrier(0);
 #pragma unroll
         for (int t = 0; t < 4; ++t) {
+            if constexpr (GON)
+                gv[t] = grad_pre_vec<vec, VW>(gv[t], zv[t], gco[0], gco[GON ? 1 : 0], gco[GON ? 2 : 0], gco[GON ? 3 : 0], gco[GON ? 4 : 0], gco[GON ? 5 : 0], gp.inv_n, gp.relu != 0);
             if (RW) gv[t] *= rw[RW ? t : 0];
             if (PRE) {
                 xv[t] = xv[t] * sc + sh;
@@ -458,6 +547,12 @@
 #pragma unroll
                 for (int c2 = 0; c2 < VW; ++c2) acc[c][c2] = Mma<MP>::mma(ga[c], xa[c2], acc[c][c2]);
         }
+    };
+    if (gp_on) {
+        if constexpr (GP)
+            for (long r0 = rb + 16 * wave; r0 < re; r0 += 64) trip(std::true_type{}, r0);
+    } else {
+        for (long r0 = rb + 16 * wave; r0 < re; r0 += 64) trip(std::false_type{}, r0);
     }
 #pragma unroll
     for (int c = 0; c < VW; ++c)
@@ -557,8 +652,6 @@
 }
 #endif
 
-static inline bool aligned16(const void *p) { return (reinterpret_cast<uintptr_t>(p) & 15) == 0; }
-
 constexpr long GROUP_MAX_ROWS = 16384;
 static bool group_form_wanted(const FwdArgs &a, int k, int blocks) {
     if (blocks % GROUP_GN) return false;
@@ -569,7 +662,7 @@
     return a.N <= GROUP_MAX_ROWS && !(k == 128 && blocks * 16 > a.O);
 }
 
-template <int K, int GN, int NIN, bool PRE, int ST, int MP>
+template <int K, int GN, int NIN, int PRE, int ST, int MP>
 static bool launch_group_kernel(const FwdArgs &a, dim3 grid, hipStream_t s) {
     constexpr int lds = group_lds_bytes<K, GN, NIN, MP>();
     static PdfLdsLimit site;
@@ -582,6 +675,9 @@
 static bool launch_fwd_group(const FwdArgs &a, int blocks, int gx, hipStream_t s) {
     const bool pre = a.scale != nullptr, stats = a.partial != nullptr, bst = stats && a.bx != nullptr;
     const dim3 grid((unsigned)gx, (unsigned)(blocks / GN));
+    if constexpr (NIN == 1) {
+        if (a.gp.z) return launch_group_kernel<K, GN, 1, 2, 0, MP>(a, grid, s);
+    }
     if (bst) return launch_group_kernel<K, GN, NIN, false, 2, MP>(a, grid, s);
     if constexpr (NIN == 1) {
         if (stats) return pre ? launch_group_kernel<K, GN, 1, true, 1, MP>(a, grid, s) : launch_group_kernel<K, GN, 1, false, 1, MP>(a, grid, s);
@@ -599,6 +695,12 @@
         if (group_form_wanted(a, K, nslabs * NOB) && launch_fwd_group<K, GROUP_GN, NIN, MP>(a, nslabs * NOB, gx, s)) return gx;
     }
     const dim3 grid((unsigned)gx, (unsigned)nslabs);
+    if constexpr (NIN == 1) {
+        if (a.gp.z) {
+            k_fwd<K, NOB, 1, 2, 0, MP><<<grid, 256, 0, s>>>(a);
+            return gx;
+        }
+    }
     if (bst) {
         k_fwd<K, NOB, NIN, false, 2, MP><<<grid, 256, 0, s>>>(a);
     } else if (NIN == 1 && stats) {
@@ -619,7 +721,8 @@
 int try_forward_mp(long n, int k, int o, int nin, int nout, const float *const *x, long ldx, const float *const *w, int transpose_w,
                    const float *const *bias, const float *scale, const float *shift, int relu, float *const *y, long ldy,
                    int accumulate, float *partial, hipStream_t s, const float *roww, long rws, const float *bx, long ldb, const float *bcoef,
-                   int brelu, int *partial_rows, long ldw, void *handoff) {
+                   int brelu, int *partial_rows, long ldw, void *handoff, const GradPre *gp) {
+    if (gp && (nin != 1 || nout != 1 || scale || partial || bx || roww || !grad_pre_ok(*gp, k))) return 0;
     if (nin < 1 || nout < 1 || (nin > 1 && nout > 1) || nin > 3 || nout > 3) return 0;
     if (nin == 2 && (scale || bx)) return 0;
     if (partial && !bx && (nin != 1 || nout != 1)) return 0;
@@ -635,6 +738,7 @@
     a.bx = bx; a.ldb = ldb; a.bcoef = bcoef; a.brelu = brelu;
     a.ho_gran = static_cast<unsigned long long *>(handoff);
     a.ho_sync = handoff ? reinterpret_cast<unsigned *>(a.ho_gran + 2 * (size_t)o) : nullptr;
+    a.gp = gp ? *gp : GradPre{nullptr, 0, nullptr, nullptr, 0.f, 0};
     a.wso = transpose_w ? 1 : (ldw ? ldw : k); a.wsk = transpose_w ? o : 1;
     for (int i = 0; i < 3; ++i) {
         a.X[i] = i < nin ? x[i] : nullptr;
@@ -673,8 +777,10 @@
 
 template <int MP>
 int try_wgrad_mp(long n, int k, int o, int ng, const float *const *g, long ldg, const float *x, long ldx, const float *scale,
-                 const float *shift, int relu, float *const *dw, float *const *db, float *ws, hipStream_t s, const float *roww, long rws) {
+                 const float *shift, int relu, float *const *dw, float *const *db, float *ws, hipStream_t s, const float *roww, long rws,
+                 const GradPre *gp) {
     if (ng < 1 || ng > 3 || !ws) return 0;
+    if (gp && (ng != 1 || roww || !grad_pre_ok(*gp, o))) return 0;
     const WgPlan p = wg_plan(n, k, o, ng);
     const int vw = p.vw;
     if (!vw) return 0;
@@ -688,6 +794,7 @@
     for (int i = 0; i < WG_MAXG; ++i) {
         a.G[i] = i < ng ? g[i] : nullptr; a.dW[i] = i < ng ? dw[i] : nullptr; a.db[i] = (db && i < ng) ? db[i] : nullptr;
         a.Xz[i] = nullptr; a.scalez[i] = a.shiftz[i] = nullptr; a.reluz[i] = 0;
+        a.gpz[i] = (gp && i == 0) ? *gp : GradPre{nullptr, 0, nullptr, nullptr, 0.f, 0};
         any_bias = any_bias || a.db[i] != nullptr;
     }
     const int b = p.b;
@@ -698,7 +805,10 @@
 #define PDF_WG(VW_) do { \
         if (roww) { if (scale) k_wg<VW_, true, true, MP><<<grid, 256, 0, s>>>(a); else k_wg<VW_, false, true, MP><<<grid, 256, 0, s>>>(a); } \
         else      { if (scale) k_wg<VW_, true, false, MP><<<grid, 256, 0, s>>>(a); else k_wg<VW_, false, false, MP><<<grid, 256, 0, s>>>(a); } } while (0)
-    if (vw == 4) PDF_WG(4); else PDF_WG(2);
+    if (gp) {
+        if (vw == 4) { if (scale) k_wg<4, true, false, MP, true><<<grid, 256, 0, s>>>(a); else k_wg<4, false, false, MP, true><<<grid, 256, 0, s>>>(a); }
+        else         { if (scale) k_wg<2, true, false, MP, true><<<grid, 256, 0, s>>>(a); else k_wg<2, false, false, MP, true><<<grid, 256, 0, s>>>(a); }
+    } else if (vw == 4) PDF_WG(4); else PDF_WG(2);
 #undef PDF_WG
     RArgs r;
     r.slab = a.slab; r.bslab = a.bslab; r.B = b; r.tiles_k = k / b; r.tiles = (o / b) * (k / b); r.otiles = o / b; r.split = (int)p.split; r.K = k; r.O = o;
@@ -710,8 +820,13 @@
 template <int MP>
 int try_wgrad_group_mp(long n, int k, int o, int ng, const float *const *g, long ldg, const float *const *x, long ldx,
                        const float *const *scale, const float *const *shift, const int *relu, float *const *dw, float *const *db,
-                       float *ws, hipStream_t s) {
+                       float *ws, hipStream_t s, const GradPre *const *gp) {
     if (ng < 1 || ng > WG_MAXG || !ws) return 0;
+    bool any_gp = false;
+    for (int i = 0; gp && i < ng; ++i) {
+        if (gp[i] && !grad_pre_ok(*gp[i], o)) return 0;
+        any_gp = any_gp || gp[i] != nullptr;
+    }
     const WgPlan p = wg_plan(n, k, o, ng);
     const int vw = p.vw;
     if (!vw) return 0;
@@ -729,6 +844,7 @@
         a.G[i] = on ? g[i] : nullptr; a.Xz[i] = on ? x[i] : nullptr;
         a.scalez[i] = on ? scale[i] : nullptr; a.shiftz[i] = on ? shift[i] : nullptr; a.reluz[i] = on ? relu[i] : 0;
         a.dW[i] = on ? dw[i] : nullptr; a.db[i] = (on && db) ? db[i] : nullptr;
+        a.gpz[i] = (on && gp && gp[i]) ? *gp[i] : GradPre{nullptr, 0, nullptr, nullptr, 0.f, 0};
         any_bias = any_bias || a.db[i] != nullptr;
     }
     const int b = p.b;
@@ -736,7 +852,8 @@
     a.slab = ws;
     a.bslab = ws + (size_t)p.nblk * p.split * b * b;
     const dim3 grid((unsigned)p.split, (unsigned)((o / b) * (k / b)), (unsigned)ng);
-    if (vw == 4) k_wg<4, true, false, MP><<<grid, 256, 0, s>>>(a); else k_wg<2, true, false, MP><<<grid, 256, 0, s>>>(a);
+    if (any_gp) { if (vw == 4) k_wg<4, true, false, MP, true><<<grid, 256, 0, s>>>(a); else k_wg<2, true, false, MP, true><<<grid, 256, 0, s>>>(a); }
+    else if (vw == 4) k_wg<4, true, false, MP><<<grid, 256, 0, s>>>(a); else k_wg<2, true, false, MP><<<grid, 256, 0, s>>>(a);
     RArgs r;
     r.slab = a.slab; r.bslab = a.bslab; r.B = b; r.tiles_k = k / b; r.tiles = (o / b) * (k / b); r.otiles = o / b; r.split = (int)p.split; r.K = k; r.O = o;
     for (int i = 0; i < WG_MAXG; ++i) { r.dW[i] = a.dW[i]; r.db[i] = a.db[i]; }
```

After: 13.69 million. About the same (-0.5%).
